# NVlabs/intrinsic3d

Hardware: AMD Instinct MI355X
Metric: Gauss-Newton iterations/s at the finest SDF level (higher is better)
Workload: dtype f32

## Files before the change

intrinsic3d_amd/csrc/device/grid_kernels.hip:

```cpp
#include "kernels.hpp"
#include "voxel_hash.hpp"

namespace i3d {

thread_local char g_errbuf[512] = {0};
static thread_local char g_launch_err[256] = {0};
bool set_dynamic_lds(const void* kernel, const char* name, size_t bytes, int K) {
    hipError_t e = bytes <= I3D_LDS_LIMIT ? hipFuncSetAttribute(kernel, hipFuncAttributeMaxDynamicSharedMemorySize, (int)bytes) : hipErrorInvalidValue;
    if (e == hipSuccess) return true;
    (void)hipGetLastError();
    if (!g_launch_err[0]) std::snprintf(g_launch_err, sizeof(g_launch_err), "%s needs %zu bytes of LDS per workgroup with K = %d keyframes (limit %zu): %s", name, bytes, K, I3D_LDS_LIMIT, hipGetErrorString(e));
    return false;
}
bool take_launch_error(char* msg, size_t n) {
    if (!g_launch_err[0]) return false;
    std::snprintf(msg, n, "%s", g_launch_err); g_launch_err[0] = 0;
    return true;
}

static __device__ inline unsigned long long spread3(unsigned long long v) {
    v &= 0x1ffffull;
    v = (v | (v << 32)) & 0x1f00000000ffffull;
    v = (v | (v << 16)) & 0x1f0000ff0000ffull;
    v = (v | (v << 8)) & 0x100f00f00f00f00full;
    v = (v | (v << 4)) & 0x10c30c30c30c30c3ull;
    v = (v | (v << 2)) & 0x1249249249249249ull;
    return v;
}

__global__ void k_sort_keys(int N, const int* __restrict__ kxyz, unsigned long long* __restrict__ keys, int* __restrict__ iota) {
    const int i = blockIdx.x * blockDim.x + threadIdx.x;
    if (i >= N) return;
    const int x = kxyz[3 * i] + (1 << 19), y = kxyz[3 * i + 1] + (1 << 19), z = kxyz[3 * i + 2] + (1 << 19);
    const unsigned long long m = spread3((unsigned)(x >> 3)) | (spread3((unsigned)(y >> 3)) << 1) | (spread3((unsigned)(z >> 3)) << 2);
    keys[i] = (m << 9) | (unsigned long long)(((z & 7) << 6) | ((y & 7) << 3) | (x & 7));
    iota[i] = i;
}
void launch_sort_keys(hipStream_t st, int N, const int* kxyz, unsigned long long* keys, int* iota) {
    if (N > 0) k_sort_keys<<<(N + 255) / 256, 256, 0, st>>>(N, kxyz, keys, iota);
}

__global__ void k_permute(int N, const int* __restrict__ perm, const int* __restrict__ kxyz, const double* __restrict__ sdf,
                          const double* __restrict__ sdf_ref, const double* __restrict__ alb, const float* __restrict__ w,
                          const uint8_t* __restrict__ rgb, int* cx, int* cy, int* cz, int* rank, double* sdf0, double* x_sdf,
                          double* x_alb, float* f_sdf, float* f_alb, float* weight, uchar4* color) {
    const int s = blockIdx.x * blockDim.x + threadIdx.x;
    if (s >= N) return;
    const int v = perm[s];
    cx[s] = kxyz[3 * v]; cy[s] = kxyz[3 * v + 1]; cz[s] = kxyz[3 * v + 2]; rank[s] = v;
    sdf0[s] = sdf[v]; x_sdf[s] = sdf_ref[v]; x_alb[s] = alb[v];
    f_sdf[s] = (float)sdf_ref[v]; f_alb[s] = (float)alb[v]; weight[s] = w[v];
    color[s] = make_uchar4(rgb[3 * v], rgb[3 * v + 1], rgb[3 * v + 2], 0);
}
void launch_permute_grid(hipStream_t st, int N, const int* perm, const int* kxyz, const double* sdf, const double* sdf_ref,
                         const double* alb, const float* w, const uint8_t* rgb, int* cx, int* cy, int* cz, int* rank, double* sdf0,
                         double* x_sdf, double* x_alb, float* f_sdf, float* f_alb, float* weight, uchar4* color) {
    if (N > 0) k_permute<<<(N + 255) / 256, 256, 0, st>>>(N, perm, kxyz, sdf, sdf_ref, alb, w, rgb, cx, cy, cz, rank, sdf0, x_sdf, x_alb, f_sdf, f_alb, weight, color);
}

__global__ void k_hash_build(int N, const int* __restrict__ cx, const int* __restrict__ cy, const int* __restrict__ cz, HashTable t) {
    const int s = blockIdx.x * blockDim.x + threadIdx.x;
    if (s >= N) return;
    const unsigned long long key = pack_key(cx[s], cy[s], cz[s]);
    unsigned int h = mix64(key) & t.mask;
    for (;;) {
        const unsigned long long prev = atomicCAS(&t.keys[h], ~0ull, key);
        if (prev == ~0ull || prev == key) { t.vals[h] = s; return; }
        h = (h + 1) & t.mask;
    }
}
void launch_hash_build(hipStream_t st, int N, const int* cx, const int* cy, const int* cz, HashTable t) {
    if (N > 0) k_hash_build<<<(N + 255) / 256, 256, 0, st>>>(N, cx, cy, cz, t);
}

__global__ void k_nbr_build(int N, const int* __restrict__ cx, const int* __restrict__ cy, const int* __restrict__ cz, HashTable t, int* __restrict__ nbr) {
    const int s = blockIdx.x * blockDim.x + threadIdx.x;
    if (s >= N) return;
    const int x = cx[s], y = cy[s], z = cz[s];
#pragma unroll
    for (int i = 0; i < NUM_NBR; ++i) {
        int dx, dy, dz; nbr_offset(i, dx, dy, dz);
        nbr[(size_t)i * N + s] = hash_find(t, x + dx, y + dy, z + dz);
    }
}
void launch_nbr_build(hipStream_t st, int N, const int* cx, const int* cy, const int* cz, HashTable t, int* nbr) {
    if (N > 0) k_nbr_build<<<(N + 255) / 256, 256, 0, st>>>(N, cx, cy, cz, t, nbr);
}

__global__ void k_classify(GridView g, OptParams p, int* __restrict__ active_flag) {
    const int s = blockIdx.x * blockDim.x + threadIdx.x;
    if (s >= g.N) return;
    const int N = g.N;
    const bool valid = g.weight[s] > 0.0f;
    const bool inshell = !(fabs(g.x_sdf[s]) > p.thres_shell);
    int nb[6]; bool nbv[6];
#pragma unroll
    for (int d = 0; d < 6; ++d) { nb[d] = g.nbr[(size_t)d * N + s]; nbv[d] = nb[d] >= 0 && g.weight[nb[d]] > 0.0f; }
    const bool ring = nbv[0] && nbv[1] && nbv[2] && nbv[3] && nbv[4] && nbv[5];
    bool normal_ok = false;
    if (valid && nbv[NB_PX] && nbv[NB_PY] && nbv[NB_PZ]) {
        const float s0 = g.f_sdf[s];
        float nx = g.f_sdf[nb[NB_PX]] - s0, ny = g.f_sdf[nb[NB_PY]] - s0, nz = g.f_sdf[nb[NB_PZ]] - s0;
        const float len = sqrtf(nx * nx + (ny * ny + nz * nz));
        if (len != 0.0f) { nx /= len; ny /= len; nz /= len; }
        normal_ok = !(fabsf(nx) <= 1e-5f && fabsf(ny) <= 1e-5f && fabsf(nz) <= 1e-5f);
    }
    const bool active = valid && inshell && normal_ok;
    const bool free_vox = valid && inshell && ring;
    const bool free_sdf = free_vox && !p.fix_sdf;
    const bool free_alb = free_vox && !(p.lambda_a < 0.0);
    g.flags[s] = (valid ? F_VALID : 0) | (active ? F_ACTIVE : 0) | (ring ? F_RING : 0) | (free_sdf ? F_FREE_SDF : 0) | (free_alb ? F_FREE_ALB : 0);
    active_flag[s] = (active || free_sdf || free_alb) ? 1 : 0;
}
void launch_classify(hipStream_t st, GridView g, OptParams p, int* active_flag) {
    if (g.N > 0) k_classify<<<(g.N + 255) / 256, 256, 0, st>>>(g, p, active_flag);
}

__global__ void k_compact(int N, const int* __restrict__ flag, const int* __restrict__ scan, const uint8_t* __restrict__ flags,
                          int* __restrict__ aidx, int* __restrict__ alist, uint8_t* __restrict__ aflags) {
    const int s = blockIdx.x * blockDim.x + threadIdx.x;
    if (s >= N) return;
    if (flag[s]) { const int a = scan[s]; aidx[s] = a; alist[a] = s; aflags[a] = flags[s]; } else aidx[s] = -1;
}
void launch_compact(hipStream_t st, int N, const int* flag, const int* scan, const uint8_t* flags, int* aidx, int* alist, uint8_t* aflags) {
    if (N > 0) k_compact<<<(N + 255) / 256, 256, 0, st>>>(N, flag, scan, flags, aidx, alist, aflags);
}

__global__ void __launch_bounds__(512) k_partition_blocks(GridView g, int A, int* __restrict__ alist, uint8_t* __restrict__ aflags, int* __restrict__ aidx) {
    __shared__ int wcount[8];
    const int base = blockIdx.x * 512, a = base + (int)threadIdx.x;
    const bool in = a < A;
    const int s = in ? alist[a] : -1;
    const uint8_t fl = in ? aflags[a] : 0;
    bool rows = in && (fl & F_ACTIVE);
    if (rows) {
#pragma unroll
        for (int c = 1; c < 10; ++c) rows &= g.nbr[(size_t)slot_fwd_nbr(c) * g.N + s] >= 0;
    }
    const unsigned long long m = __ballot(rows);
    const int lane = threadIdx.x & 63, w = threadIdx.x >> 6;
    if (lane == 0) wcount[w] = __popcll(m);
    __syncthreads();
    int before = 0, total = 0;
    for (int i = 0; i < 8; ++i) { const int cnt = wcount[i]; if (i < w) before += cnt; total += cnt; }
    const int rank_rows = before + __popcll(m & ((1ull << lane) - 1ull));
    const int pos = rows ? rank_rows : total + ((int)threadIdx.x - rank_rows);
    if (in) { const int na = base + pos; alist[na] = s; aflags[na] = fl; aidx[s] = na; }
}
void launch_partition_blocks(hipStream_t st, GridView g, int A, int* alist, uint8_t* aflags, int* aidx) {
    if (A > 0) k_partition_blocks<<<(A + 511) / 512, 512, 0, st>>>(g, A, alist, aflags, aidx);
}
__global__ void k_group_rows(int A, const uint8_t* __restrict__ nrows, int* __restrict__ gmax) {
    const int gq = blockIdx.x * blockDim.x + threadIdx.x;
    if (64 * gq >= A) return;
    int m = 0;
    for (int i = 0; i < 64 && 64 * gq + i < A; ++i) m = max(m, (int)nrows[64 * (size_t)gq + i]);
    gmax[gq] = m;
}
void launch_group_rows(hipStream_t st, int A, const uint8_t* nrows, int* gmax) { if (A > 0) k_group_rows<<<((A + 63) / 64 + 255) / 256, 256, 0, st>>>(A, nrows, gmax); }

__global__ void k_anbr(int N, int A, int Acap, const int* __restrict__ alist, const int* __restrict__ nbr, const int* __restrict__ aidx, int* __restrict__ anbr) {
    const int a = blockIdx.x * blockDim.x + threadIdx.x;
    if (a >= A) return;
    const int s = alist[a];
#pragma unroll
    for (int i = 0; i < NUM_NBR; ++i) { const int nb = nbr[(size_t)i * N + s]; anbr[(size_t)i * Acap + a] = nb >= 0 ? aidx[nb] : -1; }
}
void launch_anbr(hipStream_t st, int N, int A, int Acap, const int* alist, const int* nbr, const int* aidx, int* anbr) {
    if (A > 0) k_anbr<<<(A + 255) / 256, 256, 0, st>>>(N, A, Acap, alist, nbr, aidx, anbr);
}

__global__ void k_scatter_sh(int N, const int* __restrict__ rank, const double* __restrict__ shv, float* __restrict__ sh) {
    const int s = blockIdx.x * blockDim.x + threadIdx.x;
    if (s >= N) return;
    const double* src = shv + (size_t)rank[s] * 9;
#pragma unroll
    for (int j = 0; j < 9; ++j) sh[(size_t)j * N + s] = (float)src[j];
}
void launch_scatter_sh(hipStream_t st, int N, const int* rank, const double* shv, float* sh) {
    if (N > 0) k_scatter_sh<<<(N + 255) / 256, 256, 0, st>>>(N, rank, shv, sh);
}

__global__ void k_gather_visit(int N, const int* __restrict__ rank, const double* __restrict__ xs, const double* __restrict__ xa, double* os, double* oa) {
    const int s = blockIdx.x * blockDim.x + threadIdx.x;
    if (s >= N) return;
    const int v = rank[s];
    if (os) os[v] = xs[s];
    if (oa) oa[v] = xa[s];
}
void launch_gather_visit(hipStream_t st, int N, const int* rank, const double* xs, const double* xa, double* os, double* oa) {
    if (N > 0) k_gather_visit<<<(N + 255) / 256, 256, 0, st>>>(N, rank, xs, xa, os, oa);
}

__global__ void k_update_fields(int N, const int* __restrict__ rank, const double* sr, const double* al, const uint8_t* rgb,
                                double* x_sdf, double* x_alb, float* f_sdf, float* f_alb, uchar4* color) {
    const int s = blockIdx.x * blockDim.x + threadIdx.x;
    if (s >= N) return;
    const int v = rank[s];
    if (sr) { x_sdf[s] = sr[v]; f_sdf[s] = (float)sr[v]; }
    if (al) { x_alb[s] = al[v]; f_alb[s] = (float)al[v]; }
    if (rgb) color[s] = make_uchar4(rgb[3 * v], rgb[3 * v + 1], rgb[3 * v + 2], 0);
}
void launch_update_fields(hipStream_t st, int N, const int* rank, const double* sr, const double* al, const uint8_t* rgb,
                          double* x_sdf, double* x_alb, float* f_sdf, float* f_alb, uchar4* color) {
    if (N > 0) k_update_fields<<<(N + 255) / 256, 256, 0, st>>>(N, rank, sr, al, rgb, x_sdf, x_alb, f_sdf, f_alb, color);
}

}
```

intrinsic3d_amd/csrc/device/kernels.hpp:

```cpp
#pragma once
#include "common.hpp"
#include "p2p_device.hpp"

namespace i3d {

struct HashTable { unsigned long long* keys; int* vals; unsigned int mask; };
void launch_sort_keys(hipStream_t st, int N, const int* keys_xyz , unsigned long long* sort_keys, int* iota);
void launch_permute_grid(hipStream_t st, int N, const int* perm, const int* keys_xyz, const double* sdf, const double* sdf_ref,
                         const double* alb, const float* w, const uint8_t* rgb,
                         int* cx, int* cy, int* cz, int* rank, double* sdf0, double* x_sdf, double* x_alb, float* f_sdf, float* f_alb,
                         float* weight, uchar4* color);
void launch_hash_build(hipStream_t st, int N, const int* cx, const int* cy, const int* cz, HashTable t);
void launch_nbr_build(hipStream_t st, int N, const int* cx, const int* cy, const int* cz, HashTable t, int* nbr);
void launch_classify(hipStream_t st, GridView g, OptParams p, int* active_flag);
void launch_compact(hipStream_t st, int N, const int* active_flag, const int* active_scan, const uint8_t* flags, int* aidx, int* alist, uint8_t* aflags);
void launch_partition_blocks(hipStream_t st, GridView g, int A, int* alist, uint8_t* aflags, int* aidx);
void launch_group_rows(hipStream_t st, int A, const uint8_t* nrows, int* gmax);
void launch_anbr(hipStream_t st, int N, int A, int Acap, const int* alist, const int* nbr, const int* aidx, int* anbr);
void launch_scatter_sh(hipStream_t st, int N, const int* rank, const double* sh_visit , float* sh );
void launch_gather_visit(hipStream_t st, int N, const int* rank, const double* x_sdf, const double* x_alb, double* out_sdf, double* out_alb);
void launch_update_fields(hipStream_t st, int N, const int* rank, const double* sdf_ref, const double* alb, const uint8_t* rgb,
                          double* x_sdf, double* x_alb, float* f_sdf, float* f_alb, uchar4* color);

void launch_observe(hipStream_t st, GridView g, RowView r, OptParams p, const FrameConst* frames, const unsigned* cull_mask = nullptr, bool prefilter = false);
constexpr int CULL_BLOCK = 8, CULL_MAX_LEVELS = 12;
struct CullPyramid { int levels, cells; int bw[CULL_MAX_LEVELS], bh[CULL_MAX_LEVELS], off[CULL_MAX_LEVELS]; };
CullPyramid cull_pyramid(int w, int h);
void launch_depth_blocks(hipStream_t st, const FrameConst* frames, int K, int w, int h, float2* out);
void launch_group_cull(hipStream_t st, GridView g, RowView r, OptParams p, const FrameConst* frames, const float2* dblocks, float4* bounds, unsigned* mask);

void launch_build(hipStream_t st, GridView g, RowView r, OptParams p, const FrameConst* frames, bool with_jacobian, double* cost_out , double* scratch,
                  const double* cam9 = nullptr, const LmState* lm = nullptr);
void launch_weight_sums(hipStream_t st, RowView r, GridView g, bool with_cost, double* sums13 , double* scratch);

enum PassMode { PASS_GRAD = 0, PASS_JTJP = 1, PASS_COLNORM = 2 };
struct Seg2 { size_t off0, off1; int n; };
struct PassBuffers {
    float* C;
    float* treg;
    double* shared;
    double* blocks;
    float* part; int part_stride;
};
struct GradColBuffers {
    float* Cg; float* Cc;
    float* tregg; float* tregc;
    float* part; int part_stride;
    int col_off;
    double* cost_partials; double* cost_out;
};
int  launch_eg_gradcol(hipStream_t st, GridView g, RowView r, OptParams p, GradColBuffers b);
int  launch_eg_pass(hipStream_t st, PassMode mode, GridView g, RowView r, OptParams p, const float* u , PassBuffers b, const PcgState* state);
void launch_sum_rows(hipStream_t st, PassMode mode, int K, const float* part, int nrows, int stride, double* shared, double* blocks);
void launch_gather(hipStream_t st, PassMode mode, RowView r, PassBuffers b, float* out );
int  launch_gather_tail(hipStream_t st, RowView r, PassBuffers b, float* out, const float* S, const float* D2, const float* v, double* dot_partials ,
                        bool dot_atomic, const PcgState* state);
void launch_reduce_partials(hipStream_t st, const double* partials, int nblk, int ncomp, double* dst, const PcgState* state, bool assign = false);
void launch_shared_finalize(hipStream_t st, size_t tail_off, int K, OptParams p, const double* shared, float* out , bool tail, const float* S, const float* D2,
                            const float* v, double* dot_out, const PcgState* state);

void launch_fill(hipStream_t st, int n, float* x, float v);
void launch_fill_d(hipStream_t st, int n, double* x, double v);
void launch_int_to_double(hipStream_t st, const int* src, double* dst);
void launch_mul(hipStream_t st, int n, const float* a, const float* b, float* out);
void launch_scale_from_colnorm(hipStream_t st, int n, const float* c, const float* freemask, float* S, float* cm);
void launch_lm_diag(hipStream_t st, int n, const float* c, const float* S, float inv_radius, float* D2, float* Minv_diag);
void launch_dot(hipStream_t st, int n, const float* a, const float* b, double* out , double* scratch);
void launch_count_above2(hipStream_t st, Seg2 sg, const float* a, const float* m, float tol, double* out, double* scratch);
void launch_count_above(hipStream_t st, int n, const float* a, const float* m, float tol, double* out, double* scratch);
void launch_dot2(hipStream_t st, Seg2 sg, const float* a, const float* b, double* out , double* scratch);
void launch_mul2(hipStream_t st, Seg2 sg, const float* a, const float* b, float* out);
void launch_freemask(hipStream_t st, RowView r, OptParams p, float* mask );

void launch_pcg_init(hipStream_t st, PcgState* state, int fixed_iterations, int max_iterations, const LmState* lm = nullptr);
int  launch_pcg_step(hipStream_t st, int mode, Seg2 sg, const float* p, const float* q, float* x, float* r, const float* b, const float* D2, const float* Minv,
                     float* z, const float* S_for_inline_q, double* partials , PcgState* state);
void launch_pcg_tail_x(hipStream_t st, size_t tail_off, int K, const float* p, float* x, const PcgState* state);
void launch_pcg_tail_a(hipStream_t st, int mode, size_t tail_off, int K, const float* Minv_blocks, const float* p, const float* q, float* x, float* r, const float* b,
                       const float* D2, float* z, const double* partials, int nblk, PcgState* state,
                       double* shared_zero, int nzero, int* host_flags, int seq,
                       const P2PDev& pd);
int  launch_pcg_direction(hipStream_t st, Seg2 sg, size_t tail_off, int ntail, const float* z, float* p, const float* S, float* u, const float* D2,
                          double* d2_partials , const PcgState* state);
void launch_pcg_tail_b(hipStream_t st, size_t tail_off, int K, OptParams p, double* shared, const double* pq_slice, const double* pq_partials, int nblk,
                       const double* pq_partials2, int nblk2, bool rowwise,
                       float* q, const float* S, const float* D2, const float* v, PcgState* state, const P2PDev& pd);
struct TilePlan {
    unsigned* lnbr;
    float* eaw_sym;
    int* halo_idx; int* halo_cnt;
    int* iota; int* ext_e; int* ext_pos;
    float* qh;
    int* ext_off;
    int* overflow;
    int T, hmax;
    int tile_first, ntiles_own;
    const int* ghost_tiles; int n_ghost;
    int det;
    const unsigned short* hp_off;
    const unsigned short* hp_src;
    int pull;
};
inline int tile_plan_pull_cap(int hmax) { return 4 * hmax; }
int    tile_plan_T();
int    tile_plan_tiles(int A);
int    tile_plan_hmax();
inline int tile_plan_hmax_of(int T) { return T == 1024 ? 2048 : 1536; }
inline int tile_plan_tiles_of(int A, int T) { return (A + T - 1) / T; }
size_t tile_plan_temp_bytes(int ntiles);
hipError_t launch_tile_plan(hipStream_t st, RowView r, TilePlan t, void* temp, size_t temp_bytes);
void launch_eaw_sym(hipStream_t st, RowView r, TilePlan t, const int* cflag );
int  launch_eg_tile(hipStream_t st, RowView r, OptParams p, const float* u, TilePlan t, double* shared, float* qacc, double* pq_partials ,
                    const PcgState* state, float* cam_partials = nullptr, int cam_stride = 0);
void launch_ext_offsets(hipStream_t st, int n, const int* ext_e, int A, int* ext_off);
void eg_tile_launch_shape(const TilePlan& t, int K, int& blocks, int& tiles_per_block);

struct LadVec;
int  eg_tile_mr_max_systems(int K);
int  launch_eg_tile_mr(hipStream_t st, RowView r, OptParams p, TilePlan t, int nsys, const int* sys, const float* u0, float* qacc0, float* qh0, double* pq0 , float* cam0, int cam_stride,
                       const PcgState* st0 , const LadVec& lv);

struct ShardArgs {
    P2PDev pd; RimLists rim; int seq;
    int n_slice_partials;
    int n_rim_wg;
    const float* zb; float* pb; float* ub; const float* cmb; int chunk;
};
struct LadVec {
    size_t vec;
    size_t qh;
    size_t cam;
    size_t part;
    size_t mblk;
    size_t tail;
    int sysid[LADDER_MAX];
};
struct Step3Args {
    int nq; int chunk4;
    const float4* p; const float4* qacc; float4* x; float4* r; const float4* b; float4* z;
    const float4* cm; const LmState* lm;
    const int* ext_off; const int* ext_pos; const float2* qh; int e0;
    const double* pq_partials; int n_pq; const double* d2_partials; int n_d2;
    int n_slice_wg;
    int K; int fix_poses, fix_intr, fix_dist;
    const float* cam_partials; int n_cam; int cam_stride; const float* Mblk;
    const float* tp; float* tx; float* tr; const float* tb; const float* tD2; float* tz; const float* tS;
    double* step_partials;
    PcgState* cur;
    int sharded; ShardArgs sh;
    int lad_sys;
    const double* redop; int redop_stride;
};
void launch_pcg_init3(hipStream_t st, PcgState* st2 , int fixed_iterations, int max_iterations, const LmState* lm = nullptr);
int  launch_pcg_dir3(hipStream_t st, bool init, Seg2 sg, size_t tail_off, int ntail, const float* z, float* p, const float* S, float* u, const float* D2, const float* cm, const LmState* lm,
                     const double* step_partials, int n_step, double* d2_partials, const PcgState* prev, PcgState* next, int* host_flags, int seq,
                     const ShardArgs* sa = nullptr);
void launch_rim_u(hipStream_t st, const ShardArgs& sa, const PcgState* state);
int  pcg_step3_slice_wgs(int n_entries, int cap = 0);
int  pcg_step3_tail_wgs(int K);
int  launch_pcg_step3(hipStream_t st, int mode , Step3Args a);
void launch_halo_fold(hipStream_t st, RowView r, TilePlan t, float* qacc, const PcgState* state);
void launch_pcg_init_lad(hipStream_t st, PcgState* st2_all , int B, int fixed_iterations, int max_iterations, const LmState* lm);
int  launch_pcg_dir3_lad(hipStream_t st, bool init, int nsys, Seg2 sg, size_t tail_off, int ntail, const float* z0, float* p0, const float* S, float* u0, const float* tD2_0, const float* cm, const LmState* lm,
                         const double* step_partials0, int n_step, double* d2_partials0, PcgState* st2_0, int prev_parity, int* host_flags0, int seq, const LadVec& lv,
                         int n_slice_partials = 0, const double* red4_0 = nullptr );
int  launch_pcg_step3_lad(hipStream_t st, int mode, int nsys, Step3Args a, const LadVec& lv);
void launch_lad_reduce_step(hipStream_t st, int nsys, const double* step_partials0, int n_slice, double* red4_0, const LadVec& lv);
void launch_lad_reduce_op(hipStream_t st, int nsys, const float* cam_partials0, int n_cam, int cam_stride, int NS, const double* pq_partials0, int n_pq, const double* d2_partials0, int n_d2,
                          double* redop0, int redop_stride, const LadVec& lv);

void launch_need_mask(hipStream_t st, RowView r, int slice, unsigned long long* need );
void launch_halo_items(hipStream_t st, int A, int slice, int me, const unsigned long long* need, unsigned long long* items, int* count , int cap);
void launch_tile_flags(hipStream_t st, int A, int T, const int* cflag, int* tileflag );
size_t halo_sort_temp_bytes(int cap);
hipError_t launch_halo_sort(hipStream_t st, void* temp, size_t temp_bytes, const unsigned long long* in, unsigned long long* out, int n);

void launch_candidate(hipStream_t st, GridView g, RowView r, int K, float sign, const float* step, const float* S, const double* x_shared, double* xc_sdf, double* xc_alb,
                      double* xc_shared, double* norms2 , const float* mask, double* scratch, const LmState* lm = nullptr);
void launch_accept(hipStream_t st, GridView g, RowView r, const double* xc_sdf, const double* xc_alb, const LmState* lm = nullptr);
void launch_set_double(hipStream_t st, double* dst, double v);
void launch_lm_init(hipStream_t st, LmState* lm, const double* cost, const double* ngrad, const double* nfree, double radius0, LmRecord* rec, int seq);
void launch_lm_begin(hipStream_t st, LmState* lm, int K, int fix_poses, int fix_intr, int fix_dist, const double* cdiag, const double* tri, float* Mblk,
                     const float* tc, const float* tS, float* tD2, float* tMinv, LmRecord* rec, int seq);
void launch_lm_diag_dev(hipStream_t st, int n, const float* c, const float* S, const LmState* lm, float* D2, float* Minv);
void launch_cand_frames(hipStream_t st, int K, const double* xc, const FrameConst* base, FrameConst* out, const LmState* lm);
void launch_lm_decide(hipStream_t st, LmState* lm, const PcgState* ps, const double* norms2, const double* cand_cost, int attempt, int lm_steps, LmRecord* rec, int seq,
                      int lad_next = -1 , int debug_invalid = 0);
void launch_lm_begin_lad(hipStream_t st, LmState* lm, int B, int K, int fix_poses, int fix_intr, int fix_dist, const double* cdiag, const double* tri, float* Mblk, size_t mblk_stride,
                         const float* tc, const float* tS, float* tD2, size_t tail_stride, LmRecord* rec, int seq);
void launch_mark_compute(hipStream_t st, RowView r, int* flag);
void launch_compact_list(hipStream_t st, int A, const int* flag, const int* scan, int* list);

}
```

intrinsic3d_amd/csrc/device/pcg_fused.hip:

```cpp
#include "kernels.hpp"
#include "reduce_device.hpp"
#include <cstring>

namespace i3d {

constexpr int PF_THREADS = 512;
constexpr int PF_MAX_WG = 512;
constexpr int PF_POSES_PER_WG = 10;

template <int NC>
static __device__ inline void reduce_partials_all(const double* __restrict__ P, int nblk, double (&tot)[NC], double* sm ,
                                                  const double* __restrict__ P2 = nullptr, int nblk2 = 0 ) {
    double v[NC];
#pragma unroll
    for (int k = 0; k < NC; ++k) v[k] = 0.0;
    for (int i = threadIdx.x; i < nblk; i += PF_THREADS) {
#pragma unroll
        for (int k = 0; k < NC; ++k) v[k] += P[(size_t)i * NC + k];
    }
    for (int i = threadIdx.x; i < nblk2; i += PF_THREADS) {
#pragma unroll
        for (int k = 0; k < NC; ++k) v[k] += P2[(size_t)i * NC + k];
    }
#pragma unroll
// ... 303 lines not shown
                    }
                    if (MODE == S3_XONLY) continue;
                    const float4 bb = in.b[seg];
                    const float bv[4] = {bb.x, bb.y, bb.z, bb.w};
                    float qq[4];
#pragma unroll
                    for (int k = 0; k < 4; ++k) qq[k] = svv[k] * accv[seg][k] + dv[k] * (MODE == S3_NORMAL ? pv[k] : xv[k]);
                    if (MODE == S3_NORMAL) { const float4 ro = in.r[seg]; rv[0] = ro.x - alpha * qq[0]; rv[1] = ro.y - alpha * qq[1]; rv[2] = ro.z - alpha * qq[2]; rv[3] = ro.w - alpha * qq[3]; }
                    else { rv[0] = bv[0] - qq[0]; rv[1] = bv[1] - qq[1]; rv[2] = bv[2] - qq[2]; rv[3] = bv[3] - qq[3]; }
                    R[i] = make_float4(rv[0], rv[1], rv[2], rv[3]);
#pragma unroll
                    for (int k = 0; k < 4; ++k) { const double xd = xv[k]; s1 += xd * ((double)bv[k] + (double)rv[k]); s2 += xd * (double)rv[k]; s3 += (double)dv[k] * xd * xd; }
                }
                const float zv[4] = {mv[0] * rv[0], mv[1] * rv[1], mv[2] * rv[2], mv[3] * rv[3]};
                Z[i] = make_float4(zv[0], zv[1], zv[2], zv[3]);
#pragma unroll
                for (int k = 0; k < 4; ++k) s0 += (double)rv[k] * (double)zv[k];
            }
        }
    } else {
        const int K = a.K, tw = (int)blockIdx.x - a.n_slice_wg, n_pose_wg = (K + PF_POSES_PER_WG - 1) / PF_POSES_PER_WG;
        int col0, ncol;
        if (tw < n_pose_wg) { col0 = 6 * PF_POSES_PER_WG * tw; const int c1 = min(6 * K, col0 + 6 * PF_POSES_PER_WG); ncol = c1 - col0; }
        else { col0 = 6 * K; ncol = 9; }
        const int t = threadIdx.x;
        if (MODE == S3_NORMAL || MODE == S3_RESET) {
            const int g = t / 64, c = t % 64;
            double v = 0.0;
            if (SH != 2 && c < ncol) for (int w = g; w < a.n_cam; w += 8) v += (double)cam_partials[(size_t)w * a.cam_stride + col0 + c];
            camred[g][c] = v;
            __syncthreads();
            if (t < ncol) {
                double s = 0.0; for (int gg = 0; gg < 8; ++gg) s += camred[gg][t];
                if (SH == 2) s = a.redop[(size_t)(o.sys < 0 ? 0 : o.sys) * a.redop_stride + col0 + t];
                if (SH == 1) {
                    const unsigned e32 = p2p_pass_epoch(a.sh.seq, MODE == S3_RESET ? P2P_X_RESET_STEP : P2P_X_STEP);
                    p2p_put_double_all(a.sh.pd, 1, e32, 1 + col0 + t, s);
                    s = 0.0; for (int j = 0; j < a.sh.pd.L.world; ++j) s += p2p_get_double(a.sh.pd, 1, e32, j, 1 + col0 + t);
                }
                camv[t] = s;
            }
            __syncthreads();
        }
        if (t < ncol) {
            const int i = col0 + t;
            const bool fixed = i < 6 * K ? a.fix_poses : (i < 6 * K + 4 ? a.fix_intr : a.fix_dist);
            float ri;
            if (MODE == S3_INIT) ri = tr[i];
            else {
                float xi = tx[i];
                if (MODE != S3_RESET) { xi += alpha * tp[i]; tx[i] = xi; }
                if (MODE == S3_XONLY) ri = 0.0f;
                else {
                    const float vv = MODE == S3_NORMAL ? tp[i] : xi;
                    const float qi = a.tS[i] * (fixed ? 0.0f : (float)camv[t]) + tD2[i] * vv;
                    ri = MODE == S3_NORMAL ? tr[i] - alpha * qi : a.tb[i] - qi;
                    tr[i] = ri;
                    const double xd = xi; s1 += xd * ((double)a.tb[i] + (double)ri); s2 += xd * (double)ri; s3 += (double)tD2[i] * xd * xd;
                }
            }
            rs[t] = ri;
        }
        if (MODE == S3_XONLY) return;
        __syncthreads();
        if (t < ncol) {
            const int i = col0 + t;
            int base, n, row; const float* M;
            if (i < 6 * K) { const int f = i / 6; base = 6 * f; n = 6; row = i - base; M = Mblk + 36 * f; }
            else if (i < 6 * K + 4) { base = 6 * K; n = 4; row = i - base; M = Mblk + 36 * K; }
            else { base = 6 * K + 4; n = 5; row = i - base; M = Mblk + 36 * K + 16; }
            float s = 0.0f;
            for (int j = 0; j < n; ++j) s += M[row * n + j] * rs[base - col0 + j];
            tz[i] = s; s0 += (double)rs[t] * (double)s;
        }
    }
    if (MODE == S3_XONLY) return;
    block_partial_d(s0, step_partials, 4, 0); block_partial_d(s1, step_partials, 4, 1); block_partial_d(s2, step_partials, 4, 2); block_partial_d(s3, step_partials, 4, 3);
}
template <int MODE, int SH>
__global__ void __launch_bounds__(PF_THREADS) k_pcg_step3(Step3Args a) { const S3Off o{0, 0, 0, 0, 0, 0, 0, 0, -1}; pcg_step3_body<MODE, SH>(a, o); }
template <int MODE, bool COLL>
__global__ void __launch_bounds__(PF_THREADS) k_pcg_step3_lad(Step3Args a, LadVec lv) {
    const int j = lv.sysid[blockIdx.y];
    const S3Off o{((size_t)j * lv.vec) >> 2, (size_t)j * lv.vec, ((size_t)j * lv.qh) >> 1, (size_t)j * lv.part, (size_t)j * lv.cam, (size_t)j * lv.mblk, (size_t)j * lv.tail, 2 * j, j};
    pcg_step3_body<MODE, COLL ? 2 : 0>(a, o);
}

int pcg_step3_slice_wgs(int n_entries, int cap) { if (cap <= 0 || cap > PF_MAX_WG) cap = PF_MAX_WG; int b = (n_entries / 4 + PF_THREADS - 1) / PF_THREADS; return b < 1 ? 1 : (b > cap ? cap : b); }
int pcg_step3_tail_wgs(int K) { return (K + PF_POSES_PER_WG - 1) / PF_POSES_PER_WG + 1; }

int launch_pcg_step3(hipStream_t st, int mode, Step3Args a) {
    const int blocks = a.n_slice_wg + pcg_step3_tail_wgs(a.K);
#define I3D_S3(M) do { if (a.sharded) k_pcg_step3<M, 1><<<blocks, PF_THREADS, 0, st>>>(a); else k_pcg_step3<M, 0><<<blocks, PF_THREADS, 0, st>>>(a); } while (0)
    switch (mode) {
        case S3_INIT:   I3D_S3(S3_INIT); break;
        case S3_NORMAL: I3D_S3(S3_NORMAL); break;
        case S3_XONLY:  I3D_S3(S3_XONLY); break;
        default:        I3D_S3(S3_RESET); break;
    }
#undef I3D_S3
    return mode == S3_XONLY ? 0 : blocks;
}

int launch_pcg_step3_lad(hipStream_t st, int mode, int nsys, Step3Args a, const LadVec& lv) {
    const int blocks = a.n_slice_wg + pcg_step3_tail_wgs(a.K);
    const dim3 grid(blocks, nsys);
#define I3D_S3L(M) do { if (a.redop) k_pcg_step3_lad<M, true><<<grid, PF_THREADS, 0, st>>>(a, lv); else k_pcg_step3_lad<M, false><<<grid, PF_THREADS, 0, st>>>(a, lv); } while (0)
    switch (mode) {
        case S3_INIT:   I3D_S3L(S3_INIT); break;
        case S3_NORMAL: I3D_S3L(S3_NORMAL); break;
        case S3_XONLY:  I3D_S3L(S3_XONLY); break;
        default:        I3D_S3L(S3_RESET); break;
    }
#undef I3D_S3L
    return mode == S3_XONLY ? 0 : blocks;
}

__global__ void __launch_bounds__(PF_THREADS) k_lad_reduce_step(const double* __restrict__ step_partials0, int n_slice, double* __restrict__ red4_0, LadVec lv) {
    __shared__ double sm[4 * 8];
    const int j = lv.sysid[blockIdx.x];
    double tot[4];
    reduce_partials_all<4>(step_partials0 + (size_t)j * lv.part, n_slice, tot, sm);
    if (threadIdx.x < 4) red4_0[4 * j + threadIdx.x] = threadIdx.x == 0 ? tot[0] : threadIdx.x == 1 ? tot[1] : threadIdx.x == 2 ? tot[2] : tot[3];
}
void launch_lad_reduce_step(hipStream_t st, int nsys, const double* step_partials0, int n_slice, double* red4_0, const LadVec& lv) {
    k_lad_reduce_step<<<nsys, PF_THREADS, 0, st>>>(step_partials0, n_slice, red4_0, lv);
}
__global__ void __launch_bounds__(PF_THREADS) k_lad_reduce_op(const float* __restrict__ cam_partials0, int n_cam, int cam_stride, int NS, const double* __restrict__ pq_partials0, int n_pq,
                                                              const double* __restrict__ d2_partials0, int n_d2, double* __restrict__ redop0, int redop_stride, LadVec lv) {
    __shared__ double sm[8];
    __shared__ double camred[8][64];
    const int j = lv.sysid[blockIdx.y];
    double* const out = redop0 + (size_t)j * redop_stride;
    const int ncw = (NS + 63) / 64;
    if ((int)blockIdx.x < ncw) {
        const int t = threadIdx.x, g = t / 64, c = t % 64, col = (int)blockIdx.x * 64 + c;
        const float* cp = cam_partials0 + (size_t)j * lv.cam;
        double v = 0.0;
        if (col < NS) for (int w = g; w < n_cam; w += 8) v += (double)cp[(size_t)w * cam_stride + col];
        camred[g][c] = v;
        __syncthreads();
        if (t < 64 && col < NS) { double s = 0.0; for (int gg = 0; gg < 8; ++gg) s += camred[gg][t]; out[col] = s; }
    } else {
        double t1[1];
        reduce_partials_all<1>(pq_partials0 + (size_t)j * lv.part, n_pq, t1, sm, d2_partials0 + (size_t)j * lv.part, n_d2);
        if (threadIdx.x == 0) out[NS] = t1[0];
    }
}
void launch_lad_reduce_op(hipStream_t st, int nsys, const float* cam_partials0, int n_cam, int cam_stride, int NS, const double* pq_partials0, int n_pq, const double* d2_partials0, int n_d2,
                          double* redop0, int redop_stride, const LadVec& lv) {
    k_lad_reduce_op<<<dim3((NS + 63) / 64 + 1, nsys), PF_THREADS, 0, st>>>(cam_partials0, n_cam, cam_stride, NS, pq_partials0, n_pq, d2_partials0, n_d2, redop0, redop_stride, lv);
}

__global__ void k_pcg_init_lad(PcgState* st2_all, int B, int fixed_iterations, int max_iterations, const LmState* lm) {
    const int j = threadIdx.x;
    if (j >= B) return;
    const bool over = lm->done != 0 || lm->lad_radius[j] < 1e-32;
    for (int b = 0; b < 2; ++b) {
        PcgState* st = st2_all + 2 * j + b;
        for (int k = 0; k < 4; ++k) st->acc[k] = 0.0;
        st->rho = 0.0; st->last_rho = 1.0; st->pq = 0.0; st->alpha = 0.0; st->beta = 0.0; st->xbr = 0.0; st->xr = 0.0; st->d2xx = 0.0;
        st->Q0 = 0.0; st->Q1 = 0.0; st->it = 0; st->done = (fixed_iterations == 0 || over) ? 1 : 0; st->fixed_iterations = fixed_iterations; st->max_iterations = max_iterations;
    }
}
void launch_pcg_init_lad(hipStream_t st, PcgState* st2_all, int B, int fixed_iterations, int max_iterations, const LmState* lm) { k_pcg_init_lad<<<1, LADDER_MAX, 0, st>>>(st2_all, B, fixed_iterations, max_iterations, lm); }

__global__ void k_ext_offsets(int n, const int* __restrict__ ext_e, int A, int* __restrict__ ext_off) {
    const int e = blockIdx.x * blockDim.x + threadIdx.x;
    if (e > A) return;
    int lo = 0, hi = n;
    while (lo < hi) { const int mid = (lo + hi) >> 1; if (ext_e[mid] < e) lo = mid + 1; else hi = mid; }
    ext_off[e] = lo;
}
void launch_ext_offsets(hipStream_t st, int n, const int* ext_e, int A, int* ext_off) { k_ext_offsets<<<(A + 1 + 255) / 256, 256, 0, st>>>(n, ext_e, A, ext_off); }

}
```

intrinsic3d_amd/csrc/device/tile_pass.hip:

```cpp
#include <cstring>
#include <cstdlib>
#include <climits>
#include "kernels.hpp"
#include "reduce_device.hpp"
#include "wave_ops.hpp"
#include "tile_device.hpp"
#include <rocprim/rocprim.hpp>

namespace i3d {

constexpr int TP_PLAN_LIST = 2048;
constexpr int TP_NONE = 0x7f7f7f7f;
__device__ __host__ inline int tp_dir(int j) {
    constexpr int8_t D[18] = {NB_PY, NB_P2Y, NB_PYZ, NB_PZ, NB_P2Z, NB_PX, NB_PXY, NB_PXZ, NB_P2X, NB_MX, NB_MY, NB_MZ,
                              NB_M2Y, NB_MYZ, NB_M2Z, NB_MXY, NB_MXZ, NB_M2X};
    return D[j];
}

__global__ void __launch_bounds__(1024) k_tile_plan(RowView r, int T, int hmax, int hlimit , int tile_first, const int* __restrict__ tile_list, unsigned* __restrict__ lnbr,
                                                    int* __restrict__ halo_idx, int* __restrict__ halo_cnt, int* __restrict__ overflow) {
    __shared__ int hkeys[4096];
    __shared__ int hlist[TP_PLAN_LIST];
    __shared__ int cnt;
    const int tile = tile_list ? tile_list[blockIdx.x] : tile_first + (int)blockIdx.x, base = tile * T, a = base + threadIdx.x;
    const bool in = (int)threadIdx.x < T && a < r.A;
    const int zslot = T + hmax;
    for (int i = threadIdx.x; i < 4096; i += 1024) hkeys[i] = -1;
    hlist[threadIdx.x] = TP_NONE; hlist[threadIdx.x + 1024] = TP_NONE;
    if (threadIdx.x == 0) cnt = 0;
    __syncthreads();
    int la[18];
#pragma unroll
    for (int j = 0; j < 18; ++j) la[j] = r.anbr[(size_t)tp_dir(j) * r.Acap + (in ? a : 0)];
#pragma unroll
    for (int j = 0; j < 18; ++j) {
        if (!in) la[j] = -1;
        if (j < 12 && la[j] >= 0 && (unsigned)(la[j] - base) >= (unsigned)T) {
            unsigned h = ((unsigned)la[j] * 2654435761u) >> 20;
            for (int probes = 0; probes < 4096; ++probes) {
                const int k = atomicCAS(&hkeys[h], -1, la[j]);
                if (k == -1 || k == la[j]) break;
                h = (h + 1) & 4095u;
            }
        }
    }
    __syncthreads();
    for (int i = threadIdx.x; i < 4096; i += 1024) if (hkeys[i] >= 0) { const int pos = atomicAdd(&cnt, 1); if (pos < TP_PLAN_LIST) hlist[pos] = hkeys[i]; }
    __syncthreads();
    const int H = cnt;
    if (H > hlimit) {
        for (int i = threadIdx.x; i < hmax; i += 1024) halo_idx[(size_t)tile * hmax + i] = TP_NONE;
        if (threadIdx.x == 0) { *overflow = 1; halo_cnt[tile] = 0; }
        return;
    }
    int NS = 64; while (NS < H) NS <<= 1;
    for (int k = 2; k <= NS; k <<= 1)
        for (int j = k >> 1; j > 0; j >>= 1) {
#pragma unroll
            for (int half = 0; half < 2; ++half) {
                const int i = threadIdx.x + half * 1024, ixj = i ^ j;
                if (i < NS && ixj > i) { const int x = hlist[i], y = hlist[ixj]; const bool up = (i & k) == 0; if ((x > y) == up) { hlist[i] = y; hlist[ixj] = x; } }
            }
            __syncthreads();
        }
    for (int i = threadIdx.x; i < hmax; i += 1024) halo_idx[(size_t)tile * hmax + i] = hlist[i];
    if (threadIdx.x == 0) halo_cnt[tile] = H;
    if (!in) return;
    unsigned short ls[18];
#pragma unroll
    for (int j = 0; j < 18; ++j) {
        int slot = zslot;
        if (la[j] >= 0) {
            const unsigned off = (unsigned)(la[j] - base);
            if (off < (unsigned)T) slot = (int)off;
            else if (j < 12) { int lo = 0, hi = H - 1; while (lo < hi) { const int mid = (lo + hi) >> 1; if (hlist[mid] < la[j]) lo = mid + 1; else hi = mid; } slot = T + lo; }
        }
        ls[j] = (unsigned short)slot;
    }
    unsigned pw[LNBR_WORDS];
#pragma unroll
    for (int w = 0; w < LNBR_WORDS; ++w) pw[w] = 0u;
#pragma unroll
    for (int j = 0; j < 18; ++j) { const int bit = 12 * j, k = bit >> 5, sh = bit & 31; pw[k] |= (unsigned)ls[j] << sh; if (sh > 20) pw[k + 1] |= (unsigned)ls[j] >> (32 - sh); }
#pragma unroll
    for (int w = 0; w < LNBR_WORDS; ++w) lnbr[(size_t)w * r.Acap + a] = pw[w];
}

__global__ void __launch_bounds__(256) k_eaw_sym(RowView r, const int* __restrict__ cflag , float* __restrict__ eaw_sym) {
    const int a = blockIdx.x * blockDim.x + threadIdx.x;
    if (a >= r.A) return;
    const bool act = (r.aflags[a] & F_ACTIVE) != 0 && (!cflag || cflag[a]);
    float wo[6]; int nb[6];
#pragma unroll
    for (int d = 0; d < 6; ++d) { wo[d] = r.ea_w[(size_t)d * r.Acap + a]; nb[d] = r.anbr[(size_t)d * r.Acap + a]; }
    uint8_t nfl[6]; int ncf[6]; float wn[6];
#pragma unroll
    for (int d = 0; d < 6; ++d) { const int n = nb[d] >= 0 ? nb[d] : a; nfl[d] = r.aflags[n]; ncf[d] = cflag ? cflag[n] : 1; wn[d] = r.ea_w[(size_t)(d ^ 1) * r.Acap + n]; }
#pragma unroll
    for (int d = 0; d < 6; ++d) {
        float w = act ? wo[d] : 0.0f;
        if (nb[d] >= 0 && (nfl[d] & F_ACTIVE) && ncf[d]) w += wn[d];
        eaw_sym[(size_t)d * r.Acap + a] = w;
    }
}

template <int T, int HMAX>
__global__ void __launch_bounds__(T) k_tile_pull_plan(RowView r, int tile_first, const int* __restrict__ tile_list, const unsigned* __restrict__ lnbr, const int* __restrict__ halo_cnt,
                                                      unsigned short* __restrict__ hp_off, unsigned short* __restrict__ hp_src, int* __restrict__ overflow) {
    constexpr int CAP = 4 * HMAX, ZSLOT = T + HMAX, PER = HMAX / T, NWV = T / 64;
    static_assert(HMAX % T == 0, "slots per thread");
    __shared__ int cnt[HMAX];
    __shared__ int off[HMAX + 1];
    __shared__ unsigned short list[CAP];
    __shared__ int wsum[NWV];
    const int tile = tile_list ? tile_list[blockIdx.x] : tile_first + (int)blockIdx.x, a = tile * T + (int)threadIdx.x;
    const bool in = a < r.A;
    for (int s2 = threadIdx.x; s2 < HMAX; s2 += T) cnt[s2] = 0;
    __syncthreads();
    unsigned ln[5];
#pragma unroll
    for (int w = 0; w < 5; ++w) ln[w] = in ? lnbr[(size_t)w * r.Acap + a] : 0u;
    constexpr int RJ[18] = {0, 1, 2, 3, 4, 5, 6, 7, 8, 5, 0, 3, 5, 9, 0, 10, 3, 11};
    constexpr int RC[18] = {0, 1, 2, 3, 4, 5, 6, 7, 8, 9, 10, 11, 12, 12, 12, 12, 12, 12};
    int hs[18];
#pragma unroll
    for (int k = 0; k < 18; ++k) { const int sl = in ? unpack12(ln, RJ[k]) : ZSLOT; hs[k] = (sl >= T && sl != ZSLOT) ? sl - T : -1; if (hs[k] >= 0) atomicAdd(&cnt[hs[k]], 1); }
    __syncthreads();
    int loc[PER], sum = 0;
#pragma unroll
    for (int q = 0; q < PER; ++q) { loc[q] = cnt[threadIdx.x * PER + q]; sum += loc[q]; }
    int inc = sum;
    for (int o = 1; o < 64; o <<= 1) { const int v = __shfl_up(inc, o, 64); if ((int)(threadIdx.x & 63) >= o) inc += v; }
    if ((threadIdx.x & 63) == 63) wsum[threadIdx.x >> 6] = inc;
    __syncthreads();
    int base = 0, total = 0;
    for (int w = 0; w < NWV; ++w) { if (w < (int)(threadIdx.x >> 6)) base += wsum[w]; total += wsum[w]; }
    int run = base + inc - sum;
#pragma unroll
    for (int q = 0; q < PER; ++q) { off[threadIdx.x * PER + q] = run; run += loc[q]; }
    if (threadIdx.x == T - 1) off[HMAX] = run;
    for (int s2 = threadIdx.x; s2 < HMAX; s2 += T) cnt[s2] = 0;
    __syncthreads();
    if (total > CAP) {
        if (threadIdx.x == 0) *overflow = 1;
        for (int s2 = threadIdx.x; s2 <= HMAX; s2 += T) hp_off[(size_t)tile * (HMAX + 1) + s2] = 0;
        return;
    }
#pragma unroll
    for (int k = 0; k < 18; ++k) if (hs[k] >= 0) { const int pos = off[hs[k]] + atomicAdd(&cnt[hs[k]], 1); list[pos] = (unsigned short)((RC[k] << 10) | (int)threadIdx.x); }
    __syncthreads();
    const int H = halo_cnt[tile];
    for (int s2 = threadIdx.x; s2 < H; s2 += T) {
        const int j0 = off[s2], j1 = off[s2 + 1];
        for (int i2 = j0 + 1; i2 < j1; ++i2) { const unsigned short v = list[i2]; int j = i2 - 1; while (j >= j0 && list[j] > v) { list[j + 1] = list[j]; --j; } list[j + 1] = v; }
    }
    __syncthreads();
    for (int s2 = threadIdx.x; s2 <= HMAX; s2 += T) hp_off[(size_t)tile * (HMAX + 1) + s2] = (unsigned short)off[s2];
    for (int p2 = threadIdx.x; p2 < total; p2 += T) hp_src[(size_t)tile * CAP + p2] = list[p2];
}

template <int NV, class F>
static __device__ inline void wave_accumulate_lds(bool valid, int f, F val, float* lds, int reps, int rs, int wave_off, int stride, int base_off = 0) {
    bool pending = valid;
    unsigned long long todo = __ballot(pending);
    for (int round = 0; todo != 0ull; ++round) {
        if (round == 3) {
            if (pending) {
                int lane_rep = (int)(threadIdx.x & (unsigned)(reps - 1));
                asm volatile("" : "+v"(lane_rep));
                const int lane_off = base_off + lane_rep * rs;
#pragma unroll
                for (int i = 0; i < NV; ++i) lds_add(&lds[lane_off + stride * f + i], val(i));
            }
            break;
        }
        const int leader = __ffsll((long long)todo) - 1;
        const int f0 = __builtin_amdgcn_readlane(f, leader);
        const bool mine = pending && f == f0;
        const bool lead = (int)(threadIdx.x & 63) == leader;
#pragma unroll
        for (int i = 0; i < NV; ++i) { const float sum = wave_sum(mine ? val(i) : 0.0f); if (lead) lds_add(&lds[wave_off + stride * f0 + i], sum); }
        pending = pending && !mine;
        todo = __ballot(pending);
    }
}

template <int T, int HMAX, int SLOTS, bool GHOSTS, int DETM>
__global__ void __launch_bounds__(T, 4) k_eg_tile(RowView r, OptParams p, const float* __restrict__ u, const unsigned* __restrict__ lnbr,
                                                        const float* __restrict__ eaw_sym, const int* __restrict__ halo_idx, const int* __restrict__ halo_cnt,
                                                        double* __restrict__ shared, float* __restrict__ qacc, float* __restrict__ qh, double* __restrict__ pq_partials,
                                                        int reps, int tiles_per_block, int tile_first, int n_own ,
                                                        const int* __restrict__ ghost_list , int ntl, const PcgState* __restrict__ state,
                                                        float* __restrict__ cam_partials , int cam_stride,
                                                        const int* __restrict__ gmaxv ,
                                                        const unsigned short* __restrict__ hp_off, const unsigned short* __restrict__ hp_src ) {
    if (state && state->done) return;
    constexpr bool DET = (DETM & 3) != 0, DORD = (DETM & 1) != 0, DTAB = (DETM & 2) != 0, HP = (DETM & 4) != 0;
    static_assert(!(DORD && HP), "a pulled halo needs no ordered pushes");
    constexpr int ZSLOT = T + HMAX, NSLOT = ZSLOT + 1;
    extern __shared__ float lds[];
    const int K = p.K; const size_t Acap = r.Acap; const int A = r.A, chunk = r.chunk;
    const int nshared = 6 * K + 9;
    const int rs = (6 * K) | 1;
    constexpr int NW = T / 64, TC = T == 1024 ? 64 : 32;
    constexpr int D_CAM9W = 4, D_TAG = D_CAM9W + ((NW * 9 + 3) & ~3), D_VAL = D_TAG + NW * TC, D0 = DET ? D_VAL + NW * TC * 6 : 0;
    const int nacc = D0 + reps * rs + 9;
    const int o_upose = (nacc + 3) & ~3, o_u = (o_upose + nshared + 3) & ~3;
    for (int i = D0 + threadIdx.x; i < nacc; i += T) lds[i] = 0.0f;
#define upose (lds + o_upose)
#define u_s (lds + o_u)
#define u_a (lds + o_u + NSLOT)
#define qh_s (lds + o_u + 2 * NSLOT)
#define qh_a (lds + o_u + 2 * NSLOT + HMAX)
#define tr_l (lds + o_u + 2 * NSLOT + 2 * HMAX)
#define C_l (lds + o_u + 2 * NSLOT + 2 * HMAX + T + 4)
    const size_t tail = 2 * (size_t)chunk;
    for (int i = threadIdx.x; i < nshared; i += T) upose[i] = u[tail + i];
    const int o_cam = D0 + reps * rs;
// ... 135 lines not shown
#pragma unroll
                for (int q = 0; q < 7; ++q) { J[4 * q] = rw[q].x; J[4 * q + 1] = rw[q].y; J[4 * q + 2] = rw[q].z; J[4 * q + 3] = rw[q].w; }
                J[28] = rb.j28;
                float d = DTAB ? J[0] * u_s[i] + J[10] * u_a[i] : J[0] * us + J[10] * ua;
#pragma unroll
                for (int c = 1; c < 10; ++c) d += J[c] * u_s[unpack12(ln, c - 1)];
                d += J[11] * u_a[sx] + J[12] * u_a[sy] + J[13] * u_a[sz];
                const int o_up = o_upose + 6 * f;
#pragma unroll
                for (int q = 0; q < 6; ++q) d += J[P_POSE + q] * lds[o_up + q];
#pragma unroll
                for (int q = 0; q < 9; ++q) d += J[P_INTR + q] * ui[q];
                const float t = rho * d;
                pq_rows += t * d;
                self_s += J[0] * t; self_a += J[10] * t;
#pragma unroll
                for (int c = 1; c < 10; ++c) Cme[(c - 1) * T] += J[c] * t;
                Cme[9 * T] += J[11] * t; Cme[10 * T] += J[12] * t; Cme[11 * T] += J[13] * t;
                if (!p.fix_poses && owned) { fsel = f; pvalid = true; tsel = t; }
                if (owned) {
#pragma unroll
                    for (int q = 0; q < 9; ++q) cam9[q] += J[P_INTR + q] * t;
                }
            }
            if (DTAB) wave_table_add<6, TC>(pvalid, fsel, [&](int q) { const float j = q == 0 ? rw[3].z : q == 1 ? rw[3].w : q == 2 ? rw[4].x : q == 3 ? rw[4].y : q == 4 ? rw[4].z : rw[4].w; return j * tsel; },
                                           lds, o_tag, o_val, tcount, D0, 6);
            else wave_accumulate_lds<6>(pvalid, fsel, [&](int q) { const float j = q == 0 ? rw[3].z : q == 1 ? rw[3].w : q == 2 ? rw[4].x : q == 3 ? rw[4].y : q == 4 ? rw[4].z : rw[4].w; return j * tsel; },
                                        lds, reps, rs, o_wave_acc, 6, D0);
        };
        if (SLOTS > 0 && ghost_tile && __ballot(nr > 0) == 0ull) {
        } else if (SLOTS > 0) {
#pragma unroll
            for (int k = 0; k < SLOTS; k += 2) {
                consume(rwA, k);
                if (k + 2 < SLOTS) load_block(rwA, k + 2, SLOTS);
                if (k + 1 < SLOTS) {
                    consume(rwB, k + 1);
                    if (k + 3 < SLOTS) load_block(rwB, k + 3, SLOTS);
                }
            }
        } else {
            for (int k = 0; k < nr_max; k += 2) {
                consume(rwA, k);
                if (k + 2 < nr_max) load_block(rwA, k + 2, r.slots);
                if (k + 1 < nr_max) {
                    consume(rwB, k + 1);
                    if (k + 3 < nr_max) load_block(rwB, k + 3, r.slots);
                }
            }
        }
        if (owned) pq_l[i] += (double)pq_rows;
        unsigned lr[2];
#pragma unroll
        for (int w = 0; w < 2; ++w) lr[w] = __builtin_nontemporal_load(&lnbr[(size_t)(5 + w) * Acap + ac]);
        float eaw[6];
#pragma unroll
        for (int d = 0; d < 6; ++d) eaw[d] = __builtin_nontemporal_load(&eaw_sym[(size_t)d * Acap + ac]);
        if (DORD) {
            ordered_enter(&lds[o_det], wave);
            if (rf & 1) {
                const float tr = tr_l[i]; const int rg[6] = {sx, mx, sy, my, sz, mz};
#pragma unroll
                for (int d = 0; d < 6; ++d) if (rg[d] >= T && rg[d] != ZSLOT) lds_add(&qh_s[rg[d] - T], tr);
            }
        }
        if (!HP && nr > 0) {
#pragma unroll
            for (int c = 1; c < 10; ++c) { const int sl = unpack12(ln, c - 1); if (sl >= T && sl != ZSLOT) lds_add(&qh_s[sl - T], Cme[(c - 1) * T]); }
            if (sx >= T && sx != ZSLOT) lds_add(&qh_a[sx - T], Cme[9 * T]);
            if (sy >= T && sy != ZSLOT) lds_add(&qh_a[sy - T], Cme[10 * T]);
            if (sz >= T && sz != ZSLOT) lds_add(&qh_a[sz - T], Cme[11 * T]);
        }
        if (DTAB && DORD) { if (tcount > TC - 16) wave_table_merge<6, TC>(lds, o_tag, o_val, tcount, D0, 6); }
        if (DORD) ordered_leave(&lds[o_det], wave);
        if (DTAB && !DORD) { if (tcount > TC - 16 && (threadIdx.x & 63u) == 0u) lds[o_det] = __int_as_float(1); }
        const int a_c = a, H_c = H, tile_c = tile; const bool in_c = in, owned_c = owned; const float ua_c = DTAB ? u_a[i] : ua;
        __syncthreads();
        if (DTAB && !DORD) {
            if (__float_as_int(lds[o_det]) != 0) {
                for (int w = 0; w < NW; ++w) { if (wave == w) wave_table_merge<6, TC>(lds, o_tag, o_val, tcount, D0, 6); __syncthreads(); }
            }
        }
        if (in_c) {
            const unsigned lall[LNBR_WORDS] = {0u, 0u, 0u, 0u, ln[4], lr[0], lr[1]};
            const int r2y = unpack12(lall, 12), ryz = unpack12(lall, 13), r2z = unpack12(lall, 14), rxy = unpack12(lall, 15), rxz = unpack12(lall, 16), r2x = unpack12(lall, 17);
            auto pull = [&](int col, int slot) { return slot < T ? C_l[col * T + slot] : 0.0f; };
            float qs = self_s, qa = self_a;
            qs += pull(0, my) + pull(1, r2y) + pull(2, ryz) + pull(3, mz) + pull(4, r2z) + pull(5, mx) + pull(6, rxy) + pull(7, rxz) + pull(8, r2x);
            qa += pull(9, mx) + pull(10, my) + pull(11, mz);
            const int rg[6] = {sx, mx, sy, my, sz, mz};
#pragma unroll
            for (int d = 0; d < 6; ++d) qs += tr_l[rg[d] < T ? rg[d] : T];
            float ea = 0.0f, eq = 0.0f;
#pragma unroll
            for (int d = 0; d < 6; ++d) { const float diff = ua_c - u_a[rg[d]]; const float t = eaw[d] * diff; ea += t; eq += (rg[d] == ZSLOT ? 1.0f : 0.5f) * t * diff; }
            qa += tw3 * ea; if (owned_c) pq_l[i] += (double)(tw3 * eq);
            qacc[a_c] = qs; qacc[chunk + a_c] = qa;
        }
#pragma unroll
        for (int q = 0; q < NQH; ++q) {
            const int hq = i + q * T;
            if (hq < H_c) {
                const size_t o = (size_t)tile_c * HMAX + hq;
                if (HP) {
                    float hsum = 0.0f, hal = 0.0f;
                    const int j1 = hp_offs[hq + 1];
                    for (int j = hp_offs[hq]; j < j1; ++j) {
                        const int e = hp_list[j], col = e >> 10, lane = e & 1023;
                        const float v = col == 12 ? tr_l[lane] : C_l[col * T + lane];
                        if (col >= 9 && col != 12) hal += v; else hsum += v;
                    }
                    qh[2 * o] = hsum; qh[2 * o + 1] = hal;
                } else { qh[2 * o] = qh_s[hq]; qh[2 * o + 1] = qh_a[hq]; }
            }
        }
        __syncthreads();
    }
#pragma unroll
    for (int q = 0; q < 9; ++q) {
        float v = cam9[q];
        for (int o = 32; o > 0; o >>= 1) v += __shfl_down(v, o, 64);
        if ((threadIdx.x & 63) == 0) { if (DTAB) lds[o_cam9w + wave * 9 + q] = v; else if (v != 0.0f) lds_add(&lds[o_cam + q], v); }
    }
    __syncthreads();
    if (DTAB) {
        for (int w = 0; w < NW; ++w) { if (wave == w) wave_table_merge<6, TC>(lds, o_tag, o_val, tcount, D0, 6); __syncthreads(); }
        if (threadIdx.x < 9) { float v = 0.0f; for (int w = 0; w < NW; ++w) v += lds[o_cam9w + w * 9 + threadIdx.x]; lds[o_cam + threadIdx.x] = v; }
        __syncthreads();
    }
    for (int q = threadIdx.x; q < nshared; q += T) {
        float v;
        if (q < 6 * K) { v = 0.0f; for (int rp = 0; rp < reps; ++rp) v += lds[D0 + rp * rs + q]; }
        else v = lds[o_cam + q - 6 * K];
        if (cam_partials) cam_partials[(size_t)blockIdx.x * cam_stride + q] = v;
        else if (v != 0.0f) atomicAdd(&shared[q], (double)v);
    }
    if (pq_partials) block_partial_d(pq_l[i], pq_partials, 1, 0);
#undef pq_l
#undef hp_list
#undef hp_offs
#undef o_tag
#undef o_val
#undef upose
#undef u_s
#undef u_a
#undef qh_s
#undef qh_a
#undef tr_l
#undef C_l
#undef ui
#undef Cme
}

__global__ void __launch_bounds__(256) k_halo_fold(int n, const int* __restrict__ ext_e, const int* __restrict__ ext_pos, const float* __restrict__ qh,
                                                   float* __restrict__ qacc, int chunk, const PcgState* __restrict__ state) {
    if (state && state->done) return;
    const int i = blockIdx.x * blockDim.x + threadIdx.x;
    if (i >= n) return;
    const int e = ext_e[i];
    if (e >= TP_NONE || (i > 0 && ext_e[i - 1] == e)) return;
    float s = 0.0f, al = 0.0f;
    for (int j = i; j < n && ext_e[j] == e; ++j) { const float2 v = reinterpret_cast<const float2*>(qh)[ext_pos[j]]; s += v.x; al += v.y; }
    qacc[e] += s; qacc[chunk + e] += al;
}

__global__ void k_iota(int n, int* __restrict__ x) { const int i = blockIdx.x * blockDim.x + threadIdx.x; if (i < n) x[i] = i; }

static int tp_T() { const char* e = std::getenv("I3D_EGT_TILE"); return (e && std::atoi(e) == 512) ? 512 : 1024; }
static int tp_H() { return tp_T() == 1024 ? 2048 : 1536; }
int tile_plan_tiles(int A) { return (A + tp_T() - 1) / tp_T(); }
int tile_plan_hmax() { return tp_H(); }
size_t tile_plan_temp_bytes(int ntiles) {
    size_t bytes = 0;
    (void)rocprim::radix_sort_pairs(nullptr, bytes, (const int*)nullptr, (int*)nullptr, (const int*)nullptr, (int*)nullptr, (size_t)ntiles * tp_H(), 0, 32, (hipStream_t)0);
    return bytes;
}

hipError_t launch_tile_plan(hipStream_t st, RowView r, TilePlan t, void* temp, size_t temp_bytes) {
    const int ntiles = tile_plan_tiles_of(r.A, t.T);
    if (ntiles <= 0) return hipSuccess;
    hipError_t e = hipMemsetAsync(t.overflow, 0, sizeof(int), st); if (e != hipSuccess) return e;
    const int n = ntiles * t.hmax;
    const int limit512 = [] { const char* s = std::getenv("I3D_EGT_HMAX_LIMIT"); return s ? std::atoi(s) : 0; }();
    const int limit1024 = [] { const char* s = std::getenv("I3D_EGT_HMAX_LIMIT_1024"); return s ? std::atoi(s) : 0; }();
    const int lim = t.T == 512 ? limit512 : limit1024;
    const int hlimit = (lim > 0 && lim < t.hmax) ? lim : t.hmax;
    const bool all = t.tile_first == 0 && t.ntiles_own >= ntiles;
    if (!all) { e = hipMemsetAsync(t.halo_idx, 0x7f, sizeof(int) * (size_t)n, st); if (e != hipSuccess) return e;
                e = hipMemsetAsync(t.halo_cnt, 0, sizeof(int) * (size_t)ntiles, st); if (e != hipSuccess) return e; }
    if (t.ntiles_own > 0) k_tile_plan<<<t.ntiles_own, 1024, 0, st>>>(r, t.T, t.hmax, hlimit, t.tile_first, nullptr, t.lnbr, t.halo_idx, t.halo_cnt, t.overflow);
    if (t.n_ghost > 0) k_tile_plan<<<t.n_ghost, 1024, 0, st>>>(r, t.T, t.hmax, hlimit, 0, t.ghost_tiles, t.lnbr, t.halo_idx, t.halo_cnt, t.overflow);
    if (t.hp_off) {
        unsigned short* off = const_cast<unsigned short*>(t.hp_off); unsigned short* src = const_cast<unsigned short*>(t.hp_src);
        if (t.T == 1024) { if (t.ntiles_own > 0) k_tile_pull_plan<1024, 2048><<<t.ntiles_own, 1024, 0, st>>>(r, t.tile_first, nullptr, t.lnbr, t.halo_cnt, off, src, t.overflow);
                           if (t.n_ghost > 0) k_tile_pull_plan<1024, 2048><<<t.n_ghost, 1024, 0, st>>>(r, 0, t.ghost_tiles, t.lnbr, t.halo_cnt, off, src, t.overflow); }
        else { if (t.ntiles_own > 0) k_tile_pull_plan<512, 1536><<<t.ntiles_own, 512, 0, st>>>(r, t.tile_first, nullptr, t.lnbr, t.halo_cnt, off, src, t.overflow);
               if (t.n_ghost > 0) k_tile_pull_plan<512, 1536><<<t.n_ghost, 512, 0, st>>>(r, 0, t.ghost_tiles, t.lnbr, t.halo_cnt, off, src, t.overflow); }
    }
    k_iota<<<(n + 255) / 256, 256, 0, st>>>(n, t.iota);
    int key_bits = 32;
    for (int b = 1; b < 32; ++b) { const unsigned mask = (1u << b) - 1u; if ((1u << b) >= (unsigned)r.A && ((unsigned)TP_NONE & mask) >= (unsigned)r.A) { key_bits = b; break; } }
    e = rocprim::radix_sort_pairs(temp, temp_bytes, (const int*)t.halo_idx, t.ext_e, (const int*)t.iota, t.ext_pos, (size_t)n, 0, key_bits, st);
    if (e != hipSuccess) return e;
    if (t.ext_off) launch_ext_offsets(st, n, t.ext_e, r.chunk, t.ext_off);
    return hipGetLastError();
}

void launch_eaw_sym(hipStream_t st, RowView r, TilePlan t, const int* cflag) { if (r.A > 0) k_eaw_sym<<<(r.A + 255) / 256, 256, 0, st>>>(r, cflag, t.eaw_sym); }

struct EgtShape { int detm, reps, per_cu, blocks, tiles_per_block; size_t lds; };
template <int T, int HMAX>
static EgtShape egt_shape(const TilePlan& t, int K, int num_cu) {
    const int nshared = 6 * K + 9, rs = (6 * K) | 1;
    static const bool ordered = [] { const char* e = std::getenv("I3D_EGT_ORDERED"); return e && e[0] == '1'; }();
    const bool pull = t.pull && t.hp_off != nullptr && !(t.det && ordered);
    EgtShape s; s.detm = t.det ? (pull ? 6 : 3) : (pull ? 4 : 0);
    const bool det = (s.detm & 3) != 0;
    constexpr int NW = T / 64, TC = T == 1024 ? 64 : 32;
    const int det_words = det ? 4 + ((NW * 9 + 3) & ~3) + NW * TC * 7 : 0;
    auto lds_bytes = [&](int reps) { const int nacc = det_words + reps * rs + 9; const int o_upose = (nacc + 3) & ~3, o_u = (o_upose + nshared + 3) & ~3;
                                     return (size_t)(o_u + 2 * (T + HMAX + 1) + 2 * HMAX + T + 4 + 12 * T + 2 * T  + (pull ? (HMAX + 4) / 2 : 0) ) * sizeof(float); };
    const size_t budget = (T == 512 ? 79 : 158) * 1024;
    s.reps = (s.detm & 2) ? 1 : 4;
    while (s.reps > 1 && lds_bytes(s.reps) > budget) s.reps >>= 1;
    s.lds = lds_bytes(s.reps);
    s.per_cu = (T == 512 && s.lds <= budget) ? 2 : 1;
    { static int knob = -1; if (knob < 0) { const char* e = std::getenv("I3D_EGT_WG_PER_CU"); knob = e ? std::atoi(e) : 0; } if (knob > 0) s.per_cu = knob; }
    const int ntl = t.ntiles_own + t.n_ghost;
    s.blocks = 0; s.tiles_per_block = 0;
    if (ntl > 0) {
        s.blocks = ntl < s.per_cu * num_cu ? ntl : s.per_cu * num_cu;
        s.tiles_per_block = (ntl + s.blocks - 1) / s.blocks;
        if (ntl > s.blocks && ntl < 2 * s.blocks) { s.tiles_per_block = 1; s.blocks = ntl; }
    }
    return s;
}
static int egt_num_cu() {
    static int num_cu = 0;
    if (!num_cu) { int dev = 0; (void)hipGetDevice(&dev); hipDeviceProp_t pr; (void)hipGetDeviceProperties(&pr, dev); num_cu = pr.multiProcessorCount > 0 ? pr.multiProcessorCount : 256; }
    return num_cu;
}
void eg_tile_launch_shape(const TilePlan& t, int K, int& blocks, int& tiles_per_block) {
    const EgtShape s = t.T == 1024 ? egt_shape<1024, 2048>(t, K, egt_num_cu()) : egt_shape<512, 1536>(t, K, egt_num_cu());
    blocks = s.blocks; tiles_per_block = s.tiles_per_block;
}

template <int T, int HMAX>
static int launch_eg_tile_t(hipStream_t st, RowView r, OptParams p, const float* u, TilePlan t, double* shared, float* qacc, double* pq_partials, const PcgState* state, int num_cu,
                            float* cam_partials, int cam_stride) {
    const EgtShape sh = egt_shape<T, HMAX>(t, p.K, num_cu);
    const int detm = sh.detm, reps = sh.reps; const size_t lds = sh.lds; const bool pull = (detm & 4) != 0;
    int written = 0;
    {
        const int ntl = t.ntiles_own + t.n_ghost;
        if (ntl > 0) {
            const int blocks = sh.blocks, tiles_per_block = sh.tiles_per_block;
#define I3D_EGT(SL, GH) do { if (detm == 3) I3D_EGT2(SL, GH, 3); else if (detm == 6) I3D_EGT2(SL, GH, 6); else if (detm == 4) I3D_EGT2(SL, GH, 4); else I3D_EGT2(SL, GH, 0); } while (0)
#define I3D_EGT2(SL, GH, DT) do { \
        if (!set_dynamic_lds((const void*)k_eg_tile<T, HMAX, SL, GH, DT>, "k_eg_tile", lds, p.K)) break; \
        k_eg_tile<T, HMAX, SL, GH, DT><<<blocks, T, lds, st>>>(r, p, u, t.lnbr, t.eaw_sym, t.halo_idx, t.halo_cnt, shared, qacc, t.qh, pq_partials, reps, tiles_per_block, t.tile_first, t.ntiles_own, \
                                                   t.ghost_tiles, ntl, state, cam_partials, cam_stride, r.gmax, pull ? t.hp_off : nullptr, pull ? t.hp_src : nullptr); } while (0)
            const bool gh = t.n_ghost > 0;
            if (r.slots == 5) { if (gh) I3D_EGT(5, true); else I3D_EGT(5, false); }
            else { if (gh) I3D_EGT(0, true); else I3D_EGT(0, false); }
#undef I3D_EGT
#undef I3D_EGT2
            written = blocks;
        }
    }
    return written;
}

int launch_eg_tile(hipStream_t st, RowView r, OptParams p, const float* u, TilePlan t, double* shared, float* qacc, double* pq_partials, const PcgState* state,
                   float* cam_partials, int cam_stride) {
    if (r.A <= 0) return 0;
    const int num_cu = egt_num_cu();
    if (t.T == 1024) return launch_eg_tile_t<1024, 2048>(st, r, p, u, t, shared, qacc, pq_partials, state, num_cu, cam_partials, cam_stride);
    return launch_eg_tile_t<512, 1536>(st, r, p, u, t, shared, qacc, pq_partials, state, num_cu, cam_partials, cam_stride);
}
void launch_halo_fold(hipStream_t st, RowView r, TilePlan t, float* qacc, const PcgState* state) {
    if (r.A <= 0) return;
    const int n = tile_plan_tiles_of(r.A, t.T) * t.hmax;
    k_halo_fold<<<(n + 255) / 256, 256, 0, st>>>(n, t.ext_e, t.ext_pos, t.qh, qacc, r.chunk, state);
}
int tile_plan_T() { return tp_T(); }

}
```

intrinsic3d_amd/csrc/host/context.cpp:

```cpp
#include "context.hpp"
#include "../device/frame_math.hpp"
#include <rocprim/rocprim.hpp>
#include <algorithm>

using namespace i3d;

static thread_local std::string g_create_error;

namespace i3d {

int ctx_fail(i3d_context* c, int code, const std::string& msg) { if (c) c->err = msg; else g_create_error = msg; return code; }
int ctx_hip(i3d_context* c, hipError_t e, const char* what) {
    return ctx_fail(c, I3D_ERR_HIP, std::string(what) + " -> " + hipGetErrorString(e));
}

int ctx_launch_check(i3d_context* c) {
    char msg[256];
    if (take_launch_error(msg, sizeof(msg))) return ctx_fail(c, I3D_ERR_CAPACITY, msg);
    const hipError_t e = hipGetLastError();
    return e == hipSuccess ? I3D_OK : ctx_hip(c, e, "kernel launch");
}

int ensure_pinned(i3d_context* c, size_t n) {
    if (n <= c->h_pinned_n) return I3D_OK;
    if (c->h_pinned) (void)hipHostFree(c->h_pinned);
    c->h_pinned = nullptr; c->h_pinned_n = 0;
    CTX_HIP(c, hipHostMalloc((void**)&c->h_pinned, n * sizeof(double), hipHostMallocDefault));
    c->h_pinned_n = n;
    return I3D_OK;
}

bool timing_begin(i3d_context* c, int cat) {
    if (!c->timing.on || !((c->timing.mask >> cat) & 1u)) return false;
    Timing::Pending p; p.cat = cat;
    auto get = [&]() { hipEvent_t e; if (!c->timing.pool.empty()) { e = c->timing.pool.back(); c->timing.pool.pop_back(); } else (void)hipEventCreate(&e); return e; };
    p.a = get(); p.b = get();
    (void)hipEventRecord(p.a, c->stream);
    c->timing.pending.push_back(p);
    return true;
}
void timing_end(i3d_context* c) {
    if (c->timing.pending.empty()) return;
    (void)hipEventRecord(c->timing.pending.back().b, c->stream);
}
void timing_flush(i3d_context* c) {
    if (c->timing.pending.empty()) return;
    (void)hipStreamSynchronize(c->stream);
    for (auto& p : c->timing.pending) {
        float ms = 0.0f;
        if (hipEventElapsedTime(&ms, p.a, p.b) == hipSuccess) { c->timing.ms[p.cat] += ms; c->timing.launches[p.cat] += 1; c->timing.each[p.cat].push_back(ms); }
        c->timing.pool.push_back(p.a); c->timing.pool.push_back(p.b);
    }
    c->timing.pending.clear();
}

void build_frame_consts(const i3d_context* c, int level, const double* poses, std::vector<FrameConst>& out) {
    out.resize(c->K);
    for (int f = 0; f < c->K; ++f) {
        FrameConst& fc = out[f];
        fm::frame_from_pose(poses + 6 * f, fc);
        const size_t k = (size_t)f * c->levels + level;
        fc.hot.lum = c->lum[k].p; fc.depth = c->depth[k].p; fc.bgr = c->bgr[k].p;
        fc.w = c->fw[level]; fc.h = c->fh[level];
    }
}

}

i3d::GridView i3d_context::grid_view() const {
    GridView g;
    g.N = N; g.voxel_size = voxel_size; g.truncation = truncation;
    g.cx = cx.p; g.cy = cy.p; g.cz = cz.p; g.rank = rank.p; g.nbr = nbr.p; g.weight = weight.p; g.color = color.p;
    g.sdf0 = sdf0.p; g.x_sdf = x_sdf.p; g.x_alb = x_alb.p; g.f_sdf = f_sdf.p; g.f_alb = f_alb.p; g.sh = sh.p;
    g.flags = flags.p; g.aidx = aidx.p;
    return g;
}
i3d::RowView i3d_context::row_view() const {
    RowView r;
    r.A = A; r.Acap = Acap; r.slots = slots; r.chunk = chunk; r.world = comm ? comm->world : 1; r.own0 = own0; r.own1 = own1;
    r.clist = (comm && (comm->world > 1 || comm->force)) ? clist.p : nullptr; r.nC = nC; r.alist = alist.p; r.aflags = aflags.p; r.anbr = anbr.p; r.obs_frame = obs_frame.p; r.obs_w = obs_w.p;
    r.rows = rows.p; r.row_wr = row_wr.p; r.nrows = nrows.p; r.gmax = gmax.p; r.regflags = regflags.p; r.ea_w = ea_w.p; r.ea_free = ea_free.p;
    return r;
}

extern "C" {

const char* i3d_version(void) { return "intrinsic3d_hip 0.1 (gfx950)"; }
const char* i3d_last_error(const i3d_context* ctx) { return ctx ? ctx->err.c_str() : g_create_error.c_str(); }

int i3d_create(int32_t device_ordinal, i3d_context** out) {
    if (!out) return ctx_fail(nullptr, I3D_ERR_INVALID_ARGUMENT, "i3d_create: null output pointer");
    *out = nullptr;
    int count = 0;
    hipError_t e = hipGetDeviceCount(&count);
    if (e != hipSuccess || count <= 0)
        return ctx_fail(nullptr, I3D_ERR_NO_DEVICE, "no HIP device visible: this library has no CPU fallback");
    if (device_ordinal < 0 || device_ordinal >= count) return ctx_fail(nullptr, I3D_ERR_INVALID_ARGUMENT, "device ordinal out of range");
    e = hipSetDevice(device_ordinal);
    if (e != hipSuccess) return ctx_hip(nullptr, e, "hipSetDevice");
    auto* c = new i3d_context();
    c->device = device_ordinal;
    e = hipStreamCreateWithFlags(&c->stream, hipStreamNonBlocking);
    if (e != hipSuccess) { delete c; return ctx_hip(nullptr, e, "hipStreamCreate"); }
    *out = c;
    return I3D_OK;
}

void i3d_destroy(i3d_context* c) {
    if (!c) return;
    (void)hipSetDevice(c->device);
    timing_flush(c);
    for (auto e : c->timing.pool) (void)hipEventDestroy(e);
    if (c->h_pinned) (void)hipHostFree(c->h_pinned);
    if (c->h_pcg) (void)hipHostFree(c->h_pcg);
    if (c->h_flags) (void)hipHostFree(c->h_flags);
    if (c->h_lmrec) (void)hipHostFree(c->h_lmrec);
    for (auto e : c->ev_asm) if (e) (void)hipEventDestroy(e);
    for (auto e : c->pcg_ev) if (e) (void)hipEventDestroy(e);
    delete c->comm;
    if (c->stream) (void)hipStreamDestroy(c->stream);
    delete c;
}

int i3d_set_grid(i3d_context* c, const i3d_grid_view* gv) {
    if (!c || !gv || gv->num_voxels <= 0 || !gv->keys || !gv->sdf || !gv->sdf_refined || !gv->albedo || !gv->weight || !gv->color)
        return ctx_fail(c, I3D_ERR_INVALID_ARGUMENT, "i3d_set_grid: null grid or empty voxel list");
    if (gv->num_voxels > (1ll << 30)) return ctx_fail(c, I3D_ERR_CAPACITY, "i3d_set_grid: more than 2^30 voxels");
    CTX_HIP(c, hipSetDevice(c->device));
    const int N = (int)gv->num_voxels;
    hipStream_t st = c->stream;
    GridStaging g;
    CTX_HIP(c, g.kxyz.alloc((size_t)3 * N)); CTX_HIP(c, g.sdf.alloc(N)); CTX_HIP(c, g.sdf_ref.alloc(N)); CTX_HIP(c, g.alb.alloc(N)); CTX_HIP(c, g.w.alloc(N)); CTX_HIP(c, g.rgb.alloc((size_t)3 * N));
    CTX_HIP(c, hipMemcpyAsync(g.kxyz.p, gv->keys, sizeof(int) * 3 * (size_t)N, hipMemcpyHostToDevice, st));
    CTX_HIP(c, hipMemcpyAsync(g.sdf.p, gv->sdf, sizeof(double) * (size_t)N, hipMemcpyHostToDevice, st));
    CTX_HIP(c, hipMemcpyAsync(g.sdf_ref.p, gv->sdf_refined, sizeof(double) * (size_t)N, hipMemcpyHostToDevice, st));
    CTX_HIP(c, hipMemcpyAsync(g.alb.p, gv->albedo, sizeof(double) * (size_t)N, hipMemcpyHostToDevice, st));
    CTX_HIP(c, hipMemcpyAsync(g.w.p, gv->weight, sizeof(float) * (size_t)N, hipMemcpyHostToDevice, st));
    CTX_HIP(c, hipMemcpyAsync(g.rgb.p, gv->color, (size_t)3 * N, hipMemcpyHostToDevice, st));
    return set_grid_device(c, N, gv->voxel_size, gv->truncation, g);
}

}

namespace i3d {
int set_grid_device(i3d_context* c, int N, float voxel_size, float truncation, GridStaging& g) {
    c->N = N; c->voxel_size = voxel_size; c->truncation = truncation; c->have_grid = false; c->have_sh = false; c->have_subvolumes = false; c->assembled = false;
    c->render_bricks_ok = false;
    c->slots = 0;
    hipStream_t st = c->stream;
    DevBuf<int> perm, iota; DevBuf<unsigned long long> skeys, skeys2;
    CTX_HIP(c, perm.alloc(N)); CTX_HIP(c, iota.alloc(N)); CTX_HIP(c, skeys.alloc(N)); CTX_HIP(c, skeys2.alloc(N));
    launch_sort_keys(st, N, g.kxyz.p, skeys.p, iota.p);
    size_t tmp_bytes = 0;
    CTX_HIP(c, rocprim::radix_sort_pairs(nullptr, tmp_bytes, skeys.p, skeys2.p, iota.p, perm.p, (size_t)N, 0, 64, st));
    DevBuf<unsigned char> tmp; CTX_HIP(c, tmp.alloc(tmp_bytes));
    CTX_HIP(c, rocprim::radix_sort_pairs(tmp.p, tmp_bytes, skeys.p, skeys2.p, iota.p, perm.p, (size_t)N, 0, 64, st));
    auto fit = [&](auto& buf, size_t n) -> hipError_t { if (buf.n != n) buf.release(); return buf.alloc(n); };
    CTX_HIP(c, fit(c->cx, N)); CTX_HIP(c, fit(c->cy, N)); CTX_HIP(c, fit(c->cz, N)); CTX_HIP(c, fit(c->rank, N));
    CTX_HIP(c, fit(c->sdf0, N)); CTX_HIP(c, fit(c->x_sdf, N)); CTX_HIP(c, fit(c->x_alb, N)); CTX_HIP(c, fit(c->xc_sdf, N)); CTX_HIP(c, fit(c->xc_alb, N));
    CTX_HIP(c, fit(c->f_sdf, N)); CTX_HIP(c, fit(c->f_alb, N)); CTX_HIP(c, fit(c->weight, N)); CTX_HIP(c, fit(c->color, N));
    CTX_HIP(c, fit(c->flags, N)); CTX_HIP(c, fit(c->aidx, N)); CTX_HIP(c, fit(c->alist, N)); CTX_HIP(c, fit(c->aflag, N)); CTX_HIP(c, fit(c->ascan, N));
    CTX_HIP(c, fit(c->sh, (size_t)9 * N)); CTX_HIP(c, fit(c->nbr, (size_t)NUM_NBR * N));
    launch_permute_grid(st, N, perm.p, g.kxyz.p, g.sdf.p, g.sdf_ref.p, g.alb.p, g.w.p, g.rgb.p, c->cx.p, c->cy.p, c->cz.p, c->rank.p, c->sdf0.p,
                        c->x_sdf.p, c->x_alb.p, c->f_sdf.p, c->f_alb.p, c->weight.p, c->color.p);
    CTX_HIP(c, hipMemcpyAsync(c->xc_sdf.p, c->x_sdf.p, sizeof(double) * (size_t)N, hipMemcpyDeviceToDevice, st));
    CTX_HIP(c, hipMemcpyAsync(c->xc_alb.p, c->x_alb.p, sizeof(double) * (size_t)N, hipMemcpyDeviceToDevice, st));
    unsigned int cap = 1; while (cap < (unsigned int)N * 2u) cap <<= 1;
    CTX_HIP(c, fit(c->hkeys, cap)); CTX_HIP(c, fit(c->hvals, cap)); c->hmask = cap - 1;
    CTX_HIP(c, hipMemsetAsync(c->hkeys.p, 0xff, sizeof(unsigned long long) * (size_t)cap, st));
    HashTable t{c->hkeys.p, c->hvals.p, cap - 1};
    launch_hash_build(st, N, c->cx.p, c->cy.p, c->cz.p, t);
    launch_nbr_build(st, N, c->cx.p, c->cy.p, c->cz.p, t, c->nbr.p);
    CTX_HIP(c, hipMemsetAsync(c->sh.p, 0, sizeof(float) * 9 * (size_t)N, st));
    size_t sb = 0;
    CTX_HIP(c, rocprim::exclusive_scan(nullptr, sb, c->aflag.p, c->ascan.p, 0, (size_t)N, rocprim::plus<int>(), st));
    c->scan_tmp.release(); CTX_HIP(c, c->scan_tmp.alloc(sb ? sb : 1)); c->scan_tmp_bytes = sb;
    CTX_HIP(c, hipStreamSynchronize(st));
    CTX_HIP(c, hipGetLastError());
    c->have_grid = true;
    return I3D_OK;
}
}

extern "C" {

int i3d_get_grid(i3d_context* c, double* sdf_refined, double* albedo) {
    if (!c || !c->have_grid) return ctx_fail(c, I3D_ERR_STATE, "i3d_get_grid: no grid");
    CTX_HIP(c, hipSetDevice(c->device));
    const int N = c->N;
    DevBuf<double> a, b; CTX_HIP(c, a.alloc(N)); CTX_HIP(c, b.alloc(N));
    launch_gather_visit(c->stream, N, c->rank.p, c->x_sdf.p, c->x_alb.p, a.p, b.p);
    if (sdf_refined) CTX_HIP(c, hipMemcpyAsync(sdf_refined, a.p, sizeof(double) * (size_t)N, hipMemcpyDeviceToHost, c->stream));
    if (albedo) CTX_HIP(c, hipMemcpyAsync(albedo, b.p, sizeof(double) * (size_t)N, hipMemcpyDeviceToHost, c->stream));
    CTX_HIP(c, hipStreamSynchronize(c->stream));
    return I3D_OK;
}

int i3d_update_grid(i3d_context* c, const double* sdf_refined, const double* albedo, const uint8_t* color) {
    if (!c || !c->have_grid) return ctx_fail(c, I3D_ERR_STATE, "i3d_update_grid: no grid");
    CTX_HIP(c, hipSetDevice(c->device));
    const int N = c->N;
    DevBuf<double> a, b; DevBuf<uint8_t> col;
    if (sdf_refined) { CTX_HIP(c, a.alloc(N)); CTX_HIP(c, hipMemcpyAsync(a.p, sdf_refined, sizeof(double) * (size_t)N, hipMemcpyHostToDevice, c->stream)); }
    if (albedo) { CTX_HIP(c, b.alloc(N)); CTX_HIP(c, hipMemcpyAsync(b.p, albedo, sizeof(double) * (size_t)N, hipMemcpyHostToDevice, c->stream)); }
    if (color) { CTX_HIP(c, col.alloc((size_t)3 * N)); CTX_HIP(c, hipMemcpyAsync(col.p, color, (size_t)3 * N, hipMemcpyHostToDevice, c->stream)); }
    launch_update_fields(c->stream, N, c->rank.p, a.p, b.p, col.p, c->x_sdf.p, c->x_alb.p, c->f_sdf.p, c->f_alb.p, c->color.p);
    CTX_HIP(c, hipStreamSynchronize(c->stream));
    c->assembled = false;
    return I3D_OK;
}

int i3d_set_frames(i3d_context* c, int32_t K, int32_t levels, const int32_t* widths, const int32_t* heights,
                   const float* const* lum, const float* const* depth, const uint8_t* const* bgr) {
    if (!c || K <= 0 || levels <= 0 || !widths || !heights || !lum || !depth) return ctx_fail(c, I3D_ERR_INVALID_ARGUMENT, "i3d_set_frames: bad arguments");
    CTX_HIP(c, hipSetDevice(c->device));
    c->have_frames = false; c->K = K; c->levels = levels; c->cull_level = -1;
    c->slots = 0; c->assembled = false;
    c->fw.assign(widths, widths + levels); c->fh.assign(heights, heights + levels);
    c->lum.clear(); c->depth.clear(); c->bgr.clear();
    c->lum.resize((size_t)K * levels); c->depth.resize((size_t)K * levels); c->bgr.resize((size_t)K * levels);
    for (int f = 0; f < K; ++f) for (int l = 0; l < levels; ++l) {
        const size_t k = (size_t)f * levels + l, px = (size_t)widths[l] * heights[l];
        if (!lum[k] || !depth[k]) return ctx_fail(c, I3D_ERR_INVALID_ARGUMENT, "i3d_set_frames: null image");
        CTX_HIP(c, c->lum[k].alloc(px + 4));        CTX_HIP(c, c->depth[k].alloc(px));
        CTX_HIP(c, hipMemcpyAsync(c->lum[k].p, lum[k], px * sizeof(float), hipMemcpyHostToDevice, c->stream));
        CTX_HIP(c, hipMemcpyAsync(c->depth[k].p, depth[k], px * sizeof(float), hipMemcpyHostToDevice, c->stream));
        if (bgr && bgr[k]) { CTX_HIP(c, c->bgr[k].alloc(px * 3)); CTX_HIP(c, hipMemcpyAsync(c->bgr[k].p, bgr[k], px * 3, hipMemcpyHostToDevice, c->stream)); }
    }
    CTX_HIP(c, c->d_frames.alloc(K)); CTX_HIP(c, c->d_frames_cand.alloc(K));
    CTX_HIP(c, hipStreamSynchronize(c->stream));
    c->have_frames = true;
    if ((int)c->poses.size() != 6 * K) { c->poses.assign((size_t)6 * K, 0.0); c->have_camera = false; }
    return I3D_OK;
}

int i3d_set_camera(i3d_context* c, const double* intr, const double* dist, const double* poses) {
    if (!c || !intr || !dist || !poses) return ctx_fail(c, I3D_ERR_INVALID_ARGUMENT, "i3d_set_camera: null pointer");
    if (!c->have_frames) return ctx_fail(c, I3D_ERR_STATE, "i3d_set_camera: set the keyframes first");
    std::memcpy(c->intr, intr, sizeof(double) * 4); std::memcpy(c->dist, dist, sizeof(double) * 5);
    c->poses.assign(poses, poses + (size_t)6 * c->K);
    c->have_camera = true;
    return I3D_OK;
}
int i3d_get_camera(i3d_context* c, double* intr, double* dist, double* poses) {
    if (!c || !c->have_camera) return ctx_fail(c, I3D_ERR_STATE, "i3d_get_camera: no camera");
    if (intr) std::memcpy(intr, c->intr, sizeof(double) * 4);
    if (dist) std::memcpy(dist, c->dist, sizeof(double) * 5);
    if (poses) std::memcpy(poses, c->poses.data(), sizeof(double) * 6 * (size_t)c->K);
    return I3D_OK;
}

int i3d_set_voxel_sh(i3d_context* c, const double* voxel_sh) {
    if (!c || !voxel_sh) return ctx_fail(c, I3D_ERR_INVALID_ARGUMENT, "i3d_set_voxel_sh: null pointer");
    if (!c->have_grid) return ctx_fail(c, I3D_ERR_STATE, "i3d_set_voxel_sh: no grid");
    CTX_HIP(c, hipSetDevice(c->device));
    DevBuf<double> tmp; CTX_HIP(c, tmp.alloc((size_t)9 * c->N));
    CTX_HIP(c, hipMemcpyAsync(tmp.p, voxel_sh, sizeof(double) * 9 * (size_t)c->N, hipMemcpyHostToDevice, c->stream));
    launch_scatter_sh(c->stream, c->N, c->rank.p, tmp.p, c->sh.p);
    CTX_HIP(c, hipStreamSynchronize(c->stream));
    c->have_sh = true;
    return I3D_OK;
}
int i3d_get_voxel_sh(i3d_context* c, double* out) {
    if (!c || !out) return ctx_fail(c, I3D_ERR_INVALID_ARGUMENT, "i3d_get_voxel_sh: null pointer");
    if (!c->have_grid) return ctx_fail(c, I3D_ERR_STATE, "i3d_get_voxel_sh: no grid");
    CTX_HIP(c, hipSetDevice(c->device));
    const int N = c->N;
    std::vector<float> sh((size_t)9 * N); std::vector<int> rank(N);
    CTX_HIP(c, hipMemcpy(sh.data(), c->sh.p, sizeof(float) * 9 * (size_t)N, hipMemcpyDeviceToHost));
    CTX_HIP(c, hipMemcpy(rank.data(), c->rank.p, sizeof(int) * (size_t)N, hipMemcpyDeviceToHost));
// ... 48 lines not shown
```

intrinsic3d_amd/csrc/host/context.hpp:

```cpp
#pragma once
#include <string>
#include <vector>
#include <cstring>
#include <cmath>
#include "../device/kernels.hpp"
#include "../device/render_kernels.hpp"
#include "../device/track_kernels.hpp"
#include "comm.hpp"
#include "../../../include/intrinsic3d_hip.h"

namespace i3d {

template <class T>
struct DevBuf {
    T* p = nullptr; size_t n = 0;
    DevBuf() = default;
    DevBuf(const DevBuf&) = delete; DevBuf& operator=(const DevBuf&) = delete;
    DevBuf(DevBuf&& o) noexcept : p(o.p), n(o.n) { o.p = nullptr; o.n = 0; }
    DevBuf& operator=(DevBuf&& o) noexcept { if (this != &o) { release(); p = o.p; n = o.n; o.p = nullptr; o.n = 0; } return *this; }
    ~DevBuf() { release(); }
    void release() { if (p) (void)hipFree(p); p = nullptr; n = 0; }
    hipError_t alloc(size_t count) {
        if (count <= n && p) return hipSuccess;
        release();
        if (count == 0) return hipSuccess;
        hipError_t e = hipMalloc((void**)&p, count * sizeof(T));
        if (e == hipSuccess) n = count;
        return e;
    }
};

struct Timing {
    bool on = false;
    unsigned mask = ~0u;
    double ms[I3D_K_COUNT] = {0};
    long long launches[I3D_K_COUNT] = {0};
    std::vector<float> each[I3D_K_COUNT];
    struct Pending { hipEvent_t a, b; int cat; };
    std::vector<Pending> pending;
    std::vector<hipEvent_t> pool;
};

}

struct i3d_context {
    int device = 0;
    hipStream_t stream = nullptr;
    std::string err;

    int N = 0; float voxel_size = 0, truncation = 0;
    i3d::DevBuf<int> cx, cy, cz, rank, nbr, aidx, alist, aflag, ascan;
    i3d::DevBuf<double> sdf0, x_sdf, x_alb, xc_sdf, xc_alb;
    i3d::DevBuf<float> f_sdf, f_alb, weight, sh;
    i3d::DevBuf<uchar4> color;
    i3d::DevBuf<uint8_t> flags;
    i3d::DevBuf<unsigned char> scan_tmp; size_t scan_tmp_bytes = 0;
    i3d::DevBuf<unsigned long long> hkeys; i3d::DevBuf<int> hvals; unsigned int hmask = 0;
    bool have_grid = false, have_sh = false;
    i3d::DevBuf<unsigned> render_bits; i3d::DevBuf<int> render_bounds; int render_lo[3] = {0, 0, 0}, render_dim[3] = {0, 0, 0}; bool render_bricks_ok = false;
    i3d::DevBuf<float> render_planes; i3d::DevBuf<i3d::RenderStatsDev> render_stats;
    i3d::DevBuf<float> track_pyr, track_vn, track_model; i3d::DevBuf<double> track_slab; i3d::DevBuf<i3d::TrackState> track_state;
    i3d::DevBuf<i3d::RenderStatsDev> track_rstats;
    std::vector<unsigned long long> sv_keys; std::vector<double> sv_sh; float sv_size = 0.0f; bool have_subvolumes = false;

    int K = 0, levels = 0;
    std::vector<int> fw, fh;
    std::vector<i3d::DevBuf<float>> lum, depth;
    std::vector<i3d::DevBuf<uint8_t>> bgr;
    i3d::DevBuf<i3d::FrameConst> d_frames, d_frames_cand;
    bool have_frames = false;

    double intr[4] = {0, 0, 0, 0}, dist[5] = {0, 0, 0, 0, 0};
    std::vector<double> poses;
    bool have_camera = false;

    int Acap = 0, slots = 0, A = 0; long long n_active = 0;
    i3d::Comm* comm = nullptr; int chunk = 1, own0 = 0, own1 = 0, nC = 0;
    i3d::DevBuf<int> clist, cflag, cscan;
    i3d::HaloPlan halo; i3d::DevBuf<unsigned long long> need_mask, halo_items, halo_sorted; i3d::DevBuf<int> halo_count, halo_send_idx, halo_recv_idx, halo_send_peer, halo_recv_peer, halo_offs, tile_flag, ghost_tiles;
    i3d::DevBuf<float> halo_send_buf, halo_recv_buf; i3d::DevBuf<unsigned char> halo_temp; int n_ghost_tiles = 0, slice = 0;
    i3d::DevBuf<int> obs_frame, anbr; i3d::DevBuf<float> obs_w, ea_w, C, treg;
    i3d::DevBuf<float4> rows; i3d::DevBuf<float2> row_wr;
    i3d::DevBuf<uint8_t> aflags, nrows, regflags, ea_free; i3d::DevBuf<int> gmax;
    i3d::DevBuf<float2> cull_blocks; i3d::DevBuf<float4> cull_bounds; i3d::DevBuf<unsigned> cull_mask; int cull_level = -1; bool cull_on = false;
    double cost_at_build = 0.0;
    i3d::DevBuf<float> C2, treg2, gc_part;
    i3d::DevBuf<float> aux_part;
    i3d::DevBuf<unsigned> tp_lnbr; i3d::DevBuf<int> tp_halo_idx, tp_halo_cnt, tp_iota, tp_ext_e, tp_ext_pos, tp_ext_off, tp_overflow; i3d::DevBuf<float> tp_qh, tp_eaw, cam_part;
    i3d::DevBuf<unsigned char> tp_temp; bool tile_ok = false;
    i3d::DevBuf<unsigned short> tp_hp_off, tp_hp_src; bool halo_pull = false;
    bool ladder_lists = false;
    bool mr1_serial = false;
    int ladder_max = 1;
    int ladder_hint = 0, ladder_hint_prev = 0;
    i3d::LadVec lad{};
    i3d::DevBuf<float> lad_vec;
    i3d::DevBuf<float> lad_qh, lad_cam, lad_mblk, lad_tail;
    i3d::DevBuf<double> lad_part;
    i3d::DevBuf<double> lad_red;
    i3d::DevBuf<i3d::PcgState> lad_st;
    long long lad_batches = 0, lad_streams = 0, lad_system_passes = 0, lad_resyncs = 0, lad_wasted = 0;
    double t_add_end = 0.0;
    bool deterministic = false;
    int tile_T = 0;
    int plan_T() const { return tile_T > 0 ? tile_T : i3d::tile_plan_T(); }
    i3d::TilePlan tile_plan() const {
        const int T = plan_T();
        const bool sh = comm && (comm->world > 1 || comm->force);
        const int t0 = sh ? own0 / T : 0, t1 = sh ? (own1 + T - 1) / T : i3d::tile_plan_tiles_of(A, T);
        return i3d::TilePlan{tp_lnbr.p, tp_eaw.p, tp_halo_idx.p, tp_halo_cnt.p, tp_iota.p, tp_ext_e.p, tp_ext_pos.p, tp_qh.p, tp_ext_off.p, tp_overflow.p, T, i3d::tile_plan_hmax_of(T), t0, t1 > t0 ? t1 - t0 : 0,
                             ghost_tiles.p, sh ? n_ghost_tiles : 0, deterministic ? 1 : 0, (halo_pull || ladder_lists) ? tp_hp_off.p : nullptr, (halo_pull || ladder_lists) ? tp_hp_src.p : nullptr, halo_pull ? 1 : 0};
    }

    i3d::DevBuf<float> v_mask, v_c, v_S, v_cm, v_D2, v_Minv, v_b, v_x, v_r, v_p, v_z, v_q, v_u, v_acc, v_tmp, v_qacc;
    i3d::DevBuf<float> Minv_blocks;
    i3d::DevBuf<double> d_shared, d_blocks, d_scal, d_xshared, d_xcshared;
    i3d::DevBuf<i3d::PcgState> d_pcg, d_pcg2; i3d::DevBuf<double> d_partials; i3d::PcgState* h_pcg = nullptr; hipEvent_t pcg_ev[2] = {nullptr, nullptr};
    int* h_flags = nullptr; int* d_flags = nullptr; int pcg_seq = 1024;
    i3d::DevBuf<i3d::LmState> d_lm; i3d::LmRecord* h_lmrec = nullptr; i3d::LmRecord* d_lmrec = nullptr; int lm_seq = 1;
    i3d::DevBuf<double> d_cam_c, d_cam_H;
    hipEvent_t ev_asm[2] = {nullptr, nullptr};
    long long n_syncs = 0;
    double* h_pinned = nullptr; size_t h_pinned_n = 0;

    i3d::OptParams last_params; bool assembled = false;
    long long last_sizes[6] = {0, 0, 0, 0, 0, 0};
    i3d::Timing timing;

    i3d::GridView grid_view() const;
    i3d::RowView row_view() const;
};

namespace i3d {

int ctx_fail(i3d_context* c, int code, const std::string& msg);
int ctx_hip(i3d_context* c, hipError_t e, const char* what);
int ctx_launch_check(i3d_context* c);
#define CTX_HIP(c, expr) do { hipError_t _e = (expr); if (_e != hipSuccess) return i3d::ctx_hip((c), _e, #expr); } while (0)
void build_frame_consts(const i3d_context* c, int level, const double* poses, std::vector<FrameConst>& out);
int ensure_pinned(i3d_context* c, size_t n);
bool timing_begin(i3d_context* c, int cat);
void timing_end(i3d_context* c);
void timing_flush(i3d_context* c);
struct TimedScope { i3d_context* c; bool active; TimedScope(i3d_context* c_, int cat) : c(c_), active(timing_begin(c_, cat)) {} ~TimedScope() { if (active) timing_end(c); } };

struct GridStaging { DevBuf<int> kxyz; DevBuf<double> sdf, sdf_ref, alb; DevBuf<float> w; DevBuf<uint8_t> rgb; };
int set_grid_device(i3d_context* c, int N, float voxel_size, float truncation, GridStaging& st);

int render_ensure_bricks(i3d_context* c);
RenderGrid render_grid(const i3d_context* c, bool refined);

int recompute_colors(i3d_context* c, float occlusion_distance, int num_observations);
int clear_outside_thin_shell(i3d_context* c, double thres_shell, int64_t* new_count);
int upsample_grid(i3d_context* c, int64_t* new_count);

int assemble(i3d_context* c, const i3d_optimizer_config& cfg, int iteration, OptParams& p, i3d_iteration_stats* st);
int optimize(i3d_context* c, const i3d_optimizer_config& cfg, i3d_iteration_stats* stats);
int normal_eq_debug(i3d_context* c, double* gradient, double* jtj_diag, double* cost);
int jtj_apply_debug(i3d_context* c, const double* x, double* y);

int estimate_sh(i3d_context* c, float subvolume_size, double lambda_reg, double thres_shell, int* num_subvolumes, double* sh,
                int32_t* sub_index, int cap, i3d_sh_stats* stats);

}
```

intrinsic3d_amd/csrc/host/solver.cpp:

```cpp
#include "context.hpp"
#include <rocprim/rocprim.hpp>
#include <chrono>
#include <limits>
#include <algorithm>

namespace i3d {

#ifdef I3D_MR_PHASES
void mr_phase_report_now();
#endif
#ifdef I3D_MR_BLOCKTIME
void mr_blocktime_report_now();
#endif

static double now_s() { return std::chrono::duration<double>(std::chrono::steady_clock::now().time_since_epoch()).count(); }

static OptParams make_params(const i3d_context* c, const i3d_optimizer_config& cfg, const double* intr, const double* dist) {
    OptParams p; std::memset(&p, 0, sizeof(p));
    p.thres_shell = cfg.thres_shell; p.lambda_a = cfg.lambda_a; p.K = c->K; p.level = cfg.rgbd_level;
    p.pyr_scale = 1.0 / std::pow(2.0, cfg.rgbd_level);
    p.occlusion = cfg.occlusion_distance;
    p.use_er = (cfg.lambda_r0 > 0.0 && cfg.lambda_r1 > 0.0); p.use_es = (cfg.lambda_s0 > 0.0 && cfg.lambda_s1 > 0.0); p.use_ea = cfg.lambda_a > 0.0;
    for (int i = 0; i < 4; ++i) { p.intr[i] = intr[i]; p.cam_f[i] = (float)(intr[i] * p.pyr_scale); }
    bool dz = true;
    for (int i = 0; i < 5; ++i) { p.dist[i] = dist[i]; p.dist_f[i] = (float)dist[i]; if (std::fabs(p.dist_f[i]) > 1e-5f) dz = false; }
    p.dist_zero = dz ? 1 : 0;
    p.w = c->fw[cfg.rgbd_level]; p.h = c->fh[cfg.rgbd_level];
    p.fix_poses = cfg.fix_poses; p.fix_intr = cfg.fix_intrinsics; p.fix_dist = cfg.fix_distortion; p.fix_sdf = cfg.fix_sdf;
    return p;
}

static double varying_lambda(int it, int n, double l0, double l1) {
    if (n <= 1) return l0;
    return l0 + ((l1 - l0) / (double)(n - 1)) * (double)it;
}

constexpr int HALO_CAP = 1 << 20;
constexpr int AUX_PART_ROWS = 320;
static size_t aux_part_stride(int K) { return ((size_t)21 * K + 34 + 3) & ~(size_t)3; }
constexpr int GC_PART_ROWS = 1024;
static size_t gc_col_off(int K) { return ((size_t)6 * K + 9 + 3) & ~(size_t)3; }
static size_t gc_part_stride(int K) { return gc_col_off(K) + aux_part_stride(K); }
constexpr int PCG_SEQ_STRIDE = 1024;
constexpr int LM_REC_SLOTS = 64;

static hipError_t sync_stream(i3d_context* c) { ++c->n_syncs; return hipStreamSynchronize(c->stream); }

static int alloc_rows(i3d_context* c, int slots) {
    const size_t Acap = (size_t)c->N;
    c->Acap = (int)Acap; c->slots = slots;
    CTX_HIP(c, c->obs_frame.alloc(Acap * slots)); CTX_HIP(c, c->obs_w.alloc(Acap * slots));
    { const size_t nrow = ((Acap + 63) / 64) * 64 * (size_t)slots;
      CTX_HIP(c, c->rows.alloc(nrow / 64 * ROW_BLOCK_F4)); CTX_HIP(c, c->row_wr.alloc(nrow)); }
    CTX_HIP(c, c->aflags.alloc(Acap)); CTX_HIP(c, c->nrows.alloc(Acap)); CTX_HIP(c, c->gmax.alloc(Acap / 64 + 2)); CTX_HIP(c, c->anbr.alloc(Acap * NUM_NBR));
    CTX_HIP(c, c->cull_bounds.alloc(Acap / 64 + 2)); CTX_HIP(c, c->cull_mask.alloc((Acap / 64 + 2) * (size_t)((c->K + 31) / 32)));
    CTX_HIP(c, c->regflags.alloc(Acap)); CTX_HIP(c, c->ea_free.alloc(Acap)); CTX_HIP(c, c->ea_w.alloc(Acap * 6));
    CTX_HIP(c, c->C.alloc(Acap * P_VOX)); CTX_HIP(c, c->treg.alloc(Acap * 8)); CTX_HIP(c, c->aux_part.alloc((size_t)AUX_PART_ROWS * aux_part_stride(c->K)));
    CTX_HIP(c, c->C2.alloc(Acap * P_VOX)); CTX_HIP(c, c->treg2.alloc(Acap * 8)); CTX_HIP(c, c->gc_part.alloc((size_t)GC_PART_ROWS * gc_part_stride(c->K)));
    {
      const size_t nt = (size_t)tile_plan_tiles_of((int)Acap, 512);
      const size_t nh = std::max(nt * (size_t)tile_plan_hmax_of(512), (size_t)tile_plan_tiles_of((int)Acap, 1024) * (size_t)tile_plan_hmax_of(1024));
      CTX_HIP(c, c->tp_lnbr.alloc(Acap * LNBR_WORDS)); CTX_HIP(c, c->tp_eaw.alloc(Acap * 6)); CTX_HIP(c, c->tp_halo_idx.alloc(nh)); CTX_HIP(c, c->tp_halo_cnt.alloc(nt)); CTX_HIP(c, c->tp_iota.alloc(nh));
      CTX_HIP(c, c->tp_ext_e.alloc(nh)); CTX_HIP(c, c->tp_ext_pos.alloc(nh)); CTX_HIP(c, c->tp_qh.alloc(2 * nh)); CTX_HIP(c, c->tp_overflow.alloc(1));
      CTX_HIP(c, c->tp_ext_off.alloc(Acap + (size_t)SHARD_ALIGN * ((c->comm ? c->comm->world : 1) + 1) + 8));
      CTX_HIP(c, c->cam_part.alloc((size_t)2048 * (((size_t)6 * c->K + 9 + 3) & ~(size_t)3)));
      CTX_HIP(c, c->tp_temp.alloc(tile_plan_temp_bytes((int)nt))); }
    const int world_a = c->comm ? c->comm->world : 1;
    const size_t NP = 2 * ((size_t)c->N + (size_t)SHARD_ALIGN * (world_a + 1)) + 6 * (size_t)c->K + 9;
    for (DevBuf<float>* v : {&c->v_mask, &c->v_c, &c->v_S, &c->v_cm, &c->v_D2, &c->v_Minv, &c->v_b, &c->v_x, &c->v_r, &c->v_p, &c->v_z, &c->v_q, &c->v_u, &c->v_acc, &c->v_tmp, &c->v_qacc})
        { const bool fresh = v->n < NP || !v->p; CTX_HIP(c, v->alloc(NP)); if (fresh) CTX_HIP(c, hipMemsetAsync(v->p, 0, sizeof(float) * v->n, c->stream)); }
    CTX_HIP(c, c->Minv_blocks.alloc((size_t)36 * c->K + 16 + 25));
    CTX_HIP(c, c->d_shared.alloc((size_t)6 * c->K + 9 + 1)); CTX_HIP(c, c->d_blocks.alloc((size_t)21 * c->K + 25));
    CTX_HIP(c, c->clist.alloc(Acap)); CTX_HIP(c, c->cflag.alloc(Acap)); CTX_HIP(c, c->cscan.alloc(Acap));
    if (c->comm) {
        const size_t cap = HALO_CAP;
        CTX_HIP(c, c->need_mask.alloc(Acap)); CTX_HIP(c, c->halo_items.alloc(cap)); CTX_HIP(c, c->halo_sorted.alloc(cap)); CTX_HIP(c, c->halo_count.alloc(1));
        CTX_HIP(c, c->halo_send_idx.alloc(cap)); CTX_HIP(c, c->halo_recv_idx.alloc(cap)); CTX_HIP(c, c->halo_send_peer.alloc(cap)); CTX_HIP(c, c->halo_recv_peer.alloc(cap)); CTX_HIP(c, c->halo_offs.alloc(2 * P2P_MAX_RANKS)); CTX_HIP(c, c->halo_send_buf.alloc((size_t)HALO_MULTI_MAX * (2 * cap))); CTX_HIP(c, c->halo_recv_buf.alloc((size_t)HALO_MULTI_MAX * (2 * cap)));
        CTX_HIP(c, c->halo_temp.alloc(halo_sort_temp_bytes((int)cap)));
        const size_t nt = (size_t)tile_plan_tiles_of((int)Acap, 512) + 1; CTX_HIP(c, c->tile_flag.alloc(nt)); CTX_HIP(c, c->ghost_tiles.alloc(nt));
    }
    CTX_HIP(c, c->d_scal.alloc(32)); CTX_HIP(c, c->d_xshared.alloc((size_t)6 * c->K + 9)); CTX_HIP(c, c->d_xcshared.alloc((size_t)6 * c->K + 9));
    CTX_HIP(c, c->d_pcg.alloc(1)); CTX_HIP(c, c->d_pcg2.alloc(2));
    CTX_HIP(c, c->d_partials.alloc((Acap / 256 + 2048) * 9));
    if (!c->h_pcg) CTX_HIP(c, hipHostMalloc((void**)&c->h_pcg, 2 * sizeof(PcgState), hipHostMallocDefault));
    for (auto& e : c->pcg_ev) if (!e) CTX_HIP(c, hipEventCreateWithFlags(&e, hipEventDisableTiming));
    if (!c->h_flags) { CTX_HIP(c, hipHostMalloc((void**)&c->h_flags, 32 * sizeof(int), hipHostMallocMapped | hipHostMallocCoherent));
                       for (int i = 0; i < 32; ++i) c->h_flags[i] = -1;
                       CTX_HIP(c, hipHostGetDevicePointer((void**)&c->d_flags, c->h_flags, 0)); }
    CTX_HIP(c, c->d_lm.alloc(1)); CTX_HIP(c, c->d_cam_c.alloc((size_t)6 * c->K + 9)); CTX_HIP(c, c->d_cam_H.alloc((size_t)21 * c->K + 25));
    if (!c->h_lmrec) { CTX_HIP(c, hipHostMalloc((void**)&c->h_lmrec, LM_REC_SLOTS * sizeof(LmRecord), hipHostMallocMapped | hipHostMallocCoherent));
                       std::memset(c->h_lmrec, 0, LM_REC_SLOTS * sizeof(LmRecord));
                       CTX_HIP(c, hipHostGetDevicePointer((void**)&c->d_lmrec, c->h_lmrec, 0)); }
    for (auto& e : c->ev_asm) if (!e) CTX_HIP(c, hipEventCreate(&e));
    return ensure_pinned(c, 64 + (size_t)27 * c->K + 64);
}

struct Layout { int A, K, NS, chunk, world, rank, slice; Seg2 own; size_t tail_off, NP; };
static Layout layout_of(const i3d_context* c) {
    Layout L; L.A = c->A; L.K = c->K; L.NS = 6 * c->K + 9; L.chunk = c->chunk; L.world = c->comm ? c->comm->world : 1; L.rank = c->comm ? c->comm->rank : 0;
    L.slice = L.chunk / L.world;
    L.own = Seg2{(size_t)L.rank * L.slice, (size_t)L.chunk + (size_t)L.rank * L.slice, L.slice};
    L.tail_off = 2 * (size_t)L.chunk; L.NP = L.tail_off + L.NS;
    return L;
}
static bool sharded(const i3d_context* c) { return c->comm && (c->comm->world > 1 || c->comm->force); }
static bool env_off(const char* name) { const char* e = std::getenv(name); return e && e[0] == '0'; }
static bool one_stream_gradcol(const i3d_context* c) { return !sharded(c) && !env_off("I3D_GRADCOL"); }
static bool cost_from_sums(const i3d_context* c) { return !env_off("I3D_COST0") && !one_stream_gradcol(c); }

static int allreduce(i3d_context* c, double* dev, size_t n) {
    if (!sharded(c)) return I3D_OK;
    TimedScope t(c, I3D_K_COMM);
    return c->comm->allreduce_sum(dev, n, c->stream) ? ctx_fail(c, I3D_ERR_COMM, "all-reduce failed") : I3D_OK;
}
static int allgather(i3d_context* c, float* vec) {
    if (!sharded(c)) return I3D_OK;
    const size_t slice = (size_t)(c->chunk / c->comm->world);
    TimedScope t(c, I3D_K_COMM);
    if (c->comm->allgather(vec, slice, c->stream) || c->comm->allgather(vec + c->chunk, slice, c->stream)) return ctx_fail(c, I3D_ERR_COMM, "all-gather failed");
    return I3D_OK;
}
static int push_halo(i3d_context* c, float* vec) {
    if (!sharded(c)) return I3D_OK;
    TimedScope t(c, I3D_K_COMM);
    return c->comm->push_halo(vec, c->halo, c->stream) ? ctx_fail(c, I3D_ERR_COMM, "halo exchange failed") : I3D_OK;
}

static int shard_plan(i3d_context* c) {
    hipStream_t s = c->stream;
    const int world = c->comm->world, rank = c->comm->rank;
    if (world > 64) return ctx_fail(c, I3D_ERR_CAPACITY, "sharding: more than 64 ranks");
    shard_range(c->A, world, rank, c->chunk, c->own0, c->own1); c->nC = 0; c->slice = c->chunk / world;
    RowView r0 = c->row_view();
    TimedScope t(c, I3D_K_CLASSIFY);
    launch_mark_compute(s, r0, c->cflag.p);
    CTX_HIP(c, rocprim::exclusive_scan(c->scan_tmp.p, c->scan_tmp_bytes, c->cflag.p, c->cscan.p, 0, (size_t)c->A, rocprim::plus<int>(), s));
    launch_compact_list(s, c->A, c->cflag.p, c->cscan.p, c->clist.p);
    const int T = c->plan_T(), ntiles = tile_plan_tiles_of(c->A, T);
    CTX_HIP(c, hipMemsetAsync(c->need_mask.p, 0, sizeof(unsigned long long) * (size_t)c->A, s));
    CTX_HIP(c, hipMemsetAsync(c->halo_count.p, 0, sizeof(int), s));
    CTX_HIP(c, hipMemsetAsync(c->tile_flag.p, 0, sizeof(int) * (size_t)(ntiles + 1), s));
    launch_need_mask(s, r0, c->slice, c->need_mask.p);
    launch_halo_items(s, c->A, c->slice, rank, c->need_mask.p, c->halo_items.p, c->halo_count.p, HALO_CAP);
    launch_tile_flags(s, c->A, T, c->cflag.p, c->tile_flag.p);
    int tl[2] = {0, 0}, nitems = 0;
    if (c->A > 0) { CTX_HIP(c, hipMemcpyAsync(&tl[0], c->cscan.p + (c->A - 1), sizeof(int), hipMemcpyDeviceToHost, s));
                    CTX_HIP(c, hipMemcpyAsync(&tl[1], c->cflag.p + (c->A - 1), sizeof(int), hipMemcpyDeviceToHost, s)); }
    CTX_HIP(c, hipMemcpyAsync(&nitems, c->halo_count.p, sizeof(int), hipMemcpyDeviceToHost, s));
    std::vector<int> tf((size_t)ntiles + 1, 0);
    CTX_HIP(c, hipMemcpyAsync(tf.data(), c->tile_flag.p, sizeof(int) * (size_t)ntiles, hipMemcpyDeviceToHost, s));
    CTX_HIP(c, sync_stream(c));
    c->nC = tl[0] + tl[1];
    if (nitems > HALO_CAP) return ctx_fail(c, I3D_ERR_CAPACITY, "sharding: the halo plan does not fit its buffers");
    std::vector<int> ghosts; const int t0 = c->own0 / T, t1 = (c->own1 + T - 1) / T;
    for (int i = 0; i < ntiles; ++i) if (tf[i] && (i < t0 || i >= t1)) ghosts.push_back(i);
    c->n_ghost_tiles = (int)ghosts.size();
    if (!ghosts.empty()) CTX_HIP(c, hipMemcpyAsync(c->ghost_tiles.p, ghosts.data(), sizeof(int) * ghosts.size(), hipMemcpyHostToDevice, s));
    HaloPlan& h = c->halo; h.world = world; h.chunk = c->chunk;
    h.send_cnt.assign(world, 0); h.send_off.assign(world, 0); h.recv_cnt.assign(world, 0); h.recv_off.assign(world, 0); h.n_send = h.n_recv = 0;
    std::vector<unsigned long long> items((size_t)nitems);
    if (nitems > 0) {
        CTX_HIP(c, launch_halo_sort(s, c->halo_temp.p, c->halo_temp.n, c->halo_items.p, c->halo_sorted.p, nitems));
        CTX_HIP(c, hipMemcpyAsync(items.data(), c->halo_sorted.p, sizeof(unsigned long long) * (size_t)nitems, hipMemcpyDeviceToHost, s));
        CTX_HIP(c, sync_stream(c));
    }
    std::vector<int> sidx, ridx, speer, rpeer;
    for (unsigned long long it : items) {
        const int dir = (int)(it >> 40) & 1, peer = (int)((it >> 32) & 0xFF), e = (int)(it & 0xFFFFFFFFull);
        if (dir == 0) { if (h.send_cnt[peer]++ == 0) h.send_off[peer] = (int)sidx.size(); sidx.push_back(e); speer.push_back(peer); }
        else          { if (h.recv_cnt[peer]++ == 0) h.recv_off[peer] = (int)ridx.size(); ridx.push_back(e); rpeer.push_back(peer); }
    }
    h.n_send = (int)sidx.size(); h.n_recv = (int)ridx.size();
    if (h.n_send) { CTX_HIP(c, hipMemcpyAsync(c->halo_send_idx.p, sidx.data(), sizeof(int) * sidx.size(), hipMemcpyHostToDevice, s));
                    CTX_HIP(c, hipMemcpyAsync(c->halo_send_peer.p, speer.data(), sizeof(int) * speer.size(), hipMemcpyHostToDevice, s)); }
    if (h.n_recv) { CTX_HIP(c, hipMemcpyAsync(c->halo_recv_idx.p, ridx.data(), sizeof(int) * ridx.size(), hipMemcpyHostToDevice, s));
                    CTX_HIP(c, hipMemcpyAsync(c->halo_recv_peer.p, rpeer.data(), sizeof(int) * rpeer.size(), hipMemcpyHostToDevice, s)); }
    int offs[2 * P2P_MAX_RANKS] = {0};
    for (int k = 0; k < world; ++k) { offs[k] = h.send_off[k]; offs[P2P_MAX_RANKS + k] = h.recv_off[k]; }
    CTX_HIP(c, hipMemcpyAsync(c->halo_offs.p, offs, sizeof(offs), hipMemcpyHostToDevice, s));
    CTX_HIP(c, sync_stream(c));
    h.d_send_idx = c->halo_send_idx.p; h.d_recv_idx = c->halo_recv_idx.p; h.d_send_buf = c->halo_send_buf.p; h.d_recv_buf = c->halo_recv_buf.p;
    { const int prc = c->comm->plan_changed(h, s);
      if (prc == 2) return ctx_fail(c, I3D_ERR_CAPACITY, "sharding: the rim of a rank pair exceeds the peer-to-peer mailbox");
      if (prc) return ctx_fail(c, I3D_ERR_COMM, "sharding: installing the halo lists of the peer-to-peer transport failed on a rank (HIP / copy error)"); }
    return I3D_OK;
}

static int read_doubles(i3d_context* c, const double* dptr, size_t n, double* out) {
    CTX_HIP(c, hipMemcpyAsync(c->h_pinned, dptr, n * sizeof(double), hipMemcpyDeviceToHost, c->stream));
    CTX_HIP(c, sync_stream(c));
    std::memcpy(out, c->h_pinned, n * sizeof(double));
    return I3D_OK;
}

int assemble(i3d_context* c, const i3d_optimizer_config& cfg, int iteration, OptParams& p, i3d_iteration_stats* st) {
    if (!c->have_grid || !c->have_frames || !c->have_camera) return ctx_fail(c, I3D_ERR_STATE, "optimize: grid, keyframes and camera must be set");
    if (cfg.rgbd_level < 0 || cfg.rgbd_level >= c->levels) return ctx_fail(c, I3D_ERR_INVALID_ARGUMENT, "optimize: rgbd_level outside the uploaded pyramid");
    int slots = (cfg.num_observations <= 0 || cfg.num_observations >= c->K) ? c->K : cfg.num_observations;
    if (slots > MAX_SLOTS) return ctx_fail(c, I3D_ERR_CAPACITY, "optimize: more than 8 observations per voxel requested");
    if (c->K > 2000) return ctx_fail(c, I3D_ERR_CAPACITY, "optimize: more than 2000 keyframes (the camera accumulators of the operator pass live in 160 KB of LDS)");
    if (c->slots != slots || c->Acap != c->N || !c->rows.p) { int rc = alloc_rows(c, slots); if (rc) return rc; }
    hipStream_t s = c->stream;
    CTX_HIP(c, hipEventRecord(c->ev_asm[0], s));
    p = make_params(c, cfg, c->intr, c->dist);
    GridView g = c->grid_view();
    { TimedScope t(c, I3D_K_CLASSIFY);
      launch_classify(s, g, p, c->aflag.p);
      CTX_HIP(c, rocprim::exclusive_scan(c->scan_tmp.p, c->scan_tmp_bytes, c->aflag.p, c->ascan.p, 0, (size_t)c->N, rocprim::plus<int>(), s));
      launch_compact(s, c->N, c->aflag.p, c->ascan.p, c->flags.p, c->aidx.p, c->alist.p, c->aflags.p); }
    int tail[2];
    CTX_HIP(c, hipMemcpyAsync(&tail[0], c->ascan.p + (c->N - 1), sizeof(int), hipMemcpyDeviceToHost, s));
    CTX_HIP(c, hipMemcpyAsync(&tail[1], c->aflag.p + (c->N - 1), sizeof(int), hipMemcpyDeviceToHost, s));
    std::vector<FrameConst> fc; build_frame_consts(c, cfg.rgbd_level, c->poses.data(), fc);
    CTX_HIP(c, sync_stream(c));
    CTX_HIP(c, hipMemcpyAsync(c->d_frames.p, fc.data(), sizeof(FrameConst) * fc.size(), hipMemcpyHostToDevice, s));
    c->A = tail[0] + tail[1];
    { TimedScope t(c, I3D_K_CLASSIFY);
      static const bool no_partition = [] { const char* e = std::getenv("I3D_NO_PARTITION"); return e && e[0] == '1'; }();
      if (!no_partition) launch_partition_blocks(s, g, c->A, c->alist.p, c->aflags.p, c->aidx.p);
      launch_anbr(s, c->N, c->A, c->Acap, c->alist.p, c->nbr.p, c->aidx.p, c->anbr.p); }
    c->tile_ok = false; c->tile_T = 0;
    { const char* e = std::getenv("I3D_DETERMINISTIC"); c->deterministic = e ? e[0] == '1' : !sharded(c); }
    {
        const char* e = std::getenv("I3D_LADDER"); const int v = e ? std::atoi(e) : LADDER_MAX;
        c->ladder_max = v < 1 ? 1 : (v > LADDER_MAX ? LADDER_MAX : v);
        if (slots != 5 || eg_tile_mr_max_systems(c->K) < 2) c->ladder_max = 1;
        if (sharded(c)) { P2PDev probe; if (c->comm->fused_exchange(&probe)) c->ladder_max = 1; }
        { const char* l = std::getenv("I3D_PCG_LEGACY"); if (l && l[0] == '1') c->ladder_max = 1; }
        { const char* m1 = std::getenv("I3D_EGT_MR1"); c->mr1_serial = m1 && m1[0] == '1' && !sharded(c) && slots == 5 && eg_tile_mr_max_systems(c->K) >= 1; }
        c->ladder_lists = c->ladder_max > 1 || c->mr1_serial;
    }
    {
        const char* e = std::getenv("I3D_HALO_PULL");
        c->halo_pull = c->deterministic || (e && e[0] == '1');
        if (c->halo_pull || c->ladder_lists) {
            const size_t n512 = (size_t)tile_plan_tiles_of(c->Acap, 512), n1024 = (size_t)tile_plan_tiles_of(c->Acap, 1024);
            CTX_HIP(c, c->tp_hp_off.alloc(std::max(n512 * (size_t)(1536 + 1), n1024 * (size_t)(2048 + 1)) + 8));
            CTX_HIP(c, c->tp_hp_src.alloc(std::max(n512 * (size_t)tile_plan_pull_cap(1536), n1024 * (size_t)tile_plan_pull_cap(2048)) + 8));
        }
    }
    if (!sharded(c)) {
        { const long long la = c->last_sizes[0], lr = c->last_sizes[1];
          const bool forced = std::getenv("I3D_EGT_TILE") != nullptr;
          if (!forced && la > 0 && (double)lr < 0.8 * (double)slots * (double)la) c->tile_T = 512;
          if (c->ladder_max > 1 || c->mr1_serial) c->tile_T = 512; }
        shard_range(c->A, 1, 0, c->chunk, c->own0, c->own1); c->nC = c->A; c->slice = c->chunk;
        RowView r0 = c->row_view(); TimedScope t(c, I3D_K_CLASSIFY);
        CTX_HIP(c, launch_tile_plan(s, r0, c->tile_plan(), c->tp_temp.p, c->tp_temp.n));
    } else {
        const int first_T = (c->ladder_max > 1) ? 512 : ((c->A / c->comm->world >= 2 * 256 * 1024) ? 1024 : 512);
        c->tile_T = first_T;
        for (int attempt = 0; attempt < 2; ++attempt) {
            int rc = shard_plan(c); if (rc) return rc;
            { RowView r0 = c->row_view(); TimedScope t(c, I3D_K_CLASSIFY);
              CTX_HIP(c, launch_tile_plan(s, r0, c->tile_plan(), c->tp_temp.p, c->tp_temp.n)); }
            launch_fill_d(s, 1, c->d_scal.p + 20, 0.0); launch_int_to_double(s, c->tp_overflow.p, c->d_scal.p + 20);
            rc = allreduce(c, c->d_scal.p + 20, 1); if (rc) return rc;
            double over = 0.0; rc = read_doubles(c, c->d_scal.p + 20, 1, &over); if (rc) return rc;
            if (over == 0.0) break;
            if (attempt == 1) return ctx_fail(c, I3D_ERR_CAPACITY, "sharded optimize: a tile of the operator pass reaches more foreign entries than either tile geometry has halo slots");
            const int other = c->plan_T() == 512 ? 1024 : 512;
            std::fprintf(stderr, "[i3d] sharded operator pass: a %d-entry tile's halo does not fit, planning again with %d-entry tiles\n", c->plan_T(), other);
            c->tile_T = other;
        }
        CTX_HIP(c, hipMemsetAsync(c->nrows.p, 0, (size_t)c->A, s)); CTX_HIP(c, hipMemsetAsync(c->regflags.p, 0, (size_t)c->A, s));
    }
    RowView r = c->row_view();
    { TimedScope t(c, I3D_K_OBSERVE);
      const char* e = std::getenv("I3D_NO_CULL"); const char mode = e ? e[0] : '0';
      const unsigned* mask = nullptr; c->cull_on = !(mode == '1' || mode == '2'); const bool prefilter = !(mode == '1' || mode == '3');
      if (c->cull_on) {
          if (c->cull_level != cfg.rgbd_level || !c->cull_blocks.p) {
              CTX_HIP(c, c->cull_blocks.alloc((size_t)c->K * cull_pyramid(p.w, p.h).cells));
              launch_depth_blocks(s, c->d_frames.p, c->K, p.w, p.h, c->cull_blocks.p); c->cull_level = cfg.rgbd_level; }
          launch_group_cull(s, g, r, p, c->d_frames.p, c->cull_blocks.p, c->cull_bounds.p, c->cull_mask.p); mask = c->cull_mask.p; }
      launch_observe(s, g, r, p, c->d_frames.p, mask, prefilter); }
    CTX_HIP(c, hipEventRecord(c->ev_asm[1], s));
    { TimedScope t(c, I3D_K_BUILD); launch_build(s, g, r, p, c->d_frames.p, true, nullptr, c->d_partials.p); }
    { TimedScope t(c, I3D_K_CLASSIFY); launch_group_rows(s, c->A, c->nrows.p, c->gmax.p); }
    { TimedScope t(c, I3D_K_CLASSIFY); launch_eaw_sym(s, r, c->tile_plan(), sharded(c) ? c->cflag.p : nullptr); }
    CTX_HIP(c, hipMemsetAsync(c->d_scal.p, 0, sizeof(double) * 32, s));
    { TimedScope t(c, I3D_K_VECTOR); launch_weight_sums(s, r, g, cost_from_sums(c), c->d_scal.p, c->d_partials.p); }
    { int rc = allreduce(c, c->d_scal.p, 13); if (rc) return rc; }
    int tp_over = 1;
    CTX_HIP(c, hipMemcpyAsync(&tp_over, c->tp_overflow.p, sizeof(int), hipMemcpyDeviceToHost, s));
    double sums[13]; { int rc = read_doubles(c, c->d_scal.p, 13, sums); if (rc) return rc; }
    if (sharded(c) && c->comm->health(s)) return ctx_fail(c, I3D_ERR_COMM, "assemble: a peer-to-peer exchange timed out (a rank stopped taking part)");
    if (!sharded(c) && tp_over != 0) {
        const int other = c->plan_T() == 1024 ? 512 : 1024;
        std::fprintf(stderr, "[i3d] operator pass: a %d-entry tile's halo does not fit, planning again with %d-entry tiles\n", c->plan_T(), other);
        c->tile_T = other;
        { RowView r0 = c->row_view(); TimedScope t(c, I3D_K_CLASSIFY);
          CTX_HIP(c, launch_tile_plan(s, r0, c->tile_plan(), c->tp_temp.p, c->tp_temp.n)); }
        CTX_HIP(c, hipMemcpyAsync(&tp_over, c->tp_overflow.p, sizeof(int), hipMemcpyDeviceToHost, s));
        CTX_HIP(c, sync_stream(c));
    }
    c->tile_ok = tp_over == 0;
    if (!sharded(c) && !c->tile_ok) std::fprintf(stderr, "[i3d] operator pass: a tile's halo does not fit, using the untiled pass (k_eg_jtjp + k_gather)\n");
    if (sharded(c) && !c->tile_ok) return ctx_fail(c, I3D_ERR_CAPACITY, "sharded optimize: the tile plan overflowed after it had been accepted");
    if (!sharded(c)) { const char* e = std::getenv("I3D_NO_TILE"); if (e && e[0] == '1') c->tile_ok = false; }
    sums[5] = sums[1]; sums[6] = sums[2];
    const double lambda[4] = {cfg.lambda_g, varying_lambda(iteration, cfg.iterations, cfg.lambda_r0, cfg.lambda_r1),
                              varying_lambda(iteration, cfg.iterations, cfg.lambda_s0, cfg.lambda_s1), cfg.lambda_a};
    for (int t = 0; t < 4; ++t) { p.type_w[t] = sums[t] != 0.0 ? (lambda[t] / sums[t]) * 1000.0 : 0.0; p.type_wf[t] = (float)p.type_w[t]; }
    c->n_active = (long long)(sums[8] + 0.5);
    c->cost_at_build = 0.5 * (p.type_w[0] * sums[9] + p.type_w[1] * sums[10] + p.type_w[2] * sums[11] + p.type_w[3] * sums[12]);
    if (st) { for (int t = 0; t < 4; ++t) { st->rows[t] = (int64_t)(sums[4 + t] + 0.5); st->weight_sum[t] = sums[t]; st->type_weight[t] = p.type_w[t]; } st->valid_voxels = c->n_active; }
    c->last_sizes[0] = c->n_active; for (int t = 0; t < 4; ++t) c->last_sizes[1 + t] = (long long)(sums[4 + t] + 0.5);
    c->last_params = p; c->assembled = true;
    { float ms = 0.0f; c->t_add_end = (hipEventElapsedTime(&ms, c->ev_asm[0], c->ev_asm[1]) == hipSuccess) ? (double)ms * 1e-3 : -1.0; }
    { const int lrc = ctx_launch_check(c); if (lrc) return lrc; }
    return I3D_OK;
}

static int run_pass(i3d_context* c, PassMode mode, const OptParams& p, const float* u, float* out ) {
    hipStream_t s = c->stream; GridView g = c->grid_view(); RowView r = c->row_view(); const Layout L = layout_of(c);
    const int stride = (int)aux_part_stride(c->K);
    PassBuffers b{c->C.p, c->treg.p, c->d_shared.p, c->d_blocks.p, c->aux_part.p, stride};
    CTX_HIP(c, hipMemsetAsync(c->d_shared.p, 0, sizeof(double) * ((size_t)L.NS + 1), s));
    if (mode == PASS_COLNORM) CTX_HIP(c, hipMemsetAsync(c->d_blocks.p, 0, sizeof(double) * (21 * (size_t)c->K + 25), s));
    if (mode == PASS_JTJP && c->tile_ok && !sharded(c)) {
        const int NSP = (L.NS + 3) & ~3; int rows = 0;
        { TimedScope t(c, I3D_K_EG_PASS); rows = launch_eg_tile(s, r, p, u, c->tile_plan(), nullptr, out, nullptr, nullptr, c->cam_part.p, NSP); }
        { TimedScope t(c, I3D_K_GATHER); launch_halo_fold(s, r, c->tile_plan(), out, nullptr); }
        { TimedScope t(c, I3D_K_VECTOR); launch_mul(s, 2 * c->chunk, c->v_mask.p, out, out);
          if (rows > 0) launch_sum_rows(s, PASS_JTJP, c->K, c->cam_part.p, rows, NSP, c->d_shared.p, c->d_blocks.p); }
    } else {
        int rows = 0;
        { TimedScope t(c, mode == PASS_JTJP ? I3D_K_EG_PASS : I3D_K_EG_AUX); rows = launch_eg_pass(s, mode, g, r, p, u, b, nullptr);
          if (rows > AUX_PART_ROWS) return ctx_fail(c, I3D_ERR_CAPACITY, "run_pass: more workgroups than rows of the camera partial buffer");
          if (rows > 0) launch_sum_rows(s, mode, c->K, c->aux_part.p, rows, stride, c->d_shared.p, c->d_blocks.p); }
        { TimedScope t(c, I3D_K_GATHER); launch_gather(s, mode, r, b, out); }
    }
    { int rc = allreduce(c, c->d_shared.p, (size_t)L.NS); if (rc) return rc; }
    if (mode == PASS_COLNORM) { int rc = allreduce(c, c->d_blocks.p, 21 * (size_t)c->K + 25); if (rc) return rc; }
    { TimedScope t(c, I3D_K_VECTOR); launch_shared_finalize(s, L.tail_off, c->K, p, c->d_shared.p, out, false, nullptr, nullptr, nullptr, nullptr, nullptr); }
    return I3D_OK;
}

template <class F> static int run_gradcol(i3d_context* c, const OptParams& p, F between) {
    hipStream_t s = c->stream; GridView g = c->grid_view(); RowView r = c->row_view(); const Layout L = layout_of(c);
    const int stride = (int)gc_part_stride(c->K), col_off = (int)gc_col_off(c->K);
    GradColBuffers gb{c->C.p, c->C2.p, c->treg.p, c->treg2.p, c->gc_part.p, stride, col_off, c->d_partials.p, c->d_scal.p + 16};
    CTX_HIP(c, hipMemsetAsync(c->d_scal.p + 16, 0, sizeof(double), s));
    CTX_HIP(c, hipMemsetAsync(c->d_shared.p, 0, sizeof(double) * ((size_t)L.NS + 1), s));
    CTX_HIP(c, hipMemsetAsync(c->d_blocks.p, 0, sizeof(double) * (21 * (size_t)c->K + 25), s));
    int rows = 0;
    { TimedScope t(c, I3D_K_EG_AUX); rows = launch_eg_gradcol(s, g, r, p, gb);
      if (rows > GC_PART_ROWS) return ctx_fail(c, I3D_ERR_CAPACITY, "run_gradcol: more workgroups than rows of the camera partial buffer");
      if (rows > 0) launch_sum_rows(s, PASS_COLNORM, c->K, c->gc_part.p + col_off, rows, stride, c->d_shared.p, c->d_blocks.p); }
    { PassBuffers b{c->C2.p, c->treg2.p, c->d_shared.p, c->d_blocks.p, nullptr, 0};
      TimedScope t(c, I3D_K_GATHER); launch_gather(s, PASS_COLNORM, r, b, c->v_c.p); }
    { TimedScope t(c, I3D_K_VECTOR); launch_shared_finalize(s, L.tail_off, c->K, p, c->d_shared.p, c->v_c.p, false, nullptr, nullptr, nullptr, nullptr, nullptr); }
    { int rc = between(); if (rc) return rc; }
    CTX_HIP(c, hipMemsetAsync(c->d_shared.p, 0, sizeof(double) * ((size_t)L.NS + 1), s));
    { TimedScope t(c, I3D_K_EG_AUX); if (rows > 0) launch_sum_rows(s, PASS_GRAD, c->K, c->gc_part.p, rows, stride, c->d_shared.p, c->d_blocks.p); }
    { PassBuffers b{c->C.p, c->treg.p, c->d_shared.p, c->d_blocks.p, nullptr, 0};
      TimedScope t(c, I3D_K_GATHER); launch_gather(s, PASS_GRAD, r, b, c->v_acc.p); }
    { TimedScope t(c, I3D_K_VECTOR); launch_shared_finalize(s, L.tail_off, c->K, p, c->d_shared.p, c->v_acc.p, false, nullptr, nullptr, nullptr, nullptr, nullptr); }
    return I3D_OK;
}

static int dot_dev(i3d_context* c, const float* a, const float* b, double* slot) {
    const Layout L = layout_of(c);
    CTX_HIP(c, hipMemsetAsync(slot, 0, sizeof(double), c->stream));
    { TimedScope t(c, I3D_K_VECTOR); launch_dot2(c->stream, L.own, a, b, slot, c->d_partials.p); }
    { int rc = allreduce(c, slot, 1); if (rc) return rc; }
    { TimedScope t(c, I3D_K_VECTOR); launch_dot(c->stream, L.NS, a + L.tail_off, b + L.tail_off, slot, c->d_partials.p); }
    return I3D_OK;
}

static int count_above_dev(i3d_context* c, const float* a, const float* m, float tol, double* slot) {
    const Layout L = layout_of(c);
    CTX_HIP(c, hipMemsetAsync(slot, 0, sizeof(double), c->stream));
    { TimedScope t(c, I3D_K_VECTOR); launch_count_above2(c->stream, L.own, a, m, tol, slot, c->d_partials.p); }
    { int rc = allreduce(c, slot, 1); if (rc) return rc; }
    { TimedScope t(c, I3D_K_VECTOR); launch_count_above(c->stream, L.NS, a + L.tail_off, m + L.tail_off, tol, slot, c->d_partials.p); }
    return I3D_OK;
}

static int eval_cost_launch(i3d_context* c, const OptParams& p, bool candidate, const FrameConst* frames, const double* cam9 = nullptr, const LmState* lm = nullptr) {
    GridView g = c->grid_view();
    if (candidate) { g.x_sdf = c->xc_sdf.p; g.x_alb = c->xc_alb.p; }
    { TimedScope t(c, I3D_K_COST); launch_build(c->stream, g, c->row_view(), p, frames, false, c->d_scal.p + 16, c->d_partials.p, cam9, lm); }
    return allreduce(c, c->d_scal.p + 16, 1);
}
static int eval_cost(i3d_context* c, const OptParams& p, bool candidate, const FrameConst* frames, double* cost) {
    int rc = eval_cost_launch(c, p, candidate, frames); if (rc) return rc;
    rc = read_doubles(c, c->d_scal.p + 16, 1, cost); if (rc) return rc;
    if (sharded(c) && c->comm->health(c->stream)) return ctx_fail(c, I3D_ERR_COMM, "cost evaluation: a peer-to-peer exchange timed out (a rank stopped taking part)");
    return I3D_OK;
}

static int pcg_solve(i3d_context* c, const i3d_optimizer_config& cfg, const OptParams& p, const PcgState** final_state) {
    hipStream_t s = c->stream;
    const Layout L = layout_of(c);
    const int K = c->K; const bool multi = sharded(c), tiled = c->tile_ok;
    GridView g = c->grid_view(); RowView r = c->row_view();
    PassBuffers pb{c->C.p, c->treg.p, c->d_shared.p, c->d_blocks.p, c->aux_part.p, (int)aux_part_stride(c->K)};
    PcgState* st = c->d_pcg.p;
    double* pq_slot = c->d_shared.p + L.NS;
    const size_t to = L.tail_off; const Seg2 own = L.own;
    { TimedScope t(c, I3D_K_VECTOR); launch_fill(s, (int)L.NP, c->v_x.p, 0.0f); launch_pcg_init(s, st, cfg.pcg_fixed_iterations, 500, c->d_lm.p); }
    CTX_HIP(c, hipMemcpyAsync(c->v_r.p, c->v_b.p, sizeof(float) * L.NP, hipMemcpyDeviceToDevice, s));
    double* const step_part = c->d_partials.p; double* const pq_part = c->d_partials.p + 4 * 2048; double* const d2_part = pq_part + 1024;
    int n_pq = 0, n_step = 0, n_d2 = 0;
    P2PDev pd; std::memset(&pd, 0, sizeof(pd));
    const bool fused = multi && tiled && c->comm->device_reduce(&pd) && L.NS + 1 <= pd.L.red_cap;
    if (!fused) pd.on = 0;
    auto rows_apply = [&](const float* v, float* out, bool with_dot, bool zero_first) -> int {
        if (zero_first) CTX_HIP(c, hipMemsetAsync(c->d_shared.p, 0, sizeof(double) * ((size_t)L.NS + 1), s));
        if (multi) { int rc = push_halo(c, c->v_u.p); if (rc) return rc; }
        if (tiled) {
            { TimedScope t(c, I3D_K_EG_PASS);
              n_pq = launch_eg_tile(s, r, p, c->v_u.p, c->tile_plan(), c->d_shared.p, c->v_qacc.p, with_dot ? pq_part : nullptr, st); }
            { TimedScope t(c, I3D_K_GATHER); launch_halo_fold(s, r, c->tile_plan(), c->v_qacc.p, st); }
            if (!with_dot) n_pq = 0;
            if (!multi || (fused && with_dot)) return I3D_OK;
            if (with_dot) { TimedScope t(c, I3D_K_VECTOR); launch_reduce_partials(s, pq_part, n_pq, 1, pq_slot, st); launch_reduce_partials(s, d2_part, n_d2, 1, pq_slot, st); }
            n_pq = 0;
            return allreduce(c, c->d_shared.p, (size_t)L.NS + 1);
        }
        { TimedScope t(c, I3D_K_EG_PASS); launch_eg_pass(s, PASS_JTJP, g, r, p, c->v_u.p, pb, st); }
        { TimedScope t(c, I3D_K_GATHER); n_pq = launch_gather_tail(s, r, pb, out, c->v_S.p, c->v_D2.p, v, with_dot ? pq_part : nullptr, false, st); }
        if (!with_dot) n_pq = 0;
        return I3D_OK;
    };
    auto fold_step = [&]() { if (multi && !fused) { launch_reduce_partials(s, step_part, n_step, 4, st->acc, st); n_step = 0; } };
    const float* const Sq = tiled ? c->v_S.p : nullptr;
    { TimedScope t(c, I3D_K_VECTOR);
      n_step = launch_pcg_step(s, 0 , own, c->v_p.p, c->v_q.p, c->v_x.p, c->v_r.p, c->v_b.p, c->v_D2.p, c->v_Minv.p, c->v_z.p, nullptr, step_part, st);
      fold_step(); }
    int tail_mode = 0;
    const int seq0 = c->pcg_seq;
    int it = 1;
    for (;; ++it) {
        if (multi && !fused) { int rc = allreduce(c, st->acc, 4); if (rc) return rc; }
        if (fused) { c->comm->count_reduce(4); c->comm->count_reduce((size_t)L.NS + 1); }
        { TimedScope t(c, I3D_K_VECTOR);
// ... 16 lines not shown
              launch_pcg_tail_x(s, to, K, c->v_p.p, c->v_x.p, st);
              launch_mul2(s, own, c->v_S.p, c->v_x.p, c->v_u.p); launch_mul(s, L.NS, c->v_S.p + to, c->v_x.p + to, c->v_u.p + to); }
            { int rc = rows_apply(c->v_x.p, c->v_tmp.p, false, true); if (rc) return rc; }
            { TimedScope t(c, I3D_K_VECTOR);
              launch_shared_finalize(s, to, K, p, c->d_shared.p, c->v_tmp.p, true, c->v_S.p, c->v_D2.p, c->v_x.p, nullptr, st);
              n_step = launch_pcg_step(s, 3, own, c->v_p.p, tiled ? c->v_qacc.p : c->v_tmp.p, c->v_x.p, c->v_r.p, c->v_b.p, c->v_D2.p, c->v_Minv.p, c->v_z.p, Sq, step_part, st);
              fold_step(); }
            tail_mode = 3;
        }
        if (it >= 2) {
            const int want = seq0 + it - 1; volatile int* ring = c->h_flags + 2 * (want & 1);
            const double t_wait = now_s();
            while (__atomic_load_n((int*)&ring[0], __ATOMIC_ACQUIRE) != want) {
                if (now_s() - t_wait > 30.0) { CTX_HIP(c, sync_stream(c)); if (__atomic_load_n((int*)&ring[0], __ATOMIC_ACQUIRE) != want) return ctx_fail(c, I3D_ERR_HIP, "pcg_solve: the device stopped publishing its state"); }
            }
            if (__atomic_load_n((int*)&ring[1], __ATOMIC_ACQUIRE)) break;
        }
        if (it > 520) break;
    }
    c->pcg_seq = seq0 + PCG_SEQ_STRIDE;
    *final_state = st;
    return I3D_OK;
}

static int pcg_solve_fused(i3d_context* c, const i3d_optimizer_config& cfg, const OptParams& p, const PcgState** final_state) {
    hipStream_t s = c->stream;
    const Layout L = layout_of(c);
    const int K = c->K; const size_t to = L.tail_off; const Seg2 own = L.own;
    RowView r = c->row_view(); TilePlan tp = c->tile_plan();
    const bool sh = sharded(c);
    ShardArgs sa; std::memset(&sa, 0, sizeof(sa));
    if (sh) {
        if (!c->comm->fused_exchange(&sa.pd) || L.NS + 2 > sa.pd.L.red_cap) return ctx_fail(c, I3D_ERR_STATE, "pcg_solve_fused: the in-kernel exchanges are not available");
        const HaloPlan& h = c->halo;
        sa.rim = RimLists{h.n_send, h.n_recv, c->halo_send_idx.p, c->halo_send_peer.p, c->halo_recv_idx.p, c->halo_recv_peer.p, c->halo_offs.p, c->halo_offs.p + P2P_MAX_RANKS};
        sa.n_rim_wg = (h.n_send + h.n_recv) > 0 ? std::max(1, std::min(4, (std::max(h.n_send, h.n_recv) + 1023) / 1024)) : 1;
        sa.zb = c->v_z.p; sa.pb = c->v_p.p; sa.ub = c->v_u.p; sa.cmb = c->v_cm.p; sa.chunk = c->chunk;
    }
    const int wg_cap = sh ? sa.pd.wg_cap : 0;
    PcgState* const st2 = c->d_pcg2.p;
    const int NSP = (L.NS + 3) & ~3;
    double* const step_part = c->d_partials.p; double* const pq_part = c->d_partials.p + 4 * 2048; double* const d2_part = pq_part + 2048;
    { TimedScope t(c, I3D_K_VECTOR); launch_fill(s, (int)L.NP, c->v_x.p, 0.0f); launch_pcg_init3(s, st2, cfg.pcg_fixed_iterations, 500, c->d_lm.p); }
    CTX_HIP(c, hipMemcpyAsync(c->v_r.p, c->v_b.p, sizeof(float) * L.NP, hipMemcpyDeviceToDevice, s));
    Step3Args a; std::memset(&a, 0, sizeof(a));
    auto c4 = [&](const float* v) { return reinterpret_cast<const float4*>(v + own.off0); };
    auto m4 = [&](float* v) { return reinterpret_cast<float4*>(v + own.off0); };
    a.nq = own.n >> 2; a.chunk4 = (int)((own.off1 - own.off0) >> 2);
    a.p = c4(c->v_p.p); a.qacc = c4(c->v_qacc.p); a.x = m4(c->v_x.p); a.r = m4(c->v_r.p); a.b = c4(c->v_b.p); a.z = m4(c->v_z.p); a.cm = c4(c->v_cm.p); a.lm = c->d_lm.p;
    a.ext_off = tp.ext_off; a.ext_pos = tp.ext_pos; a.qh = reinterpret_cast<const float2*>(tp.qh); a.e0 = (int)own.off0;
    a.pq_partials = pq_part; a.d2_partials = d2_part; a.n_pq = 0; a.n_d2 = 0;
    a.n_slice_wg = pcg_step3_slice_wgs(own.n, wg_cap);
    a.sharded = sh ? 1 : 0;
    a.K = K; a.fix_poses = p.fix_poses; a.fix_intr = p.fix_intr; a.fix_dist = p.fix_dist; a.lad_sys = -1;
    a.cam_partials = c->cam_part.p; a.n_cam = 0; a.cam_stride = NSP; a.Mblk = c->Minv_blocks.p;
    a.tp = c->v_p.p + to; a.tx = c->v_x.p + to; a.tr = c->v_r.p + to; a.tb = c->v_b.p + to; a.tD2 = c->v_D2.p + to; a.tz = c->v_z.p + to; a.tS = c->v_S.p + to;
    a.step_partials = step_part;
    int n_step = 0;
    { TimedScope t(c, I3D_K_VECTOR); a.cur = st2; n_step = launch_pcg_step3(s, 0 , a); }
    const bool mr1 = c->mr1_serial && !sh && tp.T == 512 && tp.hp_off != nullptr && r.slots == 5;
    auto op = [&](double* pq, const PcgState* cur) -> int {
        if (mr1) { const int sys0[3] = {0, 0, 0}; LadVec z; std::memset(&z, 0, sizeof(z));
                   return launch_eg_tile_mr(s, r, p, tp, 1, sys0, c->v_u.p, c->v_qacc.p, tp.qh, pq, c->cam_part.p, NSP, cur, z); }
        return launch_eg_tile(s, r, p, c->v_u.p, tp, nullptr, c->v_qacc.p, pq, cur, c->cam_part.p, NSP);
    };
    const int seq0 = c->pcg_seq;
    int it = 1;
    for (;; ++it) {
        PcgState* const prev = st2 + ((it + 1) & 1); PcgState* const cur = st2 + (it & 1);
        sa.seq = seq0 + it; sa.n_slice_partials = a.n_slice_wg; a.sh = sa;
        { TimedScope t(c, I3D_K_VECTOR);
          a.n_d2 = launch_pcg_dir3(s, it == 1, own, to, L.NS, c->v_z.p, c->v_p.p, c->v_S.p, c->v_u.p, c->v_D2.p, c->v_cm.p, c->d_lm.p, step_part, n_step, d2_part, prev, cur, c->d_flags, seq0 + it,
                                   sh ? &sa : nullptr); }
        if (sh) { c->comm->count_reduce(4); c->comm->count_halo(c->halo.n_send); c->comm->count_reduce((size_t)L.NS + 1); }
        { TimedScope t(c, I3D_K_EG_PASS); a.n_pq = op(pq_part, cur); a.n_cam = a.n_pq; }
        a.cur = cur;
        if (it % 10 != 0) { TimedScope t(c, I3D_K_VECTOR); n_step = launch_pcg_step3(s, 1, a); }
        else {
            { TimedScope t(c, I3D_K_VECTOR); launch_pcg_step3(s, 2, a);
              launch_mul2(s, own, c->v_S.p, c->v_x.p, c->v_u.p); launch_mul(s, L.NS, c->v_S.p + to, c->v_x.p + to, c->v_u.p + to); }
            if (sh) { TimedScope t(c, I3D_K_COMM); launch_rim_u(s, sa, cur); c->comm->count_halo(c->halo.n_send); }
            { TimedScope t(c, I3D_K_EG_PASS); a.n_cam = op(nullptr, cur); }
            { TimedScope t(c, I3D_K_VECTOR); n_step = launch_pcg_step3(s, 3, a); }
        }
        if (it >= 2) {
            const int want = seq0 + it - 1; volatile int* ring = c->h_flags + 2 * (want & 1);
            const double t_wait = now_s();
            while (__atomic_load_n((int*)&ring[0], __ATOMIC_ACQUIRE) != want) {
                if (now_s() - t_wait > 30.0) { CTX_HIP(c, sync_stream(c)); if (__atomic_load_n((int*)&ring[0], __ATOMIC_ACQUIRE) != want) return ctx_fail(c, I3D_ERR_HIP, "pcg_solve: the device stopped publishing its state"); }
            }
            if (__atomic_load_n((int*)&ring[1], __ATOMIC_ACQUIRE)) break;
        }
        if (it > 520) break;
    }
    c->pcg_seq = seq0 + PCG_SEQ_STRIDE;
    *final_state = st2 + (it & 1);
    { const int lrc = ctx_launch_check(c); if (lrc) return lrc; }
    return I3D_OK;
}

constexpr int LAD_PART_STEP = 4 * 2048, LAD_PART_PQ = 2048, LAD_PART_D2 = 2048;
static size_t lad_redop_stride(int NS) { return ((size_t)NS + 1 + 3) & ~(size_t)3; }
static int alloc_ladder(i3d_context* c) {
    const Layout L = layout_of(c);
    const int nsys = c->ladder_max;
    LadVec& lv = c->lad;
    const size_t vec = ((size_t)L.NP + 65535) & ~(size_t)65535;
    const size_t qh = 2 * (size_t)tile_plan_tiles_of((int)std::min((size_t)c->Acap, ((size_t)c->chunk + 65535) & ~(size_t)65535), 512) * (size_t)tile_plan_hmax_of(512);
    const size_t cam = (size_t)2048 * (((size_t)L.NS + 3) & ~(size_t)3);
    lv.vec = vec; lv.qh = qh; lv.cam = cam; lv.part = LAD_PART_STEP + LAD_PART_PQ + LAD_PART_D2; lv.mblk = ((size_t)36 * c->K + 41 + 3) & ~(size_t)3; lv.tail = ((size_t)L.NS + 3) & ~(size_t)3;
    const bool fresh = c->lad_vec.n < (size_t)6 * nsys * vec || !c->lad_vec.p;
    bool ok = c->lad_vec.alloc((size_t)6 * nsys * vec) == hipSuccess;
    if (ok && fresh) ok = hipMemsetAsync(c->lad_vec.p, 0, sizeof(float) * c->lad_vec.n, c->stream) == hipSuccess;
    ok = ok && c->lad_qh.alloc((size_t)nsys * qh) == hipSuccess && c->lad_cam.alloc((size_t)nsys * cam) == hipSuccess && c->lad_part.alloc((size_t)nsys * lv.part) == hipSuccess
            && c->lad_mblk.alloc((size_t)nsys * lv.mblk) == hipSuccess && c->lad_tail.alloc((size_t)nsys * lv.tail) == hipSuccess && c->lad_st.alloc((size_t)2 * LADDER_MAX) == hipSuccess;
    if (ok && sharded(c)) {
        const size_t n = (size_t)LADDER_MAX * (4 + lad_redop_stride(L.NS));
        const bool fresh_r = c->lad_red.n < n || !c->lad_red.p;
        ok = c->lad_red.alloc(n) == hipSuccess;
        if (ok && fresh_r) ok = hipMemsetAsync(c->lad_red.p, 0, sizeof(double) * c->lad_red.n, c->stream) == hipSuccess;
    }
    if (!ok) {
        (void)hipGetLastError();
        c->lad_vec.release(); c->lad_qh.release(); c->lad_cam.release(); c->lad_part.release();
        std::fprintf(stderr, "[i3d] the slabs of the damping ladder (%d systems x %.1f MB) do not fit the device: this outer iteration runs the serial trust-region loop\n", nsys,
                     (double)(6 * vec + qh + cam) * 4.0 / 1e6);
        return 1;
    }
    return I3D_OK;
}
enum { LV_X = 0, LV_R, LV_P, LV_Z, LV_U, LV_Q };
static float* lad_vecp(const i3d_context* c, int kind, int sys = 0) { return c->lad_vec.p + ((size_t)kind * c->ladder_max + sys) * c->lad.vec; }

static int pcg_solve_ladder(i3d_context* c, const i3d_optimizer_config& cfg, const OptParams& p, int B, const PcgState** finals, int* passes_out) {
    hipStream_t s = c->stream;
    const Layout L = layout_of(c);
    const int K = c->K; const size_t to = L.tail_off; const Seg2 own = L.own;
    RowView r = c->row_view(); TilePlan tp = c->tile_plan();
    LadVec lv = c->lad;
    float* const X0 = lad_vecp(c, LV_X); float* const R0 = lad_vecp(c, LV_R); float* const P0 = lad_vecp(c, LV_P); float* const Z0 = lad_vecp(c, LV_Z);
    float* const U0 = lad_vecp(c, LV_U); float* const Q0 = lad_vecp(c, LV_Q);
    PcgState* const st2 = c->lad_st.p;
    const int NSP = (L.NS + 3) & ~3;
    double* const step_part0 = c->lad_part.p; double* const pq_part0 = step_part0 + LAD_PART_STEP; double* const d2_part0 = pq_part0 + LAD_PART_PQ;
    const bool use_mr = [] { const char* e = std::getenv("I3D_LADDER_MR"); return !(e && e[0] == '0'); }();
    const bool mr1 = [] { const char* e = std::getenv("I3D_LADDER_MR1"); return e && e[0] == '1'; }();
    const int group_cap = [] { const char* e = std::getenv("I3D_LADDER_GROUP"); const int v = e ? std::atoi(e) : 3; return v < 1 ? 1 : (v > 3 ? 3 : v); }();
    const int mr_cap = std::min(group_cap, eg_tile_mr_max_systems(K));
    const bool mr_ok = use_mr && mr_cap >= 1 && tp.T == 512 && tp.hp_off != nullptr && r.slots == 5;
    const bool sh = sharded(c);
    double* const red4 = sh ? c->lad_red.p : nullptr;
    const int rstride = (int)lad_redop_stride(L.NS);
    double* const redop = sh ? c->lad_red.p + (size_t)LADDER_MAX * 4 : nullptr;
    { TimedScope t(c, I3D_K_VECTOR);
      for (int j = 0; j < B; ++j) { CTX_HIP(c, hipMemsetAsync(X0 + (size_t)j * lv.vec, 0, sizeof(float) * L.NP, s));
                                    CTX_HIP(c, hipMemcpyAsync(R0 + (size_t)j * lv.vec, c->v_b.p, sizeof(float) * L.NP, hipMemcpyDeviceToDevice, s)); }
      launch_pcg_init_lad(s, st2, B, cfg.pcg_fixed_iterations, 500, c->d_lm.p); }
    Step3Args a; std::memset(&a, 0, sizeof(a));
    auto c4 = [&](const float* v) { return reinterpret_cast<const float4*>(v + own.off0); };
    auto m4 = [&](float* v) { return reinterpret_cast<float4*>(v + own.off0); };
    a.nq = own.n >> 2; a.chunk4 = (int)((own.off1 - own.off0) >> 2);
    a.p = c4(P0); a.qacc = c4(Q0); a.x = m4(X0); a.r = m4(R0); a.b = c4(c->v_b.p); a.z = m4(Z0); a.cm = c4(c->v_cm.p); a.lm = c->d_lm.p;
    a.ext_off = tp.ext_off; a.ext_pos = tp.ext_pos; a.qh = reinterpret_cast<const float2*>(c->lad_qh.p); a.e0 = (int)own.off0;
    a.pq_partials = pq_part0; a.d2_partials = d2_part0; a.n_pq = 0; a.n_d2 = 0;
    a.n_slice_wg = pcg_step3_slice_wgs(own.n, 0);
    a.sharded = 0; a.lad_sys = 0; a.redop = redop; a.redop_stride = rstride;
    a.K = K; a.fix_poses = p.fix_poses; a.fix_intr = p.fix_intr; a.fix_dist = p.fix_dist;
    a.cam_partials = c->lad_cam.p; a.n_cam = 0; a.cam_stride = NSP; a.Mblk = c->lad_mblk.p;
    a.tp = P0 + to; a.tx = X0 + to; a.tr = R0 + to; a.tb = c->v_b.p + to; a.tD2 = c->lad_tail.p; a.tz = Z0 + to; a.tS = c->v_S.p + to;
    a.step_partials = step_part0;
    std::vector<int> live(B); for (int j = 0; j < B; ++j) live[j] = j;
    auto set_slots = [&]() { for (int q = 0; q < LADDER_MAX; ++q) lv.sysid[q] = live[q < (int)live.size() ? q : (int)live.size() - 1]; };
    auto rows_apply = [&](int parity, bool with_dot) -> int {
        int n = 0; const int nl = (int)live.size();
        if (sh) { TimedScope t(c, I3D_K_COMM);
                  if (c->comm->push_halo_multi(U0, lv.vec, live.data(), nl, c->halo, s)) return -1; }
        if (mr_ok && (nl > 1 || mr1 || sh)) {
            const int groups = (nl + mr_cap - 1) / mr_cap;
            int at = 0;
            for (int g = 0; g < groups; ++g) {
                const int ng = (nl - at + (groups - g) - 1) / (groups - g);
                TimedScope t(c, ng == 1 ? I3D_K_EG_PASS : (ng == 2 ? I3D_K_EG_MR2 : I3D_K_EG_MR3));
                n = launch_eg_tile_mr(s, r, p, tp, ng, live.data() + at, U0, Q0, c->lad_qh.p, with_dot ? pq_part0 : nullptr, c->lad_cam.p, NSP, st2 + parity, lv);
                if (n <= 0) return -1;
                at += ng; ++c->lad_streams;
            }
        } else {
            for (int j : live) {
                TilePlan tj = tp; tj.qh = c->lad_qh.p + (size_t)j * lv.qh;
                TimedScope t(c, I3D_K_EG_PASS);
                n = launch_eg_tile(s, r, p, U0 + (size_t)j * lv.vec, tj, nullptr, Q0 + (size_t)j * lv.vec, with_dot ? pq_part0 + (size_t)j * lv.part : nullptr, st2 + 2 * j + parity,
                                   c->lad_cam.p + (size_t)j * lv.cam, NSP);
                ++c->lad_streams;
            }
        }
        c->lad_system_passes += nl;
        if (sh) {
            { TimedScope t(c, I3D_K_VECTOR); launch_lad_reduce_op(s, nl, c->lad_cam.p, n, NSP, L.NS, pq_part0, with_dot ? n : 0, d2_part0, with_dot ? a.n_d2 : 0, redop, rstride, lv); }
            if (allreduce(c, redop, (size_t)LADDER_MAX * rstride)) return -1;
        }
        return n;
    };
    auto step_sums = [&](int nl, int n_slice) -> int {
        if (!sh) return I3D_OK;
        { TimedScope t(c, I3D_K_VECTOR); launch_lad_reduce_step(s, nl, step_part0, n_slice, red4, lv); }
        return allreduce(c, red4, (size_t)LADDER_MAX * 4);
    };
    int n_step = 0;
    set_slots();
    { TimedScope t(c, I3D_K_VECTOR); a.cur = st2; n_step = launch_pcg_step3_lad(s, 0 , B, a, lv); }
    const int seq0 = c->pcg_seq;
    for (int j = 0; j < B; ++j) finals[j] = st2 + 2 * j;
    int it = 1;
    for (;; ++it) {
        set_slots();
        const int nl = (int)live.size();
        { const int rc = step_sums(nl, a.n_slice_wg); if (rc) return rc; }
        { TimedScope t(c, I3D_K_VECTOR);
          a.n_d2 = launch_pcg_dir3_lad(s, it == 1, nl, own, to, L.NS, Z0, P0, c->v_S.p, U0, c->lad_tail.p, c->v_cm.p, c->d_lm.p, step_part0, n_step, d2_part0, st2, (it + 1) & 1, c->d_flags, seq0 + it, lv,
                                       a.n_slice_wg, red4); }
        { const int n = rows_apply(it & 1, true); if (n < 0) return ctx_fail(c, I3D_ERR_STATE, "pcg_solve_ladder: the multi-system operator pass could not be launched"); a.n_pq = n; a.n_cam = n; }
        a.cur = st2 + (it & 1);
        if (it % 10 != 0) { TimedScope t(c, I3D_K_VECTOR); n_step = launch_pcg_step3_lad(s, 1, nl, a, lv); }
        else {
            { TimedScope t(c, I3D_K_VECTOR); launch_pcg_step3_lad(s, 2, nl, a, lv);
              for (int j : live) { float* xj = X0 + (size_t)j * lv.vec; float* uj = U0 + (size_t)j * lv.vec;
                                   launch_mul2(s, own, c->v_S.p, xj, uj); launch_mul(s, L.NS, c->v_S.p + to, xj + to, uj + to); } }
            { const int n = rows_apply(it & 1, false); if (n < 0) return ctx_fail(c, I3D_ERR_STATE, "pcg_solve_ladder: the multi-system operator pass could not be launched"); a.n_cam = n; }
            { TimedScope t(c, I3D_K_VECTOR); n_step = launch_pcg_step3_lad(s, 3, nl, a, lv); }
        }
        {
            const int want = seq0 + it;
            std::vector<int> still;
            for (int j : live) {
                volatile int* ring = c->h_flags + 4 * j + 2 * (want & 1);
                const double t_wait = now_s();
                while (__atomic_load_n((int*)&ring[0], __ATOMIC_ACQUIRE) != want) {
                    if (now_s() - t_wait > 30.0) { CTX_HIP(c, sync_stream(c)); if (__atomic_load_n((int*)&ring[0], __ATOMIC_ACQUIRE) != want) return ctx_fail(c, I3D_ERR_HIP, "pcg_solve_ladder: the device stopped publishing its state"); }
                }
                if (!__atomic_load_n((int*)&ring[1], __ATOMIC_ACQUIRE)) still.push_back(j);
                else finals[j] = st2 + 2 * j + (it & 1);
            }
            live.swap(still);
            if (live.empty()) break;
        }
        if (it > 520) break;
    }
    if (passes_out) *passes_out = it;
    c->pcg_seq = seq0 + PCG_SEQ_STRIDE;
    for (int j : live) finals[j] = st2 + 2 * j + (it & 1);
    { const int lrc = ctx_launch_check(c); if (lrc) return lrc; }
    return I3D_OK;
}

static int wait_record(i3d_context* c, int idx, int seq, LmRecord& out) {
    LmRecord* const r = c->h_lmrec + idx;
    const double t0 = now_s();
    while (__atomic_load_n(&r->seq, __ATOMIC_ACQUIRE) != seq) {
        if (now_s() - t0 > 60.0) {
            CTX_HIP(c, sync_stream(c));
            if (__atomic_load_n(&r->seq, __ATOMIC_ACQUIRE) != seq) return ctx_fail(c, I3D_ERR_HIP, "lm_solve: the device stopped publishing the state of the trust-region loop");
        }
    }
    out = *r;
    return I3D_OK;
}

static int lm_solve(i3d_context* c, const i3d_optimizer_config& cfg, OptParams& p, i3d_iteration_stats* st, double initial_radius) {
    hipStream_t s = c->stream;
    const Layout L = layout_of(c);
    const int N = c->N, K = c->K, NP = (int)L.NP, NS = L.NS;
    GridView g = c->grid_view(); RowView r = c->row_view();
    if (cfg.lm_steps > LM_REC_SLOTS - 2) return ctx_fail(c, I3D_ERR_CAPACITY, "optimize: more than 62 LM steps per outer iteration");
    { TimedScope t(c, I3D_K_VECTOR); launch_freemask(s, r, p, c->v_mask.p); }
    CTX_HIP(c, hipMemcpyAsync(c->xc_sdf.p, c->x_sdf.p, sizeof(double) * (size_t)N, hipMemcpyDeviceToDevice, s));
    CTX_HIP(c, hipMemcpyAsync(c->xc_alb.p, c->x_alb.p, sizeof(double) * (size_t)N, hipMemcpyDeviceToDevice, s));
    const bool one_stream = one_stream_gradcol(c);
    auto after_colnorm = [&]() -> int {
        CTX_HIP(c, hipMemcpyAsync(c->d_cam_c.p, c->d_shared.p, sizeof(double) * (size_t)NS, hipMemcpyDeviceToDevice, s));
        CTX_HIP(c, hipMemcpyAsync(c->d_cam_H.p, c->d_blocks.p, sizeof(double) * ((size_t)21 * K + 25), hipMemcpyDeviceToDevice, s));
        { int rc2 = allgather(c, c->v_c.p); if (rc2) return rc2; }
        { TimedScope t(c, I3D_K_VECTOR); launch_scale_from_colnorm(s, NP, c->v_c.p, c->v_mask.p, c->v_S.p, c->v_cm.p); }
        return I3D_OK;
    };
    int rc = I3D_OK;
    if (one_stream) { rc = run_gradcol(c, p, after_colnorm); if (rc) return rc; }
    else {
        rc = run_pass(c, PASS_COLNORM, p, nullptr, c->v_c.p); if (rc) return rc;
        rc = after_colnorm(); if (rc) return rc;
        rc = run_pass(c, PASS_GRAD, p, nullptr, c->v_acc.p); if (rc) return rc;
    }
    { TimedScope t(c, I3D_K_VECTOR); launch_mul(s, NP, c->v_S.p, c->v_acc.p, c->v_b.p); }
    if (env_off("I3D_COST0")) { rc = eval_cost_launch(c, p, false, c->d_frames.p); if (rc) return rc; }
    else if (!one_stream) { TimedScope t(c, I3D_K_VECTOR); launch_set_double(s, c->d_scal.p + 16, c->cost_at_build); }
    rc = count_above_dev(c, c->v_acc.p, c->v_mask.p, 1e-10f, c->d_scal.p + 8); if (rc) return rc;
    rc = dot_dev(c, c->v_mask.p, c->v_mask.p, c->d_scal.p + 9); if (rc) return rc;
    {
        double* xs = c->h_pinned;
        for (int i = 0; i < 6 * K; ++i) xs[i] = c->poses[i];
        for (int i = 0; i < 4; ++i) xs[6 * K + i] = c->intr[i];
        for (int i = 0; i < 5; ++i) xs[6 * K + 4 + i] = c->dist[i];
        CTX_HIP(c, hipMemcpyAsync(c->d_xshared.p, xs, sizeof(double) * NS, hipMemcpyHostToDevice, s));
    }
    const int seq0 = c->lm_seq; c->lm_seq += LM_REC_SLOTS;
    LmState* const lm = c->d_lm.p;
    launch_lm_init(s, lm, c->d_scal.p + 16, c->d_scal.p + 8, c->d_scal.p + 9, initial_radius, c->d_lmrec, seq0);

    static const bool legacy = [] { const char* e = std::getenv("I3D_PCG_LEGACY"); return e && e[0] == '1'; }();
    bool fused = c->tile_ok && !legacy;
    if (fused && sharded(c)) { P2PDev probe; fused = c->comm->fused_exchange(&probe) && L.NS + 2 <= probe.L.red_cap; }
    int attempts = 0; bool ended = false, accepted = false;
    auto consume = [&](const LmRecord& rec) {
        if (rec.kind == 0) {
            if (st) { st->cost_initial = rec.cost; st->cost_final = rec.cost; st->free_parameters = (int64_t)(rec.nfree + 0.5); st->termination = rec.final_ ? 1 : 0; st->final_radius = initial_radius; }
            c->last_sizes[5] = (long long)(rec.nfree + 0.5);
        } else if (rec.kind == 2) { if (st) st->termination = 1; }
        else {
            if (st) {
                st->lm_iterations = attempts + 1;
                if (attempts < 50) { st->pcg_iterations[attempts] = rec.pcg_it; st->step_accepted[attempts] = rec.accepted; }
                st->final_radius = rec.radius_after; st->termination = rec.termination;
                if (rec.accepted) { st->cost_final = rec.cost; st->successful_steps += 1; }
            }
            if (cfg.verbose) std::printf("  [i3d LM] it %d cand %.9e model %.3e rho %.4f radius -> %.3e cg %d%s\n", attempts + 1, rec.cand_cost, rec.model_change, rec.rel, rec.radius_after, rec.pcg_it,
                                         rec.accepted ? " accepted" : "");
            accepted = rec.accepted != 0;
            ++attempts;
        }
        if (rec.final_) ended = true;
    };
    const int dbg_invalid = [] { const char* e = std::getenv("I3D_DEBUG_INVALID_ATTEMPT"); return e ? std::atoi(e) : -1; }();
    bool ladder = c->ladder_max > 1 && c->tile_ok && !legacy && (sharded(c) ? !fused : fused) && c->plan_T() == 512 && c->tile_plan().hp_off != nullptr && c->slots == 5;
    if (ladder && alloc_ladder(c) != I3D_OK) {
        ladder = false;
    }
    if (ladder) {
        const LadVec& lv = c->lad;
        { LmRecord rec; rc = wait_record(c, 0, seq0, rec); if (rc) return rc; consume(rec); }
        const bool warm = c->ladder_hint > 0;
        int k = 0, prevB = 0; bool after_resync = false;
        while (k < cfg.lm_steps && !ended) {
            int B = after_resync ? 1 : (prevB == 0 ? (warm ? std::max(c->ladder_hint, c->ladder_hint_prev) : 2) : (warm ? 2 : 2 * prevB));
            B = std::max(1, std::min(B, std::min(c->ladder_max, cfg.lm_steps - k)));
            after_resync = false; prevB = B;
            { TimedScope t(c, I3D_K_VECTOR);
              launch_lm_begin_lad(s, lm, B, K, p.fix_poses, p.fix_intr, p.fix_dist, c->d_cam_c.p, c->d_cam_H.p, c->lad_mblk.p, lv.mblk, c->v_c.p + L.tail_off, c->v_S.p + L.tail_off, c->lad_tail.p, lv.tail,
                                  c->d_lmrec + 1 + k, seq0 + 1 + k); }
            const PcgState* fin[LADDER_MAX] = {nullptr};
            rc = pcg_solve_ladder(c, cfg, p, B, fin, nullptr); if (rc) return rc;
            ++c->lad_batches;
            for (int j = 0; j < B && sharded(c); ++j) { rc = allgather(c, lad_vecp(c, LV_X, j)); if (rc) return rc; }
            for (int j = 0; j < B; ++j) {
                { TimedScope t(c, I3D_K_VECTOR);
                  launch_candidate(s, g, r, K, -1.0f, lad_vecp(c, LV_X, j), c->v_S.p, c->d_xshared.p, c->xc_sdf.p, c->xc_alb.p, c->d_xcshared.p, c->d_scal.p + 4, c->v_mask.p, c->d_partials.p, lm);
                  launch_cand_frames(s, K, c->d_xcshared.p, c->d_frames.p, c->d_frames_cand.p, lm); }
                rc = eval_cost_launch(c, p, true, c->d_frames_cand.p, c->d_xcshared.p + 6 * K, lm); if (rc) return rc;
                { TimedScope t(c, I3D_K_VECTOR);
                  launch_lm_decide(s, lm, fin[j], c->d_scal.p + 4, c->d_scal.p + 16, k + j, cfg.lm_steps, c->d_lmrec + 1 + k + j, seq0 + 1 + k + j, j + 1, dbg_invalid == k + j ? 1 : 0);
                  launch_accept(s, g, r, c->xc_sdf.p, c->xc_alb.p, lm); }
            }
            int decided = 0;
            for (int j = 0; j < B && !ended; ++j) {
                LmRecord rec; rc = wait_record(c, 1 + k + j, seq0 + 1 + k + j, rec); if (rc) return rc;
                if (rec.kind == 3) {
                    __atomic_store_n(&c->h_lmrec[1 + k + j].seq, 0, __ATOMIC_RELEASE);
                    ++c->lad_resyncs; after_resync = true; break;
                }
                consume(rec); ++decided;
            }
            if (ended && decided < B) c->lad_wasted += B - decided;
            k += decided;
        }
        if (attempts > 0) { c->ladder_hint_prev = c->ladder_hint; c->ladder_hint = attempts; }
        ended = true;
    }
    int k = 0;
    for (; !ladder && k < cfg.lm_steps; ++k) {
        { TimedScope t(c, I3D_K_VECTOR);
          launch_lm_begin(s, lm, K, p.fix_poses, p.fix_intr, p.fix_dist, c->d_cam_c.p, c->d_cam_H.p, c->Minv_blocks.p, c->v_c.p + L.tail_off, c->v_S.p + L.tail_off, c->v_D2.p + L.tail_off, c->v_Minv.p + L.tail_off,
                          c->d_lmrec + 1 + k, seq0 + 1 + k);
          if (!fused) launch_lm_diag_dev(s, (int)L.tail_off, c->v_c.p, c->v_S.p, lm, c->v_D2.p, c->v_Minv.p); }
        const PcgState* ps = nullptr;
        rc = fused ? pcg_solve_fused(c, cfg, p, &ps) : pcg_solve(c, cfg, p, &ps); if (rc) return rc;
        { LmRecord rec; rc = wait_record(c, k, seq0 + k, rec); if (rc) return rc; consume(rec); }
        if (ended) break;
        { int rc2 = allgather(c, c->v_x.p); if (rc2) return rc2; }
        { TimedScope t(c, I3D_K_VECTOR);
          launch_candidate(s, g, r, K, -1.0f, c->v_x.p, c->v_S.p, c->d_xshared.p, c->xc_sdf.p, c->xc_alb.p, c->d_xcshared.p, c->d_scal.p + 4, c->v_mask.p, c->d_partials.p, lm);
          launch_cand_frames(s, K, c->d_xcshared.p, c->d_frames.p, c->d_frames_cand.p, lm); }
        rc = eval_cost_launch(c, p, true, c->d_frames_cand.p, c->d_xcshared.p + 6 * K, lm); if (rc) return rc;
        { TimedScope t(c, I3D_K_VECTOR);
          launch_lm_decide(s, lm, ps, c->d_scal.p + 4, c->d_scal.p + 16, k, cfg.lm_steps, c->d_lmrec + 1 + k, seq0 + 1 + k, -1, dbg_invalid == k ? 1 : 0);
          launch_accept(s, g, r, c->xc_sdf.p, c->xc_alb.p, lm); }
    }
    if (!ended) { LmRecord rec; rc = wait_record(c, k, seq0 + k, rec); if (rc) return rc; consume(rec); }
    if (st) st->num_attempts = std::min(attempts, 50);
    CTX_HIP(c, hipMemcpyAsync(c->h_pinned, c->d_xcshared.p, sizeof(double) * NS, hipMemcpyDeviceToHost, s));
    CTX_HIP(c, sync_stream(c));
    if (sharded(c) && c->comm->health(s)) return ctx_fail(c, I3D_ERR_COMM, "lm_solve: a peer-to-peer exchange timed out (a rank stopped taking part)");
    if (accepted) {
        for (int i = 0; i < 6 * K; ++i) c->poses[i] = c->h_pinned[i];
        for (int i = 0; i < 4; ++i) c->intr[i] = c->h_pinned[6 * K + i];
        for (int i = 0; i < 5; ++i) c->dist[i] = c->h_pinned[6 * K + 4 + i];
    }
    { const int lrc = ctx_launch_check(c); if (lrc) return lrc; }
    return I3D_OK;
}

int optimize(i3d_context* c, const i3d_optimizer_config& cfg, i3d_iteration_stats* stats) {
    if (!c->have_grid || cfg.iterations < 1) return ctx_fail(c, I3D_ERR_INVALID_ARGUMENT, "optimize: no grid or iterations < 1");
    CTX_HIP(c, hipSetDevice(c->device));
    double carried_radius = 1e4;
    for (int itr = 0; itr < cfg.iterations; ++itr) {
        i3d_iteration_stats local; std::memset(&local, 0, sizeof(local));
        i3d_iteration_stats* st = stats ? &stats[itr] : &local;
        std::memset(st, 0, sizeof(*st));
        OptParams p;
        const double t0 = now_s();
        int rc = assemble(c, cfg, itr, p, st); if (rc) return rc;
        const double t1 = now_s();
        st->time_add = (c->t_add_end >= 0.0 && c->t_add_end <= t1 - t0) ? c->t_add_end : t1 - t0; st->time_build = (t1 - t0) - st->time_add;
        if (c->n_active > 0) { rc = lm_solve(c, cfg, p, st, cfg.carry_trust_radius ? carried_radius : 1e4); if (rc) return rc;
                               if (st->final_radius > 0.0) carried_radius = st->final_radius; }
        const double t2 = now_s();
        st->time_solve = t2 - t1;
        if (cfg.verbose) std::printf("[i3d] itr %d rows %lld/%lld/%lld/%lld valid %lld cost %.9e -> %.9e (add %.3f ms, solve %.3f ms)\n", itr,
                                     (long long)st->rows[0], (long long)st->rows[1], (long long)st->rows[2], (long long)st->rows[3], (long long)st->valid_voxels,
                                     st->cost_initial, st->cost_final, st->time_add * 1e3, st->time_solve * 1e3);
        timing_flush(c);
// ... 60 lines not shown
```

Measured before the change: 40.15.

## Keep active count on device and replace halo pair sort with counting scatter

The active-voxel count is now written by the compact kernel and read by the partition and neighbour kernels on the device, so they are launched before the host learns the count. The host reads it through pinned memory and waits on an event instead of a full stream sync. The radix sort of halo pairs is replaced by per-voxel atomic counts, an exclusive scan, an atomic scatter and a per-run insertion sort. PCG vector initialisation is folded into the init kernel instead of per-system memsets and copies. The xc copies are moved to overlap a host read. The trade-off is launches sized for the worst-case count, grid-stride loops, and atomic-based ordering that relies on the per-run sort to stay deterministic.

```diff
diff --git a/intrinsic3d_amd/csrc/device/grid_kernels.hip b/intrinsic3d_amd/csrc/device/grid_kernels.hip
--- a/intrinsic3d_amd/csrc/device/grid_kernels.hip
+++ b/intrinsic3d_amd/csrc/device/grid_kernels.hip
@@ -117,38 +117,43 @@
 }
 
 __global__ void k_compact(int N, const int* __restrict__ flag, const int* __restrict__ scan, const uint8_t* __restrict__ flags,
-                          int* __restrict__ aidx, int* __restrict__ alist, uint8_t* __restrict__ aflags) {
+                          int* __restrict__ aidx, int* __restrict__ alist, uint8_t* __restrict__ aflags, int* __restrict__ count) {
     const int s = blockIdx.x * blockDim.x + threadIdx.x;
     if (s >= N) return;
     if (flag[s]) { const int a = scan[s]; aidx[s] = a; alist[a] = s; aflags[a] = flags[s]; } else aidx[s] = -1;
-}
-void launch_compact(hipStream_t st, int N, const int* flag, const int* scan, const uint8_t* flags, int* aidx, int* alist, uint8_t* aflags) {
-    if (N > 0) k_compact<<<(N + 255) / 256, 256, 0, st>>>(N, flag, scan, flags, aidx, alist, aflags);
-}
-
-__global__ void __launch_bounds__(512) k_partition_blocks(GridView g, int A, int* __restrict__ alist, uint8_t* __restrict__ aflags, int* __restrict__ aidx) {
+    if (s == N - 1) *count = scan[s] + flag[s];
+}
+void launch_compact(hipStream_t st, int N, const int* flag, const int* scan, const uint8_t* flags, int* aidx, int* alist, uint8_t* aflags, int* count) {
+    if (N > 0) k_compact<<<(N + 255) / 256, 256, 0, st>>>(N, flag, scan, flags, aidx, alist, aflags, count);
+}
+
+__global__ void __launch_bounds__(512) k_partition_blocks(GridView g, const int* __restrict__ A_dev, int* __restrict__ alist, uint8_t* __restrict__ aflags, int* __restrict__ aidx) {
     __shared__ int wcount[8];
-    const int base = blockIdx.x * 512, a = base + (int)threadIdx.x;
-    const bool in = a < A;
-    const int s = in ? alist[a] : -1;
-    const uint8_t fl = in ? aflags[a] : 0;
-    bool rows = in && (fl & F_ACTIVE);
-    if (rows) {
-#pragma unroll
-        for (int c = 1; c < 10; ++c) rows &= g.nbr[(size_t)slot_fwd_nbr(c) * g.N + s] >= 0;
-    }
-    const unsigned long long m = __ballot(rows);
-    const int lane = threadIdx.x & 63, w = threadIdx.x >> 6;
-    if (lane == 0) wcount[w] = __popcll(m);
-    __syncthreads();
-    int before = 0, total = 0;
-    for (int i = 0; i < 8; ++i) { const int cnt = wcount[i]; if (i < w) before += cnt; total += cnt; }
-    const int rank_rows = before + __popcll(m & ((1ull << lane) - 1ull));
-    const int pos = rows ? rank_rows : total + ((int)threadIdx.x - rank_rows);
-    if (in) { const int na = base + pos; alist[na] = s; aflags[na] = fl; aidx[s] = na; }
-}
-void launch_partition_blocks(hipStream_t st, GridView g, int A, int* alist, uint8_t* aflags, int* aidx) {
-    if (A > 0) k_partition_blocks<<<(A + 511) / 512, 512, 0, st>>>(g, A, alist, aflags, aidx);
+    const int A = *A_dev;
+    for (int base = blockIdx.x * 512; base < A; base += gridDim.x * 512) {
+        const int a = base + (int)threadIdx.x;
+        const bool in = a < A;
+        const int s = in ? alist[a] : -1;
+        const uint8_t fl = in ? aflags[a] : 0;
+        bool rows = in && (fl & F_ACTIVE);
+        if (rows) {
+#pragma unroll
+            for (int c = 1; c < 10; ++c) rows &= g.nbr[(size_t)slot_fwd_nbr(c) * g.N + s] >= 0;
+        }
+        const unsigned long long m = __ballot(rows);
+        const int lane = threadIdx.x & 63, w = threadIdx.x >> 6;
+        if (lane == 0) wcount[w] = __popcll(m);
+        __syncthreads();
+        int before = 0, total = 0;
+        for (int i = 0; i < 8; ++i) { const int cnt = wcount[i]; if (i < w) before += cnt; total += cnt; }
+        const int rank_rows = before + __popcll(m & ((1ull << lane) - 1ull));
+        const int pos = rows ? rank_rows : total + ((int)threadIdx.x - rank_rows);
+        if (in) { const int na = base + pos; alist[na] = s; aflags[na] = fl; aidx[s] = na; }
+        __syncthreads();
+    }
+}
+void launch_partition_blocks(hipStream_t st, GridView g, int A_max, const int* A_dev, int* alist, uint8_t* aflags, int* aidx) {
+    if (A_max > 0) k_partition_blocks<<<std::min((A_max + 511) / 512, 4096), 512, 0, st>>>(g, A_dev, alist, aflags, aidx);
 }
 __global__ void k_group_rows(int A, const uint8_t* __restrict__ nrows, int* __restrict__ gmax) {
     const int gq = blockIdx.x * blockDim.x + threadIdx.x;
@@ -159,15 +164,16 @@
 }
 void launch_group_rows(hipStream_t st, int A, const uint8_t* nrows, int* gmax) { if (A > 0) k_group_rows<<<((A + 63) / 64 + 255) / 256, 256, 0, st>>>(A, nrows, gmax); }
 
-__global__ void k_anbr(int N, int A, int Acap, const int* __restrict__ alist, const int* __restrict__ nbr, const int* __restrict__ aidx, int* __restrict__ anbr) {
-    const int a = blockIdx.x * blockDim.x + threadIdx.x;
-    if (a >= A) return;
-    const int s = alist[a];
-#pragma unroll
-    for (int i = 0; i < NUM_NBR; ++i) { const int nb = nbr[(size_t)i * N + s]; anbr[(size_t)i * Acap + a] = nb >= 0 ? aidx[nb] : -1; }
-}
-void launch_anbr(hipStream_t st, int N, int A, int Acap, const int* alist, const int* nbr, const int* aidx, int* anbr) {
-    if (A > 0) k_anbr<<<(A + 255) / 256, 256, 0, st>>>(N, A, Acap, alist, nbr, aidx, anbr);
+__global__ void k_anbr(int N, const int* __restrict__ A_dev, int Acap, const int* __restrict__ alist, const int* __restrict__ nbr, const int* __restrict__ aidx, int* __restrict__ anbr) {
+    const int A = *A_dev;
+    for (int a = blockIdx.x * blockDim.x + threadIdx.x; a < A; a += gridDim.x * blockDim.x) {
+        const int s = alist[a];
+#pragma unroll
+        for (int i = 0; i < NUM_NBR; ++i) { const int nb = nbr[(size_t)i * N + s]; anbr[(size_t)i * Acap + a] = nb >= 0 ? aidx[nb] : -1; }
+    }
+}
+void launch_anbr(hipStream_t st, int N, int A_max, const int* A_dev, int Acap, const int* alist, const int* nbr, const int* aidx, int* anbr) {
+    if (A_max > 0) k_anbr<<<std::min((A_max + 255) / 256, 16384), 256, 0, st>>>(N, A_dev, Acap, alist, nbr, aidx, anbr);
 }
 
 __global__ void k_scatter_sh(int N, const int* __restrict__ rank, const double* __restrict__ shv, float* __restrict__ sh) {
diff --git a/intrinsic3d_amd/csrc/device/kernels.hpp b/intrinsic3d_amd/csrc/device/kernels.hpp
--- a/intrinsic3d_amd/csrc/device/kernels.hpp
+++ b/intrinsic3d_amd/csrc/device/kernels.hpp
@@ -13,10 +13,10 @@
 void launch_hash_build(hipStream_t st, int N, const int* cx, const int* cy, const int* cz, HashTable t);
 void launch_nbr_build(hipStream_t st, int N, const int* cx, const int* cy, const int* cz, HashTable t, int* nbr);
 void launch_classify(hipStream_t st, GridView g, OptParams p, int* active_flag);
-void launch_compact(hipStream_t st, int N, const int* active_flag, const int* active_scan, const uint8_t* flags, int* aidx, int* alist, uint8_t* aflags);
-void launch_partition_blocks(hipStream_t st, GridView g, int A, int* alist, uint8_t* aflags, int* aidx);
+void launch_compact(hipStream_t st, int N, const int* active_flag, const int* active_scan, const uint8_t* flags, int* aidx, int* alist, uint8_t* aflags, int* count );
+void launch_partition_blocks(hipStream_t st, GridView g, int A_max, const int* A_dev, int* alist, uint8_t* aflags, int* aidx);
 void launch_group_rows(hipStream_t st, int A, const uint8_t* nrows, int* gmax);
-void launch_anbr(hipStream_t st, int N, int A, int Acap, const int* alist, const int* nbr, const int* aidx, int* anbr);
+void launch_anbr(hipStream_t st, int N, int A_max, const int* A_dev, int Acap, const int* alist, const int* nbr, const int* aidx, int* anbr);
 void launch_scatter_sh(hipStream_t st, int N, const int* rank, const double* sh_visit , float* sh );
 void launch_gather_visit(hipStream_t st, int N, const int* rank, const double* x_sdf, const double* x_alb, double* out_sdf, double* out_alb);
 void launch_update_fields(hipStream_t st, int N, const int* rank, const double* sdf_ref, const double* alb, const uint8_t* rgb,
@@ -89,7 +89,8 @@
     unsigned* lnbr;
     float* eaw_sym;
     int* halo_idx; int* halo_cnt;
-    int* iota; int* ext_e; int* ext_pos;
+    int* pair_cnt;
+    int* ext_e; int* ext_pos;
     float* qh;
     int* ext_off;
     int* overflow;
@@ -107,12 +108,11 @@
 int    tile_plan_hmax();
 inline int tile_plan_hmax_of(int T) { return T == 1024 ? 2048 : 1536; }
 inline int tile_plan_tiles_of(int A, int T) { return (A + T - 1) / T; }
-size_t tile_plan_temp_bytes(int ntiles);
+size_t tile_plan_temp_bytes(size_t n_off);
 hipError_t launch_tile_plan(hipStream_t st, RowView r, TilePlan t, void* temp, size_t temp_bytes);
 void launch_eaw_sym(hipStream_t st, RowView r, TilePlan t, const int* cflag );
 int  launch_eg_tile(hipStream_t st, RowView r, OptParams p, const float* u, TilePlan t, double* shared, float* qacc, double* pq_partials ,
                     const PcgState* state, float* cam_partials = nullptr, int cam_stride = 0);
-void launch_ext_offsets(hipStream_t st, int n, const int* ext_e, int A, int* ext_off);
 void eg_tile_launch_shape(const TilePlan& t, int K, int& blocks, int& tiles_per_block);
 
 struct LadVec;
@@ -160,7 +160,8 @@
 int  pcg_step3_tail_wgs(int K);
 int  launch_pcg_step3(hipStream_t st, int mode , Step3Args a);
 void launch_halo_fold(hipStream_t st, RowView r, TilePlan t, float* qacc, const PcgState* state);
-void launch_pcg_init_lad(hipStream_t st, PcgState* st2_all , int B, int fixed_iterations, int max_iterations, const LmState* lm);
+void launch_pcg_init_lad(hipStream_t st, PcgState* st2_all , int B, int fixed_iterations, int max_iterations, const LmState* lm,
+                         int NP, size_t vec, const float* b, float* x0, float* r0);
 int  launch_pcg_dir3_lad(hipStream_t st, bool init, int nsys, Seg2 sg, size_t tail_off, int ntail, const float* z0, float* p0, const float* S, float* u0, const float* tD2_0, const float* cm, const LmState* lm,
                          const double* step_partials0, int n_step, double* d2_partials0, PcgState* st2_0, int prev_parity, int* host_flags0, int seq, const LadVec& lv,
                          int n_slice_partials = 0, const double* red4_0 = nullptr );
diff --git a/intrinsic3d_amd/csrc/device/pcg_fused.hip b/intrinsic3d_amd/csrc/device/pcg_fused.hip
--- a/intrinsic3d_amd/csrc/device/pcg_fused.hip
+++ b/intrinsic3d_amd/csrc/device/pcg_fused.hip
@@ -479,9 +479,19 @@
     k_lad_reduce_op<<<dim3((NS + 63) / 64 + 1, nsys), PF_THREADS, 0, st>>>(cam_partials0, n_cam, cam_stride, NS, pq_partials0, n_pq, d2_partials0, n_d2, redop0, redop_stride, lv);
 }
 
-__global__ void k_pcg_init_lad(PcgState* st2_all, int B, int fixed_iterations, int max_iterations, const LmState* lm) {
+__global__ void __launch_bounds__(256) k_pcg_init_lad(PcgState* st2_all, int B, int fixed_iterations, int max_iterations, const LmState* lm,
+                                                      int NP, size_t vec, const float* __restrict__ b, float* __restrict__ x0, float* __restrict__ r0) {
+    const int n4 = NP >> 2;
+    for (int i = blockIdx.x * blockDim.x + threadIdx.x; i < n4; i += gridDim.x * blockDim.x) {
+        const float4 bv = reinterpret_cast<const float4*>(b)[i];
+        for (int k = 0; k < B; ++k) { reinterpret_cast<float4*>(x0 + (size_t)k * vec)[i] = make_float4(0.0f, 0.0f, 0.0f, 0.0f); reinterpret_cast<float4*>(r0 + (size_t)k * vec)[i] = bv; }
+    }
+    if (blockIdx.x == 0 && (int)threadIdx.x < NP - 4 * n4) {
+        const int i = 4 * n4 + (int)threadIdx.x;
+        for (int k = 0; k < B; ++k) { x0[(size_t)k * vec + i] = 0.0f; r0[(size_t)k * vec + i] = b[i]; }
+    }
     const int j = threadIdx.x;
-    if (j >= B) return;
+    if (blockIdx.x != 0 || j >= B) return;
     const bool over = lm->done != 0 || lm->lad_radius[j] < 1e-32;
     for (int b = 0; b < 2; ++b) {
         PcgState* st = st2_all + 2 * j + b;
@@ -490,15 +500,9 @@
         st->Q0 = 0.0; st->Q1 = 0.0; st->it = 0; st->done = (fixed_iterations == 0 || over) ? 1 : 0; st->fixed_iterations = fixed_iterations; st->max_iterations = max_iterations;
     }
 }
-void launch_pcg_init_lad(hipStream_t st, PcgState* st2_all, int B, int fixed_iterations, int max_iterations, const LmState* lm) { k_pcg_init_lad<<<1, LADDER_MAX, 0, st>>>(st2_all, B, fixed_iterations, max_iterations, lm); }
-
-__global__ void k_ext_offsets(int n, const int* __restrict__ ext_e, int A, int* __restrict__ ext_off) {
-    const int e = blockIdx.x * blockDim.x + threadIdx.x;
-    if (e > A) return;
-    int lo = 0, hi = n;
-    while (lo < hi) { const int mid = (lo + hi) >> 1; if (ext_e[mid] < e) lo = mid + 1; else hi = mid; }
-    ext_off[e] = lo;
-}
-void launch_ext_offsets(hipStream_t st, int n, const int* ext_e, int A, int* ext_off) { k_ext_offsets<<<(A + 1 + 255) / 256, 256, 0, st>>>(n, ext_e, A, ext_off); }
-
-}
+void launch_pcg_init_lad(hipStream_t st, PcgState* st2_all, int B, int fixed_iterations, int max_iterations, const LmState* lm, int NP, size_t vec, const float* b, float* x0, float* r0) {
+    const int blocks = std::max(1, std::min(2048, ((NP >> 2) + 255) / 256));
+    k_pcg_init_lad<<<blocks, 256, 0, st>>>(st2_all, B, fixed_iterations, max_iterations, lm, NP, vec, b, x0, r0);
+}
+
+}
diff --git a/intrinsic3d_amd/csrc/device/tile_pass.hip b/intrinsic3d_amd/csrc/device/tile_pass.hip
--- a/intrinsic3d_amd/csrc/device/tile_pass.hip
+++ b/intrinsic3d_amd/csrc/device/tile_pass.hip
@@ -18,7 +18,7 @@
 }
 
 __global__ void __launch_bounds__(1024) k_tile_plan(RowView r, int T, int hmax, int hlimit , int tile_first, const int* __restrict__ tile_list, unsigned* __restrict__ lnbr,
-                                                    int* __restrict__ halo_idx, int* __restrict__ halo_cnt, int* __restrict__ overflow) {
+                                                    int* __restrict__ halo_idx, int* __restrict__ halo_cnt, int* __restrict__ pair_cnt, int* __restrict__ overflow) {
     __shared__ int hkeys[4096];
     __shared__ int hlist[TP_PLAN_LIST];
     __shared__ int cnt;
@@ -64,6 +64,7 @@
             __syncthreads();
         }
     for (int i = threadIdx.x; i < hmax; i += 1024) halo_idx[(size_t)tile * hmax + i] = hlist[i];
+    for (int i = threadIdx.x; i < H; i += 1024) atomicAdd(&pair_cnt[hlist[i]], 1);
     if (threadIdx.x == 0) halo_cnt[tile] = H;
     if (!in) return;
     unsigned short ls[18];
@@ -505,10 +506,10 @@
 #undef Cme
 }
 
-__global__ void __launch_bounds__(256) k_halo_fold(int n, const int* __restrict__ ext_e, const int* __restrict__ ext_pos, const float* __restrict__ qh,
+__global__ void __launch_bounds__(256) k_halo_fold(const int* __restrict__ n_pairs, const int* __restrict__ ext_e, const int* __restrict__ ext_pos, const float* __restrict__ qh,
                                                    float* __restrict__ qacc, int chunk, const PcgState* __restrict__ state) {
     if (state && state->done) return;
-    const int i = blockIdx.x * blockDim.x + threadIdx.x;
+    const int i = blockIdx.x * blockDim.x + threadIdx.x, n = *n_pairs;
     if (i >= n) return;
     const int e = ext_e[i];
     if (e >= TP_NONE || (i > 0 && ext_e[i - 1] == e)) return;
@@ -517,15 +518,29 @@
     qacc[e] += s; qacc[chunk + e] += al;
 }
 
-__global__ void k_iota(int n, int* __restrict__ x) { const int i = blockIdx.x * blockDim.x + threadIdx.x; if (i < n) x[i] = i; }
+__global__ void __launch_bounds__(256) k_pair_scatter(int hmax, const int* __restrict__ halo_idx, const int* __restrict__ halo_cnt, const int* __restrict__ ext_off,
+                                                      int* __restrict__ pair_cnt, int* __restrict__ ext_e, int* __restrict__ ext_pos) {
+    const int tile = blockIdx.x, H = halo_cnt[tile];
+    for (int i = threadIdx.x; i < H; i += 256) {
+        const int slot = tile * hmax + i, e = halo_idx[slot];
+        const int j0 = ext_off[e], pos = j0 + atomicSub(&pair_cnt[e], 1) - 1;
+        if (pos >= j0 && pos < ext_off[e + 1]) { ext_e[pos] = e; ext_pos[pos] = slot; }
+    }
+}
+__global__ void __launch_bounds__(256) k_pair_runs(int A, const int* __restrict__ ext_off, int* __restrict__ ext_pos) {
+    const int e = blockIdx.x * blockDim.x + threadIdx.x;
+    if (e >= A) return;
+    const int j0 = ext_off[e], j1 = ext_off[e + 1];
+    for (int i = j0 + 1; i < j1; ++i) { const int v = ext_pos[i]; int j = i - 1; while (j >= j0 && ext_pos[j] > v) { ext_pos[j + 1] = ext_pos[j]; --j; } ext_pos[j + 1] = v; }
+}
 
 static int tp_T() { const char* e = std::getenv("I3D_EGT_TILE"); return (e && std::atoi(e) == 512) ? 512 : 1024; }
 static int tp_H() { return tp_T() == 1024 ? 2048 : 1536; }
 int tile_plan_tiles(int A) { return (A + tp_T() - 1) / tp_T(); }
 int tile_plan_hmax() { return tp_H(); }
-size_t tile_plan_temp_bytes(int ntiles) {
+size_t tile_plan_temp_bytes(size_t n_off) {
     size_t bytes = 0;
-    (void)rocprim::radix_sort_pairs(nullptr, bytes, (const int*)nullptr, (int*)nullptr, (const int*)nullptr, (int*)nullptr, (size_t)ntiles * tp_H(), 0, 32, (hipStream_t)0);
+    (void)rocprim::exclusive_scan(nullptr, bytes, (const int*)nullptr, (int*)nullptr, 0, n_off, rocprim::plus<int>(), (hipStream_t)0);
     return bytes;
 }
 
@@ -541,8 +556,8 @@
     const bool all = t.tile_first == 0 && t.ntiles_own >= ntiles;
     if (!all) { e = hipMemsetAsync(t.halo_idx, 0x7f, sizeof(int) * (size_t)n, st); if (e != hipSuccess) return e;
                 e = hipMemsetAsync(t.halo_cnt, 0, sizeof(int) * (size_t)ntiles, st); if (e != hipSuccess) return e; }
-    if (t.ntiles_own > 0) k_tile_plan<<<t.ntiles_own, 1024, 0, st>>>(r, t.T, t.hmax, hlimit, t.tile_first, nullptr, t.lnbr, t.halo_idx, t.halo_cnt, t.overflow);
-    if (t.n_ghost > 0) k_tile_plan<<<t.n_ghost, 1024, 0, st>>>(r, t.T, t.hmax, hlimit, 0, t.ghost_tiles, t.lnbr, t.halo_idx, t.halo_cnt, t.overflow);
+    if (t.ntiles_own > 0) k_tile_plan<<<t.ntiles_own, 1024, 0, st>>>(r, t.T, t.hmax, hlimit, t.tile_first, nullptr, t.lnbr, t.halo_idx, t.halo_cnt, t.pair_cnt, t.overflow);
+    if (t.n_ghost > 0) k_tile_plan<<<t.n_ghost, 1024, 0, st>>>(r, t.T, t.hmax, hlimit, 0, t.ghost_tiles, t.lnbr, t.halo_idx, t.halo_cnt, t.pair_cnt, t.overflow);
     if (t.hp_off) {
         unsigned short* off = const_cast<unsigned short*>(t.hp_off); unsigned short* src = const_cast<unsigned short*>(t.hp_src);
         if (t.T == 1024) { if (t.ntiles_own > 0) k_tile_pull_plan<1024, 2048><<<t.ntiles_own, 1024, 0, st>>>(r, t.tile_first, nullptr, t.lnbr, t.halo_cnt, off, src, t.overflow);
@@ -550,12 +565,10 @@
         else { if (t.ntiles_own > 0) k_tile_pull_plan<512, 1536><<<t.ntiles_own, 512, 0, st>>>(r, t.tile_first, nullptr, t.lnbr, t.halo_cnt, off, src, t.overflow);
                if (t.n_ghost > 0) k_tile_pull_plan<512, 1536><<<t.n_ghost, 512, 0, st>>>(r, 0, t.ghost_tiles, t.lnbr, t.halo_cnt, off, src, t.overflow); }
     }
-    k_iota<<<(n + 255) / 256, 256, 0, st>>>(n, t.iota);
-    int key_bits = 32;
-    for (int b = 1; b < 32; ++b) { const unsigned mask = (1u << b) - 1u; if ((1u << b) >= (unsigned)r.A && ((unsigned)TP_NONE & mask) >= (unsigned)r.A) { key_bits = b; break; } }
-    e = rocprim::radix_sort_pairs(temp, temp_bytes, (const int*)t.halo_idx, t.ext_e, (const int*)t.iota, t.ext_pos, (size_t)n, 0, key_bits, st);
+    e = rocprim::exclusive_scan(temp, temp_bytes, (const int*)t.pair_cnt, t.ext_off, 0, (size_t)r.chunk + 1, rocprim::plus<int>(), st);
     if (e != hipSuccess) return e;
-    if (t.ext_off) launch_ext_offsets(st, n, t.ext_e, r.chunk, t.ext_off);
+    k_pair_scatter<<<ntiles, 256, 0, st>>>(t.hmax, t.halo_idx, t.halo_cnt, t.ext_off, t.pair_cnt, t.ext_e, t.ext_pos);
+    k_pair_runs<<<(r.A + 255) / 256, 256, 0, st>>>(r.A, t.ext_off, t.ext_pos);
     return hipGetLastError();
 }
 
@@ -634,7 +647,7 @@
 void launch_halo_fold(hipStream_t st, RowView r, TilePlan t, float* qacc, const PcgState* state) {
     if (r.A <= 0) return;
     const int n = tile_plan_tiles_of(r.A, t.T) * t.hmax;
-    k_halo_fold<<<(n + 255) / 256, 256, 0, st>>>(n, t.ext_e, t.ext_pos, t.qh, qacc, r.chunk, state);
+    k_halo_fold<<<(n + 255) / 256, 256, 0, st>>>(t.ext_off + r.chunk, t.ext_e, t.ext_pos, t.qh, qacc, r.chunk, state);
 }
 int tile_plan_T() { return tp_T(); }
 
diff --git a/intrinsic3d_amd/csrc/host/context.cpp b/intrinsic3d_amd/csrc/host/context.cpp
--- a/intrinsic3d_amd/csrc/host/context.cpp
+++ b/intrinsic3d_amd/csrc/host/context.cpp
@@ -116,6 +116,7 @@
     if (c->h_flags) (void)hipHostFree(c->h_flags);
     if (c->h_lmrec) (void)hipHostFree(c->h_lmrec);
     for (auto e : c->ev_asm) if (e) (void)hipEventDestroy(e);
+    if (c->ev_count) (void)hipEventDestroy(c->ev_count);
     for (auto e : c->pcg_ev) if (e) (void)hipEventDestroy(e);
     delete c->comm;
     if (c->stream) (void)hipStreamDestroy(c->stream);
diff --git a/intrinsic3d_amd/csrc/host/context.hpp b/intrinsic3d_amd/csrc/host/context.hpp
--- a/intrinsic3d_amd/csrc/host/context.hpp
+++ b/intrinsic3d_amd/csrc/host/context.hpp
@@ -50,6 +50,7 @@
 
     int N = 0; float voxel_size = 0, truncation = 0;
     i3d::DevBuf<int> cx, cy, cz, rank, nbr, aidx, alist, aflag, ascan;
+    i3d::DevBuf<int> acount;
     i3d::DevBuf<double> sdf0, x_sdf, x_alb, xc_sdf, xc_alb;
     i3d::DevBuf<float> f_sdf, f_alb, weight, sh;
     i3d::DevBuf<uchar4> color;
@@ -86,7 +87,7 @@
     double cost_at_build = 0.0;
     i3d::DevBuf<float> C2, treg2, gc_part;
     i3d::DevBuf<float> aux_part;
-    i3d::DevBuf<unsigned> tp_lnbr; i3d::DevBuf<int> tp_halo_idx, tp_halo_cnt, tp_iota, tp_ext_e, tp_ext_pos, tp_ext_off, tp_overflow; i3d::DevBuf<float> tp_qh, tp_eaw, cam_part;
+    i3d::DevBuf<unsigned> tp_lnbr; i3d::DevBuf<int> tp_halo_idx, tp_halo_cnt, tp_pair_cnt, tp_ext_e, tp_ext_pos, tp_ext_off, tp_overflow; i3d::DevBuf<float> tp_qh, tp_eaw, cam_part;
     i3d::DevBuf<unsigned char> tp_temp; bool tile_ok = false;
     i3d::DevBuf<unsigned short> tp_hp_off, tp_hp_src; bool halo_pull = false;
     bool ladder_lists = false;
@@ -108,7 +109,7 @@
         const int T = plan_T();
         const bool sh = comm && (comm->world > 1 || comm->force);
         const int t0 = sh ? own0 / T : 0, t1 = sh ? (own1 + T - 1) / T : i3d::tile_plan_tiles_of(A, T);
-        return i3d::TilePlan{tp_lnbr.p, tp_eaw.p, tp_halo_idx.p, tp_halo_cnt.p, tp_iota.p, tp_ext_e.p, tp_ext_pos.p, tp_qh.p, tp_ext_off.p, tp_overflow.p, T, i3d::tile_plan_hmax_of(T), t0, t1 > t0 ? t1 - t0 : 0,
+        return i3d::TilePlan{tp_lnbr.p, tp_eaw.p, tp_halo_idx.p, tp_halo_cnt.p, tp_pair_cnt.p, tp_ext_e.p, tp_ext_pos.p, tp_qh.p, tp_ext_off.p, tp_overflow.p, T, i3d::tile_plan_hmax_of(T), t0, t1 > t0 ? t1 - t0 : 0,
                              ghost_tiles.p, sh ? n_ghost_tiles : 0, deterministic ? 1 : 0, (halo_pull || ladder_lists) ? tp_hp_off.p : nullptr, (halo_pull || ladder_lists) ? tp_hp_src.p : nullptr, halo_pull ? 1 : 0};
     }
 
@@ -119,6 +120,7 @@
     int* h_flags = nullptr; int* d_flags = nullptr; int pcg_seq = 1024;
     i3d::DevBuf<i3d::LmState> d_lm; i3d::LmRecord* h_lmrec = nullptr; i3d::LmRecord* d_lmrec = nullptr; int lm_seq = 1;
     i3d::DevBuf<double> d_cam_c, d_cam_H;
+    hipEvent_t ev_count = nullptr;
     hipEvent_t ev_asm[2] = {nullptr, nullptr};
     long long n_syncs = 0;
     double* h_pinned = nullptr; size_t h_pinned_n = 0;
diff --git a/intrinsic3d_amd/csrc/host/solver.cpp b/intrinsic3d_amd/csrc/host/solver.cpp
--- a/intrinsic3d_amd/csrc/host/solver.cpp
+++ b/intrinsic3d_amd/csrc/host/solver.cpp
@@ -60,11 +60,14 @@
     {
       const size_t nt = (size_t)tile_plan_tiles_of((int)Acap, 512);
       const size_t nh = std::max(nt * (size_t)tile_plan_hmax_of(512), (size_t)tile_plan_tiles_of((int)Acap, 1024) * (size_t)tile_plan_hmax_of(1024));
-      CTX_HIP(c, c->tp_lnbr.alloc(Acap * LNBR_WORDS)); CTX_HIP(c, c->tp_eaw.alloc(Acap * 6)); CTX_HIP(c, c->tp_halo_idx.alloc(nh)); CTX_HIP(c, c->tp_halo_cnt.alloc(nt)); CTX_HIP(c, c->tp_iota.alloc(nh));
+      CTX_HIP(c, c->tp_lnbr.alloc(Acap * LNBR_WORDS)); CTX_HIP(c, c->tp_eaw.alloc(Acap * 6)); CTX_HIP(c, c->tp_halo_idx.alloc(nh)); CTX_HIP(c, c->tp_halo_cnt.alloc(nt));
       CTX_HIP(c, c->tp_ext_e.alloc(nh)); CTX_HIP(c, c->tp_ext_pos.alloc(nh)); CTX_HIP(c, c->tp_qh.alloc(2 * nh)); CTX_HIP(c, c->tp_overflow.alloc(1));
-      CTX_HIP(c, c->tp_ext_off.alloc(Acap + (size_t)SHARD_ALIGN * ((c->comm ? c->comm->world : 1) + 1) + 8));
+      const size_t n_off = Acap + (size_t)SHARD_ALIGN * ((c->comm ? c->comm->world : 1) + 1) + 8;
+      CTX_HIP(c, c->tp_ext_off.alloc(n_off));
+      { const bool fresh = c->tp_pair_cnt.n < n_off || !c->tp_pair_cnt.p;
+        CTX_HIP(c, c->tp_pair_cnt.alloc(n_off)); if (fresh) CTX_HIP(c, hipMemsetAsync(c->tp_pair_cnt.p, 0, sizeof(int) * c->tp_pair_cnt.n, c->stream)); }
       CTX_HIP(c, c->cam_part.alloc((size_t)2048 * (((size_t)6 * c->K + 9 + 3) & ~(size_t)3)));
-      CTX_HIP(c, c->tp_temp.alloc(tile_plan_temp_bytes((int)nt))); }
+      CTX_HIP(c, c->tp_temp.alloc(tile_plan_temp_bytes(n_off))); }
     const int world_a = c->comm ? c->comm->world : 1;
     const size_t NP = 2 * ((size_t)c->N + (size_t)SHARD_ALIGN * (world_a + 1)) + 6 * (size_t)c->K + 9;
     for (DevBuf<float>* v : {&c->v_mask, &c->v_c, &c->v_S, &c->v_cm, &c->v_D2, &c->v_Minv, &c->v_b, &c->v_x, &c->v_r, &c->v_p, &c->v_z, &c->v_q, &c->v_u, &c->v_acc, &c->v_tmp, &c->v_qacc})
@@ -92,6 +95,8 @@
                        std::memset(c->h_lmrec, 0, LM_REC_SLOTS * sizeof(LmRecord));
                        CTX_HIP(c, hipHostGetDevicePointer((void**)&c->d_lmrec, c->h_lmrec, 0)); }
     for (auto& e : c->ev_asm) if (!e) CTX_HIP(c, hipEventCreate(&e));
+    if (!c->ev_count) CTX_HIP(c, hipEventCreateWithFlags(&c->ev_count, hipEventDisableTiming));
+    CTX_HIP(c, c->acount.alloc(1));
     return ensure_pinned(c, 64 + (size_t)27 * c->K + 64);
 }
 
@@ -207,18 +212,18 @@
     { TimedScope t(c, I3D_K_CLASSIFY);
       launch_classify(s, g, p, c->aflag.p);
       CTX_HIP(c, rocprim::exclusive_scan(c->scan_tmp.p, c->scan_tmp_bytes, c->aflag.p, c->ascan.p, 0, (size_t)c->N, rocprim::plus<int>(), s));
-      launch_compact(s, c->N, c->aflag.p, c->ascan.p, c->flags.p, c->aidx.p, c->alist.p, c->aflags.p); }
-    int tail[2];
-    CTX_HIP(c, hipMemcpyAsync(&tail[0], c->ascan.p + (c->N - 1), sizeof(int), hipMemcpyDeviceToHost, s));
-    CTX_HIP(c, hipMemcpyAsync(&tail[1], c->aflag.p + (c->N - 1), sizeof(int), hipMemcpyDeviceToHost, s));
-    std::vector<FrameConst> fc; build_frame_consts(c, cfg.rgbd_level, c->poses.data(), fc);
-    CTX_HIP(c, sync_stream(c));
-    CTX_HIP(c, hipMemcpyAsync(c->d_frames.p, fc.data(), sizeof(FrameConst) * fc.size(), hipMemcpyHostToDevice, s));
-    c->A = tail[0] + tail[1];
+      launch_compact(s, c->N, c->aflag.p, c->ascan.p, c->flags.p, c->aidx.p, c->alist.p, c->aflags.p, c->acount.p); }
+    int* const h_count = reinterpret_cast<int*>(c->h_pinned + c->h_pinned_n - 1);
+    CTX_HIP(c, hipMemcpyAsync(h_count, c->acount.p, sizeof(int), hipMemcpyDeviceToHost, s));
+    CTX_HIP(c, hipEventRecord(c->ev_count, s));
     { TimedScope t(c, I3D_K_CLASSIFY);
       static const bool no_partition = [] { const char* e = std::getenv("I3D_NO_PARTITION"); return e && e[0] == '1'; }();
-      if (!no_partition) launch_partition_blocks(s, g, c->A, c->alist.p, c->aflags.p, c->aidx.p);
-      launch_anbr(s, c->N, c->A, c->Acap, c->alist.p, c->nbr.p, c->aidx.p, c->anbr.p); }
+      if (!no_partition) launch_partition_blocks(s, g, c->N, c->acount.p, c->alist.p, c->aflags.p, c->aidx.p);
+      launch_anbr(s, c->N, c->N, c->acount.p, c->Acap, c->alist.p, c->nbr.p, c->aidx.p, c->anbr.p); }
+    std::vector<FrameConst> fc; build_frame_consts(c, cfg.rgbd_level, c->poses.data(), fc);
+    ++c->n_syncs; CTX_HIP(c, hipEventSynchronize(c->ev_count));
+    c->A = *h_count;
+    CTX_HIP(c, hipMemcpyAsync(c->d_frames.p, fc.data(), sizeof(FrameConst) * fc.size(), hipMemcpyHostToDevice, s));
     c->tile_ok = false; c->tile_T = 0;
     { const char* e = std::getenv("I3D_DETERMINISTIC"); c->deterministic = e ? e[0] == '1' : !sharded(c); }
     {
@@ -282,9 +287,15 @@
     CTX_HIP(c, hipMemsetAsync(c->d_scal.p, 0, sizeof(double) * 32, s));
     { TimedScope t(c, I3D_K_VECTOR); launch_weight_sums(s, r, g, cost_from_sums(c), c->d_scal.p, c->d_partials.p); }
     { int rc = allreduce(c, c->d_scal.p, 13); if (rc) return rc; }
-    int tp_over = 1;
-    CTX_HIP(c, hipMemcpyAsync(&tp_over, c->tp_overflow.p, sizeof(int), hipMemcpyDeviceToHost, s));
-    double sums[13]; { int rc = read_doubles(c, c->d_scal.p, 13, sums); if (rc) return rc; }
+    int* const h_over = reinterpret_cast<int*>(c->h_pinned + c->h_pinned_n - 2);
+    CTX_HIP(c, hipMemcpyAsync(h_over, c->tp_overflow.p, sizeof(int), hipMemcpyDeviceToHost, s));
+    CTX_HIP(c, hipMemcpyAsync(c->h_pinned, c->d_scal.p, 13 * sizeof(double), hipMemcpyDeviceToHost, s));
+    CTX_HIP(c, hipEventRecord(c->ev_count, s));
+    CTX_HIP(c, hipMemcpyAsync(c->xc_sdf.p, c->x_sdf.p, sizeof(double) * (size_t)c->N, hipMemcpyDeviceToDevice, s));
+    CTX_HIP(c, hipMemcpyAsync(c->xc_alb.p, c->x_alb.p, sizeof(double) * (size_t)c->N, hipMemcpyDeviceToDevice, s));
+    ++c->n_syncs; CTX_HIP(c, hipEventSynchronize(c->ev_count));
+    int tp_over = *h_over;
+    double sums[13]; std::memcpy(sums, c->h_pinned, sizeof(sums));
     if (sharded(c) && c->comm->health(s)) return ctx_fail(c, I3D_ERR_COMM, "assemble: a peer-to-peer exchange timed out (a rank stopped taking part)");
     if (!sharded(c) && tp_over != 0) {
         const int other = c->plan_T() == 1024 ? 512 : 1024;
@@ -607,10 +618,7 @@
     double* const red4 = sh ? c->lad_red.p : nullptr;
     const int rstride = (int)lad_redop_stride(L.NS);
     double* const redop = sh ? c->lad_red.p + (size_t)LADDER_MAX * 4 : nullptr;
-    { TimedScope t(c, I3D_K_VECTOR);
-      for (int j = 0; j < B; ++j) { CTX_HIP(c, hipMemsetAsync(X0 + (size_t)j * lv.vec, 0, sizeof(float) * L.NP, s));
-                                    CTX_HIP(c, hipMemcpyAsync(R0 + (size_t)j * lv.vec, c->v_b.p, sizeof(float) * L.NP, hipMemcpyDeviceToDevice, s)); }
-      launch_pcg_init_lad(s, st2, B, cfg.pcg_fixed_iterations, 500, c->d_lm.p); }
+    { TimedScope t(c, I3D_K_VECTOR); launch_pcg_init_lad(s, st2, B, cfg.pcg_fixed_iterations, 500, c->d_lm.p, (int)L.NP, lv.vec, c->v_b.p, X0, R0); }
     Step3Args a; std::memset(&a, 0, sizeof(a));
     auto c4 = [&](const float* v) { return reinterpret_cast<const float4*>(v + own.off0); };
     auto m4 = [&](float* v) { return reinterpret_cast<float4*>(v + own.off0); };
@@ -724,12 +732,10 @@
 static int lm_solve(i3d_context* c, const i3d_optimizer_config& cfg, OptParams& p, i3d_iteration_stats* st, double initial_radius) {
     hipStream_t s = c->stream;
     const Layout L = layout_of(c);
-    const int N = c->N, K = c->K, NP = (int)L.NP, NS = L.NS;
+    const int K = c->K, NP = (int)L.NP, NS = L.NS;
     GridView g = c->grid_view(); RowView r = c->row_view();
     if (cfg.lm_steps > LM_REC_SLOTS - 2) return ctx_fail(c, I3D_ERR_CAPACITY, "optimize: more than 62 LM steps per outer iteration");
     { TimedScope t(c, I3D_K_VECTOR); launch_freemask(s, r, p, c->v_mask.p); }
-    CTX_HIP(c, hipMemcpyAsync(c->xc_sdf.p, c->x_sdf.p, sizeof(double) * (size_t)N, hipMemcpyDeviceToDevice, s));
-    CTX_HIP(c, hipMemcpyAsync(c->xc_alb.p, c->x_alb.p, sizeof(double) * (size_t)N, hipMemcpyDeviceToDevice, s));
     const bool one_stream = one_stream_gradcol(c);
     auto after_colnorm = [&]() -> int {
         CTX_HIP(c, hipMemcpyAsync(c->d_cam_c.p, c->d_shared.p, sizeof(double) * (size_t)NS, hipMemcpyDeviceToDevice, s));
```

Measured after the change: 40.74 (median of 6 runs). 1.01x the previous value.
